# timweiland/DiffEqGMRFs.jl

Hardware: AMD Instinct MI355X
Metric: GMRF posterior solves/sec (mean+samples), 256^2 Darcy (higher is better)
Workload: dtype f64; 1 GPU; darcy256: n=65536, 64 blocks x 1024, nnz=1624084; 256 independent posterior(s) per GPU and step (4 stream(s) x batch 64), each factor + mean + 64 samples; mode=problems, samples_per_problem_per_rank=64, l_blocks_kept=False

## Files before the change

diffeqgmrfs.jl_amd/_cabi.py:

```python
from __future__ import annotations

import ctypes as C
import os
from typing import Optional

_HERE = os.path.dirname(os.path.abspath(__file__))
LIB_PATH = os.environ.get("GMRF_HIP_LIBRARY") or os.path.join(_HERE, "csrc", "libgmrf_hip.so")

GMRF_OK = 0
ERR_NOT_SPD, ERR_BAD_SHAPE, ERR_BAND, ERR_HIP, ERR_NO_FACTOR, ERR_NO_DEVICE, ERR_ALLOC, ERR_RCCL = -1, -2, -3, -4, -5, -6, -7, -8
SOLVE_FULL, SOLVE_FORWARD, SOLVE_BACKWARD = 0, 1, 2
VAR_EXACT, VAR_RBMC, VAR_MC = 0, 1, 2
BLOCK_L, BLOCK_C, BLOCK_LINV = 0, 1, 2
ORDER_REFERENCE, ORDER_TWISTED = 0, 1

EXPORTS = [
    "gmrf_bt_create", "gmrf_bt_destroy", "gmrf_last_error", "gmrf_version",
    "gmrf_bt_factor_csc", "gmrf_bt_factor_blocks", "gmrf_bt_refactor_values",
    "gmrf_bt_solve", "gmrf_bt_sample", "gmrf_bt_posterior", "gmrf_bt_set_factor_rhs", "gmrf_bt_normals", "gmrf_bt_marginal_var",
    "gmrf_bt_var_accumulate", "gmrf_bt_logdet", "gmrf_bt_get_block", "gmrf_bt_factor_buffer",
    "gmrf_bt_adopt_shape", "gmrf_bt_adopt_commit", "gmrf_bt_adopt_layout", "gmrf_bt_get_layout", "gmrf_bt_block_range",
    "gmrf_bt_set_keep_l", "gmrf_bt_storage_bytes", "gmrf_bt_set_storage", "gmrf_bt_factor_begin_csc",
    "gmrf_bt_factor_step_async", "gmrf_bt_factor_end", "gmrf_bt_stats",
    "gmrf_bt_set_profiling", "gmrf_bt_set_eager", "gmrf_bt_synchronize", "gmrf_bt_set_batch", "gmrf_bt_select_problem",
    "gmrf_bt_marginal_var_batch", "gmrf_bt_selinv", "gmrf_bt_trace_inv", "gmrf_bt_set_order", "gmrf_bt_get_order", "gmrf_bt_half_stats", "gmrf_bt_export_size", "gmrf_bt_export_factor", "gmrf_bt_import_factor",
    "gmrf_comm_unique_id", "gmrf_comm_create", "gmrf_comm_destroy", "gmrf_comm_bcast_host", "gmrf_comm_allreduce_sum",
    "gmrf_bt_bcast_blocks_async", "gmrf_bt_allgather_blocks_async", "gmrf_comm_wait", "gmrf_comm_bytes", "gmrf_streams_create", "gmrf_streams_destroy",
    "gmrf_bt_packed_size", "gmrf_bt_pack_blocks_async", "gmrf_bt_unpack_blocks_async",
    "gmrf_csr_create", "gmrf_csr_destroy", "gmrf_spmm", "gmrf_spmm_rows", "gmrf_spmm_async", "gmrf_spmm_rows_async",
    "gmrf_darcy_p1_create", "gmrf_darcy_p2_create", "gmrf_darcy_p1_destroy", "gmrf_darcy_p1_pattern", "gmrf_darcy_p1_assemble",
    "gmrf_burgers_p1_create", "gmrf_burgers_p2_create", "gmrf_burgers_p1_destroy", "gmrf_burgers_p1_pattern", "gmrf_burgers_p1_tangent",
    "gmrf_shallow_water_p1_create", "gmrf_shallow_water_p1_destroy", "gmrf_shallow_water_p1_pattern", "gmrf_shallow_water_p1_qpoints",
    "gmrf_shallow_water_p1_assemble", "gmrf_shallow_water_p1_operators",
    "gmrf_assemble_create", "gmrf_assemble_destroy", "gmrf_assemble_pattern", "gmrf_assemble_precision", "gmrf_assemble_rhs",
    "gmrf_burgers_p1_tangent_batch", "gmrf_assemble_precision_batch", "gmrf_assemble_rhs_batch", "gmrf_assemble_objective_batch",
    "gmrf_gn_create", "gmrf_gn_destroy", "gmrf_gn_run", "gmrf_gn_finalize",
    "gmrf_elliptic_p1_create", "gmrf_elliptic_p1_destroy", "gmrf_elliptic_p1_pattern", "gmrf_elliptic_p1_qpoints",
    "gmrf_elliptic_p1_tangent", "gmrf_elliptic_p1_tangent_batch", "gmrf_elliptic_p1_load", "gmrf_gn_create_elliptic",
    "gmrf_darcy_p1_assemble_batch", "gmrf_dc_create", "gmrf_dc_destroy", "gmrf_dc_run",
    "gmrf_burgers_prior_create", "gmrf_burgers_prior_destroy", "gmrf_burgers_prior_pattern", "gmrf_burgers_prior_values_batch",
    "gmrf_bic_create", "gmrf_bic_destroy", "gmrf_bic_run", "gmrf_field_errors_batch",
    "gmrf_test_gemm", "gmrf_test_gemm_rate", "gmrf_test_gemm_shapes", "gmrf_test_potrf_tile", "gmrf_test_potrf_block", "gmrf_test_tile_timing", "gmrf_test_persist_stamps", "gmrf_test_persist_aborts", "gmrf_test_factor_fwd", "gmrf_test_gn_route", "gmrf_test_dc_route", "gmrf_test_bic_route", "gmrf_test_var_groups", "gmrf_test_persist_budget", "gmrf_test_clock_probe_start", "gmrf_test_clock_probe_finish",
    "gmrf_test_mfma_f64_rate", "gmrf_test_hbm_rate", "gmrf_test_microbench", "gmrf_test_symbolic_csc",
]


class SparseBlock(C.Structure):
    _fields_ = [("nnz", C.c_int64), ("ptr", C.c_void_p), ("idx", C.c_void_p), ("val", C.c_void_p)]


class Stats(C.Structure):
    _fields_ = [
        ("factor_ms", C.c_double), ("solve_ms", C.c_double), ("sample_ms", C.c_double),
        ("factor_flops", C.c_double), ("sweep_bytes", C.c_double), ("sweep_ms", C.c_double),
        ("n", C.c_int64), ("n_blocks", C.c_int64), ("block_size", C.c_int64),
        ("block_size_padded", C.c_int64), ("factor_bytes", C.c_int64),
        ("kernel_ms", C.c_double * 24), ("kernel_work", C.c_double * 24), ("kernel_launches", C.c_int64 * 24),
        ("sweep_bytes_streamed", C.c_double),
        ("persist_route", C.c_int32), ("persist_aborts", C.c_int32), ("persist_cus", C.c_int32), ("persist_refused", C.c_int32),
        ("sweep_persist", C.c_int32), ("sweep_persist_launches", C.c_int32),
    ]


class GmrfError(RuntimeError):
    def __init__(self, status: int, msg: str, info: int = 0):
        super().__init__(f"libgmrf_hip status {status}: {msg}")
        self.status = status
        self.info = info


class NotPositiveDefinite(GmrfError):
    """Julia's PosDefException(info): `.info` is the failing block (1-based)."""


_lib: Optional[C.CDLL] = None


def load() -> C.CDLL:
    global _lib
    if _lib is not None:
        return _lib
    if not os.path.exists(LIB_PATH):
        raise ImportError(
            f"{LIB_PATH} is missing: build it with `python -c 'import __graft_entry__ as g; g.build()'` "
            "or `make -C diffeqgmrfs.jl_amd/csrc` (the HIP library is the only compute path)")
    try:
        import torch
    except Exception:
        pass
    lib = C.CDLL(LIB_PATH)
    vp, i32, i64, u64, dbl = C.c_void_p, C.c_int32, C.c_int64, C.c_uint64, C.c_double
    P = C.POINTER
    sigs = {
        "gmrf_bt_create": [i32, vp, P(vp)],
        "gmrf_bt_destroy": [vp],
        "gmrf_version": [],
        "gmrf_bt_factor_csc": [vp, i64, i64, vp, vp, vp, i32, P(i32)],
        "gmrf_bt_factor_blocks": [vp, i64, i64, vp, vp, i32, i32, P(i32)],
        "gmrf_bt_refactor_values": [vp, vp, P(i32)],
        "gmrf_bt_solve": [vp, vp, vp, i64, i64, i64, i32],
        "gmrf_bt_sample": [vp, u64, i64, i64, vp, vp, vp, i64],
        "gmrf_bt_posterior": [vp, vp, u64, i64, i64, vp, vp, i64],
        "gmrf_bt_set_factor_rhs": [vp, vp],
        "gmrf_bt_normals": [vp, u64, i64, i64, vp, i64],
        "gmrf_bt_marginal_var": [vp, i32, i64, u64, vp, vp],
        "gmrf_bt_var_accumulate": [vp, i32, i64, i64, u64, vp, vp],
        "gmrf_bt_logdet": [vp, P(dbl)],
        "gmrf_bt_get_block": [vp, i32, i64, vp, i64],
        "gmrf_bt_factor_buffer": [vp, i32, P(vp), P(i64)],
        "gmrf_bt_adopt_shape": [vp, i64, i64],
        "gmrf_bt_storage_bytes": [i64, i64, i64, P(i64), P(i64), P(i64)],
        "gmrf_bt_set_storage": [vp, i64, i64, i64, vp, vp, vp],
        "gmrf_bt_adopt_commit": [vp, i32],
        "gmrf_bt_adopt_layout": [vp, i64, i64, vp, i64],
        "gmrf_bt_get_layout": [vp, vp, i64, P(i64)],
        "gmrf_bt_block_range": [vp, i32, i64, i64, P(i64), P(i64), P(i64)],
        "gmrf_bt_set_keep_l": [vp, i32],
        "gmrf_comm_unique_id": [vp],
        "gmrf_comm_create": [i32, i32, i32, vp, P(vp)],
        "gmrf_comm_destroy": [vp],
        "gmrf_comm_bcast_host": [vp, vp, i64, i32],
        "gmrf_comm_allreduce_sum": [vp, vp, vp, i64],
        "gmrf_bt_bcast_blocks_async": [vp, vp, i32, i64, i64, i32],
        "gmrf_bt_allgather_blocks_async": [vp, vp, vp, i64, i64],
        "gmrf_comm_wait": [vp, vp],
        "gmrf_comm_bytes": [vp, i32, P(dbl)],
        "gmrf_bt_packed_size": [vp, i64, i64, P(i64)],
        "gmrf_bt_pack_blocks_async": [vp, i64, i64, vp],
        "gmrf_bt_unpack_blocks_async": [vp, i64, i64, vp],
        "gmrf_streams_create": [i32, i32, vp, vp],
        "gmrf_streams_destroy": [i32, i32, vp],
        "gmrf_bt_factor_begin_csc": [vp, i64, i64, vp, vp, vp, i32],
        "gmrf_bt_factor_step_async": [vp, i64, i64],
        "gmrf_bt_factor_end": [vp, P(i32)],
        "gmrf_bt_stats": [vp, P(Stats)],
        "gmrf_bt_set_order": [vp, i32, i64],
        "gmrf_bt_get_order": [vp, P(i32), P(i64)],
        "gmrf_bt_half_stats": [vp, i32, P(Stats)],
        "gmrf_bt_set_profiling": [vp, i32],
        "gmrf_bt_set_eager": [vp, i32],
        "gmrf_bt_synchronize": [vp],
        "gmrf_bt_set_batch": [vp, i64],
        "gmrf_bt_select_problem": [vp, i64],
        "gmrf_csr_create": [i32, vp, i64, i64, vp, vp, vp, i32, i32, P(vp)],
        "gmrf_bt_marginal_var_batch": [vp, i32, i64, u64, vp, vp, vp],
        "gmrf_bt_selinv": [vp, vp, vp],
        "gmrf_bt_trace_inv": [vp, vp, vp, i64, vp],
        "gmrf_bt_export_size": [vp, P(i64)],
        "gmrf_bt_export_factor": [vp, vp, i64],
        "gmrf_bt_import_factor": [vp, vp, i64],
        "gmrf_csr_destroy": [vp],
        "gmrf_assemble_create": [i32, vp, i64, vp, vp, i64, vp, vp, i32, P(vp)],
        "gmrf_assemble_destroy": [vp],
        "gmrf_assemble_pattern": [vp, P(i64), P(i64), vp, vp, i32],
        "gmrf_assemble_precision": [vp, vp, vp, dbl, vp],
        "gmrf_assemble_rhs": [vp, vp, vp, vp, vp, dbl, vp],
        "gmrf_darcy_p1_create": [i32, vp, i64, i64, P(vp)],
        "gmrf_darcy_p2_create": [i32, vp, i64, i64, P(vp)],
        "gmrf_darcy_p1_destroy": [vp],
        "gmrf_darcy_p1_pattern": [vp, P(i64), vp, vp, i32],
        "gmrf_darcy_p1_assemble": [vp, vp, i64, dbl, vp, vp],
        "gmrf_burgers_p1_create": [i32, vp, i64, i64, dbl, dbl, P(vp)],
        "gmrf_burgers_p2_create": [i32, vp, i64, i64, dbl, dbl, P(vp)],
        "gmrf_burgers_p1_destroy": [vp],
        "gmrf_burgers_p1_pattern": [vp, P(i64), vp, vp, i32],
        "gmrf_burgers_p1_tangent": [vp, vp, vp, vp],
        "gmrf_burgers_p1_tangent_batch": [vp, i64, vp, vp, vp],
        "gmrf_assemble_precision_batch": [vp, i64, vp, i64, vp, dbl, vp],
        "gmrf_assemble_rhs_batch": [vp, i64, vp, vp, vp, vp, dbl, vp],
        "gmrf_assemble_objective_batch": [vp, i64, vp, i64, vp, vp, vp, dbl, vp],
        "gmrf_gn_create": [vp, vp, vp, P(vp)],
        "gmrf_gn_create_elliptic": [vp, vp, vp, P(vp)],
        "gmrf_elliptic_p1_create": [i32, vp, i64, i64, P(vp)],
        "gmrf_elliptic_p1_destroy": [vp],
        "gmrf_elliptic_p1_pattern": [vp, P(i64), vp, vp, i32],
        "gmrf_elliptic_p1_qpoints": [vp, vp],
        "gmrf_elliptic_p1_tangent": [vp, vp, vp, vp],
        "gmrf_elliptic_p1_tangent_batch": [vp, i64, vp, vp, vp],
        "gmrf_elliptic_p1_load": [vp, i64, vp, vp],
        "gmrf_gn_destroy": [vp],
        "gmrf_gn_run": [vp, vp, i64, vp, vp, vp, vp, dbl, dbl, i32, vp, vp, P(i32)],
        "gmrf_gn_finalize": [vp, P(i32)],
        "gmrf_darcy_p1_assemble_batch": [vp, i64, vp, i64, dbl, vp, vp],
        "gmrf_dc_create": [vp, vp, vp, P(vp)],
        "gmrf_dc_destroy": [vp],
        "gmrf_dc_run": [vp, vp, i64, dbl, vp, i64, vp, dbl, i64, u64, i32, i64, u64, vp, vp, vp, vp, P(i32)],
        "gmrf_burgers_prior_create": [i32, vp, i64, i64, dbl, dbl, dbl, P(vp)],
        "gmrf_burgers_prior_destroy": [vp],
        "gmrf_burgers_prior_pattern": [vp, P(i64), vp, vp, i32],
        "gmrf_burgers_prior_values_batch": [vp, i64, vp, vp, vp, vp],
        "gmrf_bic_create": [vp, vp, vp, P(vp)],
        "gmrf_bic_destroy": [vp],
        "gmrf_bic_run": [vp, vp, vp, vp, vp, vp, P(i32)],
        "gmrf_field_errors_batch": [i32, vp, i64, i64, i64, vp, vp, vp],
        "gmrf_shallow_water_p1_create": [i32, vp, i64, i64, P(vp)],
        "gmrf_shallow_water_p1_destroy": [vp],
        "gmrf_shallow_water_p1_pattern": [vp, i32, P(i64), vp, vp, i32],
        "gmrf_shallow_water_p1_qpoints": [vp, vp],
        "gmrf_shallow_water_p1_assemble": [vp, vp, dbl, dbl, dbl, vp, vp, vp, vp],
        "gmrf_shallow_water_p1_operators": [vp, vp, vp, vp, vp, dbl, dbl, dbl, vp, vp, vp, vp],
        "gmrf_spmm": [vp, vp, vp, i64, i64, i64],
        "gmrf_spmm_async": [vp, vp, vp, i64, i64, i64],
        "gmrf_spmm_rows_async": [vp, vp, vp, i64, i64, i64],
        "gmrf_spmm_rows": [vp, vp, vp, i64, i64, i64],
        "gmrf_test_gemm": [i32, i64, i64, i64, i32, i32, i32, i32, dbl, vp, i64, vp, i64, dbl, vp, i64],
        "gmrf_test_gemm_shapes": [vp, P(dbl), i64, P(i64)],
        "gmrf_test_gemm_rate": [i32, i64, i64, i64, i32, i32, i32, i32, i32, i32, P(dbl)],
        "gmrf_test_potrf_tile": [i32, vp, vp, P(i32)],
        "gmrf_test_potrf_block": [i32, i64, vp, vp, P(i32)],
        "gmrf_test_tile_timing": [vp, i32],
        "gmrf_test_persist_stamps": [vp, i32],
        "gmrf_test_persist_aborts": [vp, vp],
        "gmrf_test_factor_fwd": [vp, vp, vp],
        "gmrf_test_gn_route": [vp, P(i32), P(i32)],
        "gmrf_test_dc_route": [vp, vp],
        "gmrf_test_bic_route": [vp, vp],
        "gmrf_test_var_groups": [vp, vp, vp],
        "gmrf_test_persist_budget": [i32, i32, vp, vp],
        "gmrf_test_clock_probe_start": [i32, i32, i32, P(vp)],
        "gmrf_test_clock_probe_finish": [vp, vp, vp],
        "gmrf_test_mfma_f64_rate": [i32, P(dbl)],
        "gmrf_test_hbm_rate": [i32, i64, P(dbl)],
        "gmrf_test_microbench": [i32, vp, i32],
        "gmrf_test_symbolic_csc": [i64, i64, vp, vp, i32, vp],
    }
    for name, args in sigs.items():
        fn = getattr(lib, name)
        fn.argtypes = args
        fn.restype = i32
    lib.gmrf_last_error.argtypes = []
    lib.gmrf_last_error.restype = C.c_char_p
    _lib = lib
    return lib


def check(status: int, info: int = 0):
    if status == GMRF_OK:
        return
    msg = load().gmrf_last_error().decode(errors="replace")
    if status == ERR_NOT_SPD:
        raise NotPositiveDefinite(status, msg, info)
    raise GmrfError(status, msg, info)


def ptr(a) -> C.c_void_p:
    if a is None:
        return C.c_void_p(0)
    if isinstance(a, int):
        return C.c_void_p(a)
    if hasattr(a, "data_ptr"):
        return C.c_void_p(a.data_ptr())
    return C.c_void_p(a.ctypes.data)
```

diffeqgmrfs.jl_amd/csrc/gemm_f64.hpp:

```cpp
#pragma once
#include <hip/hip_runtime.h>
#include <hip/hip_ext.h>
#include <stdint.h>
#include <stdlib.h>
#include <algorithm>
#include <array>
#include <map>
#include <mutex>
#include <vector>

namespace gmrf {

typedef double v4d __attribute__((ext_vector_type(4)));
typedef double v2d __attribute__((ext_vector_type(2)));

enum : int {
    TRI_A_LOWER = 1,
    TRI_A_UPPER = 2,
    TRI_B_LOWER = 4,
    TRI_B_UPPER = 8
};

struct GemmArgs {
    const double* A;
    const double* B;
    double* C;
    int64_t lda, ldb, ldc;
    int64_t strideA, strideB, strideC;
    int64_t pA, pB, pC;
    int nb1;
    int M, N, K;
    int tri;
    int lower_only;
    double alpha, beta;
    const double* D;
    int64_t ldd, pD;
    unsigned long long* stamps;
    const int* kb_m = nullptr;
    const int* kb_n = nullptr;
    const int* ke_n = nullptr;
    const double* tA = nullptr;
    double* tC = nullptr;
    const double* tD = nullptr;
    int64_t ptA = 0, ptC = 0, ptD = 0;
    double tbeta = 0.0;
};

constexpr int GEMM_BM = 64;
constexpr int GEMM_BN = 64;

template <bool ROWS_CONTIG, int BK>
__device__ __forceinline__ void gemm_load_tile(const double* __restrict__ P, int64_t ld, int row0, int k0,
                                               int t, v2d (&rg)[BK / 8]) {
    if (!ROWS_CONTIG) {
        constexpr int TPR = BK / 2, RPP = 256 / TPR;
        const int r = t / TPR, kk = (t % TPR) * 2;
        const double* p = P + (int64_t)(row0 + r) * ld + k0 + kk;
#pragma unroll
        for (int i = 0; i < BK / 8; ++i) rg[i] = *reinterpret_cast<const v2d*>(p + (int64_t)(i * RPP) * ld);
    } else {
        const int kk = t >> 5, r = (t & 31) * 2;
        const double* p = P + (int64_t)(k0 + kk) * ld + row0 + r;
#pragma unroll
        for (int i = 0; i < BK / 8; ++i) rg[i] = *reinterpret_cast<const v2d*>(p + (int64_t)(i * 8) * ld);
    }
}

template <bool ROWS_CONTIG, int BK>
__device__ __forceinline__ void gemm_tile_offsets(int64_t ld, int row0, int t, uint32_t (&off)[BK / 8]) {
    if (!ROWS_CONTIG) {
        constexpr int TPR = BK / 2, RPP = 256 / TPR;
        const int r = t / TPR, kk = (t % TPR) * 2;
#pragma unroll
        for (int i = 0; i < BK / 8; ++i) off[i] = (uint32_t)(((int64_t)(row0 + r + i * RPP) * ld + kk) * 8);
    } else {
        const int kk = t >> 5, r = (t & 31) * 2;
#pragma unroll
        for (int i = 0; i < BK / 8; ++i) off[i] = (uint32_t)(((int64_t)(kk + i * 8) * ld + row0 + r) * 8);
    }
}
template <bool ROWS_CONTIG>
__device__ __forceinline__ const char* gemm_tile_base(const double* P, int64_t ld, int k0) {
    return reinterpret_cast<const char*>(ROWS_CONTIG ? P + (int64_t)k0 * ld : P + k0);
}
template <int BK>
__device__ __forceinline__ void gemm_load_tile_off(const char* base, uint32_t (&off)[BK / 8], v2d (&rg)[BK / 8]) {
#pragma unroll
    for (int i = 0; i < BK / 8; ++i) {
        asm volatile("" : "+v"(off[i]));
        rg[i] = *reinterpret_cast<const v2d*>(base + off[i]);
    }
}

template <int BK>
__device__ __forceinline__ void gemm_store_tile_natural(double* sm, int t, const v2d (&rg)[BK / 8]) {
    const int kk = t >> 5, r = (t & 31) * 2;
#pragma unroll
    for (int i = 0; i < BK / 8; ++i) *reinterpret_cast<v2d*>(sm + (kk + 8 * i) * 64 + r) = rg[i];
}

template <bool ROWS_CONTIG, int BK>
__device__ __forceinline__ void gemm_store_tile(double* sm, int t, const v2d (&rg)[BK / 8]) {
    constexpr int LD = BK + 4;
    if (!ROWS_CONTIG) {
        constexpr int TPR = BK / 2, RPP = 256 / TPR;
        const int r = t / TPR, kk = (t % TPR) * 2;
#pragma unroll
        for (int i = 0; i < BK / 8; ++i) *reinterpret_cast<v2d*>(sm + (r + i * RPP) * LD + kk) = rg[i];
    } else {
        const int kk = t >> 5, r = (t & 31) * 2;
#pragma unroll
        for (int i = 0; i < BK / 8; ++i) {
            sm[r * LD + kk + 8 * i] = rg[i].x;
            sm[(r + 1) * LD + kk + 8 * i] = rg[i].y;
        }
    }
}

template <int BT>
__device__ __forceinline__ void gemm_tile_order(const GemmArgs& g, int& bm, int& bn, int& z) {
    const int nx = g.N / BT, ny = g.M / BT;
    const int tpp = g.lower_only == 1 ? nx * (nx + 1) / 2 : nx * ny;
    const int nz = (int)gridDim.x / tpp;
    const int groups = (nz % 8 == 0) ? 8 : 1;
    const int xg = (int)blockIdx.x % groups, q = (int)blockIdx.x / groups, nzg = nz / groups;
    int zq;
    if (g.lower_only == 1) {
        const int tile = q % tpp;
// ... 594 lines not shown
```

diffeqgmrfs.jl_amd/csrc/gemm_f64_dma.hpp:

```cpp
#pragma once
#include "gemm_f64.hpp"

namespace gmrf {

constexpr int DMA_BK = 16;
constexpr int DMA_ROWS_ASCENDING = 1024;
#ifndef GMRF_DMA_READS_FIRST
#define GMRF_DMA_READS_FIRST 0
#endif

template <int BM, int BN>
constexpr size_t gemm_dma_lds_bytes(int stages) { return (size_t)stages * (BM + BN) * DMA_BK * sizeof(double); }

#define GMRF_LDS_PTR(p) ((__attribute__((address_space(3))) void*)(p))
#define GMRF_GLB_PTR(p) ((const __attribute__((address_space(1))) void*)(p))

template <int BM, int BN>
__device__ __forceinline__ void gemm_dma_tile_order(const GemmArgs& g, int& bm, int& bn, int& z) {
    const int nx = g.N / BN, ny = g.M / BM;
    int tpp;
    if (g.lower_only == 1) {
        if (BM >= BN) tpp = (BM / BN) * ny * (ny + 1) / 2;
        else tpp = 0;
    } else tpp = nx * ny;
    const int nz = (int)gridDim.x / tpp;
    const int groups = (nz % 8 == 0) ? 8 : 1;
    const int xg = (int)blockIdx.x % groups, q = (int)blockIdx.x / groups, nzg = nz / groups;
    int zq;
    if (g.lower_only == 1) {
        constexpr int R = BM / BN > 0 ? BM / BN : 1;
        const int tile = q % tpp;
        zq = q / tpp;
        const int tr = (g.tri & DMA_ROWS_ASCENDING) ? tile : tpp - 1 - tile;
        int b = (int)((sqrtf(8.0f * (float)(tr / R) + 1.0f) - 1.0f) * 0.5f);
        while (R * b * (b + 1) / 2 > tr) --b;
        while (R * (b + 1) * (b + 2) / 2 <= tr) ++b;
        bm = b;
        bn = tr - R * b * (b + 1) / 2;
    } else {
        const bool cls_n = (g.tri & (TRI_B_LOWER | TRI_B_UPPER)) || !(g.tri & (TRI_A_LOWER | TRI_A_UPPER));
        const bool desc = cls_n ? ((g.tri & TRI_B_UPPER) != 0 || (g.ke_n && !g.kb_n)) : (g.tri & TRI_A_LOWER) != 0;
        const int ncls = cls_n ? nx : ny, other = cls_n ? ny : nx;
        int c = q / (other * nzg);
        const int rem = q % (other * nzg);
        const int o = rem % other;
        zq = rem / other;
        if (desc) c = ncls - 1 - c;
        bn = cls_n ? c : o;
        bm = cls_n ? o : c;
    }
    z = xg + groups * zq;
}

template <int BM, int BN, bool B_N, int STAGES, bool A_T = false, bool TAIL = false>
__global__ __launch_bounds__(256, (BM + BN > 128) ? 3 : 4) void gemm_f64_dma(GemmArgs g) {
    constexpr int BK = DMA_BK;
    constexpr int MI = BM / 32, NJ = BN / 32;
    constexpr int NA = BM / 32, NB = BN / 32;
    constexpr int A_ST = BM * BK, B_ST = BN * BK, T_ST = TAIL ? BK : 0, ST = A_ST + B_ST + T_ST;
    static_assert(NJ % 2 == 0 || !B_N, "the [k][n] image pairs neighbouring column tiles");
    static_assert(MI % 2 == 0 || !A_T, "the [k][m] image pairs neighbouring row tiles");
    static_assert(!TAIL || (BM == 64 && BN == 64 && !A_T), "the tail row: 64 x 64 tiles");
    int bm, bn, z;
    gemm_dma_tile_order<BM, BN>(g, bm, bn, z);
    const bool tail = TAIL && (g.lower_only == 1 ? bm == bn : bm == g.M / BM - 1);
    const int m0 = bm * BM, n0 = bn * BN;
    if (g.lower_only == 2 && n0 > m0 + BM - 1) return;
    const int zi = z % g.nb1, zp = z / g.nb1;
    const double* __restrict__ A = g.A + (int64_t)zi * g.strideA + (int64_t)zp * g.pA;
    const double* __restrict__ B = g.B + (int64_t)zi * g.strideB + (int64_t)zp * g.pB;
    double* C = g.C + (int64_t)zi * g.strideC + (int64_t)zp * g.pC;
    const double* Dm = g.D ? g.D + (int64_t)zp * g.pD : C;
    const int64_t ldd = g.D ? g.ldd : g.ldc;

    int kb = 0, ke = g.K;
    if (g.tri & TRI_A_LOWER) ke = min(ke, m0 + BM);
    if (g.tri & TRI_A_UPPER) kb = max(kb, m0);
    if (g.tri & TRI_B_LOWER) kb = max(kb, n0);
    if (g.tri & TRI_B_UPPER) ke = min(ke, n0 + BN);
    if (g.kb_m) kb = max(kb, g.kb_m[bm * (BM / 64)]);
    if (g.kb_n) kb = max(kb, g.kb_n[bn * (BN / 64)]);
    if (g.ke_n) ke = min(ke, g.ke_n[bn * (BN / 64) + BN / 64 - 1]);
    const int nkt = (ke > kb) ? (ke - kb) / BK : 0;

    extern __shared__ __attribute__((aligned(16))) double gsm[];
    const int t = threadIdx.x;
    const int lane = t & 63, w = __builtin_amdgcn_readfirstlane(t >> 6);
    const int wm = (w >> 1) * (BM / 2), wn = (w & 1) * (BN / 2);
    const int li = lane & 15, lq = lane >> 4;
    const bool idle = g.lower_only != 0 && ((n0 + wn) / 64 > (m0 + wm + BM / 2 - 1) / 64);

    uint32_t offa[NA], offb[NB];
#pragma unroll
    for (int i = 0; i < NA; ++i) {
        const int q = w + 4 * i;
        if (A_T) {
            constexpr int LPR = BM / 2;
            const int k = q * (64 / LPR) + lane / LPR, col = (lane % LPR) * 2;
            offa[i] = (uint32_t)(((int64_t)k * g.lda + m0 + col) * 8);
        } else {
            const int row = 8 * q + (lane >> 3), ch = (lane & 7) ^ ((row >> 1) & 7);
            offa[i] = (uint32_t)(((int64_t)(m0 + row) * g.lda + 2 * ch) * 8);
        }
    }
#pragma unroll
    for (int i = 0; i < NB; ++i) {
        const int q = w + 4 * i;
        if (B_N) {
            constexpr int LPR = BN / 2;
            const int k = q * (64 / LPR) + lane / LPR, col = (lane % LPR) * 2;
            offb[i] = (uint32_t)(((int64_t)k * g.ldb + n0 + col) * 8);
        } else {
            const int row = 8 * q + (lane >> 3), ch = (lane & 7) ^ ((row >> 1) & 7);
            offb[i] = (uint32_t)(((int64_t)(n0 + row) * g.ldb + 2 * ch) * 8);
        }
    }
    const double* arow = g.tC ? g.tA + (int64_t)zp * g.ptA : A + (int64_t)g.M * g.lda;
    auto issue = [&](int kt, int stage) {
        const int k0 = kb + kt * BK;
        const char* abase = reinterpret_cast<const char*>(A_T ? A + (int64_t)k0 * g.lda : A + k0);
        const char* bbase = reinterpret_cast<const char*>(B_N ? B + (int64_t)k0 * g.ldb : B + k0);
        double* as = gsm + stage * ST;
        double* bs = as + A_ST;
        if constexpr (TAIL)
            if (tail && w == 0 && lane < 8)
                __builtin_amdgcn_global_load_lds(GMRF_GLB_PTR(arow + k0 + 2 * lane), GMRF_LDS_PTR(bs + B_ST), 16, 0, 0);
#pragma unroll
        for (int i = 0; i < NA; ++i) {
            asm volatile("" : "+v"(offa[i]));
            __builtin_amdgcn_global_load_lds(GMRF_GLB_PTR(abase + offa[i]), GMRF_LDS_PTR(as + (w + 4 * i) * 128), 16, 0, 0);
        }
#pragma unroll
        for (int i = 0; i < NB; ++i) {
            asm volatile("" : "+v"(offb[i]));
            __builtin_amdgcn_global_load_lds(GMRF_GLB_PTR(bbase + offb[i]), GMRF_LDS_PTR(bs + (w + 4 * i) * 128), 16, 0, 0);
        }
    };

    v4d acc[MI][NJ];
#pragma unroll
    for (int i = 0; i < MI; ++i)
#pragma unroll
        for (int j = 0; j < NJ; ++j) acc[i][j] = (v4d){0.0, 0.0, 0.0, 0.0};
    v2d tacc = (v2d){0.0, 0.0};
    const int tkg = w >> 1;

    int fa[MI], fb[NJ];
#pragma unroll
// ... 2 lines not shown
        fa[i] = A_T ? (2 * lq + (i & 1)) * BM + wm + 32 * (i >> 1) + 2 * li : row * 16 + 2 * (lq ^ ((row >> 1) & 3));
    }
    int sa2[MI], sb2[NJ];
#pragma unroll
    for (int i = 0; i < MI; ++i) { const int row = wm + 16 * i + li; sa2[i] = (!A_T && ((row >> 1) & 4)) ? 8 : 0; }
    if (!B_N) {
#pragma unroll
        for (int j = 0; j < NJ; ++j) {
            const int row = wn + 16 * j + li;
            fb[j] = A_ST + row * 16 + 2 * (lq ^ ((row >> 1) & 3));
            sb2[j] = ((row >> 1) & 4) ? 8 : 0;
        }
    } else {
#pragma unroll
        for (int j = 0; j < NJ; ++j) { fb[j] = A_ST + (2 * lq + (j & 1)) * BN + wn + 32 * (j >> 1) + 2 * li; sb2[j] = 0; }
    }

    constexpr int DEPTH = STAGES - 1;
#pragma unroll
    for (int s = 0; s < DEPTH; ++s)
        if (s < nkt) issue(s, s);
    for (int kt = 0; kt < nkt; ++kt) {
        const int ahead = min(DEPTH - 1, nkt - 1 - kt);
        if (ahead <= 0) asm volatile("s_waitcnt vmcnt(0)" ::: "memory");
        else if (ahead == 1) asm volatile("s_waitcnt vmcnt(%0)" ::"n"(NA + NB) : "memory");
        else asm volatile("s_waitcnt vmcnt(%0)" ::"n"(2 * (NA + NB)) : "memory");
        __builtin_amdgcn_s_barrier();
        __builtin_amdgcn_sched_barrier(0);
        if (!GMRF_DMA_READS_FIRST && kt + DEPTH < nkt) issue(kt + DEPTH, (kt + DEPTH) % STAGES);
        if (!idle) {
            const double* sm = gsm + (kt % STAGES) * ST;
            v2d a[BK / 8][MI], b[BK / 8][NJ];
#pragma unroll
            for (int kg = 0; kg < BK / 8; ++kg) {
#pragma unroll
                for (int i = 0; i < MI; ++i) a[kg][i] = *reinterpret_cast<const v2d*>(sm + fa[i] + (A_T ? kg * 8 * BM : ((kg * 8) ^ sa2[i])));
#pragma unroll
                for (int j = 0; j < NJ; ++j)
                    b[kg][j] = *reinterpret_cast<const v2d*>(sm + fb[j] + (B_N ? kg * 8 * BN : ((kg * 8) ^ sb2[j])));
            }
            v2d ta = (v2d){0.0, 0.0};
            if constexpr (TAIL)
                if (tail) ta = *reinterpret_cast<const v2d*>(sm + A_ST + B_ST + tkg * 8 + 2 * lq);
            __builtin_amdgcn_sched_barrier(0);
            if (GMRF_DMA_READS_FIRST && kt + DEPTH < nkt) issue(kt + DEPTH, (kt + DEPTH) % STAGES);
            __builtin_amdgcn_sched_barrier(0);
#pragma unroll
            for (int kg = 0; kg < BK / 8; ++kg)
#pragma unroll
                for (int p = 0; p < 2; ++p)
#pragma unroll
                    for (int i = 0; i < MI; ++i)
#pragma unroll
                        for (int j = 0; j < NJ; ++j) {
                            double av;
                            if (A_T) av = (i & 1) ? a[kg][2 * (i >> 1) + p].y : a[kg][2 * (i >> 1) + p].x;
                            else av = p ? a[kg][i].y : a[kg][i].x;
                            double bv;
                            if (B_N) bv = (j & 1) ? b[kg][2 * (j >> 1) + p].y : b[kg][2 * (j >> 1) + p].x;
                            else bv = p ? b[kg][j].y : b[kg][j].x;
                            acc[i][j] = __builtin_amdgcn_mfma_f64_16x16x4f64(av, bv, acc[i][j], 0, 0, 0);
                        }
            if constexpr (TAIL) {
                if (tail) {
                    const v2d b0 = tkg ? b[1][0] : b[0][0], b1 = tkg ? b[1][1] : b[0][1];
                    if (B_N) {
                        tacc.x = fma(ta.x, b0.x, tacc.x); tacc.x = fma(ta.y, b1.x, tacc.x);
                        tacc.y = fma(ta.x, b0.y, tacc.y); tacc.y = fma(ta.y, b1.y, tacc.y);
                    } else {
                        tacc.x = fma(ta.x, b0.x, tacc.x); tacc.x = fma(ta.y, b0.y, tacc.x);
                        tacc.y = fma(ta.x, b1.x, tacc.y); tacc.y = fma(ta.y, b1.y, tacc.y);
                    }
                }
            }
            __builtin_amdgcn_sched_barrier(0);
        } else if (GMRF_DMA_READS_FIRST && kt + DEPTH < nkt) issue(kt + DEPTH, (kt + DEPTH) % STAGES);
    }
    if (idle) return;

    const double alpha = g.alpha, beta = g.beta;
    auto orow = [&](int i, int r) -> int64_t {
        return A_T ? m0 + wm + 32 * (i >> 1) + 2 * (lq + 4 * r) + (i & 1) : m0 + wm + i * 16 + lq + 4 * r;
    };
    if (B_N) {
        v2d d[MI][4][NJ / 2 > 0 ? NJ / 2 : 1];
        if (beta != 0.0) {
#pragma unroll
            for (int i = 0; i < MI; ++i)
#pragma unroll
                for (int r = 0; r < 4; ++r)
#pragma unroll
                    for (int jp = 0; jp < NJ / 2; ++jp)
                        d[i][r][jp] = *reinterpret_cast<const v2d*>(Dm + orow(i, r) * ldd + n0 + wn + jp * 32 + 2 * li);
        }
#pragma unroll
        for (int i = 0; i < MI; ++i)
#pragma unroll
            for (int r = 0; r < 4; ++r)
#pragma unroll
                for (int jp = 0; jp < NJ / 2; ++jp) {
                    v2d v = (v2d){alpha * acc[i][2 * jp][r], alpha * acc[i][2 * jp + 1][r]};
                    if (beta != 0.0) { v.x += beta * d[i][r][jp].x; v.y += beta * d[i][r][jp].y; }
                    *reinterpret_cast<v2d*>(C + orow(i, r) * g.ldc + n0 + wn + jp * 32 + 2 * li) = v;
                }
    } else {
        double d[MI][4][NJ];
        if (beta != 0.0) {
#pragma unroll
            for (int i = 0; i < MI; ++i)
#pragma unroll
                for (int r = 0; r < 4; ++r)
#pragma unroll
                    for (int j = 0; j < NJ; ++j)
                        d[i][r][j] = Dm[orow(i, r) * ldd + n0 + wn + j * 16 + li];
        }
#pragma unroll
        for (int i = 0; i < MI; ++i)
#pragma unroll
            for (int r = 0; r < 4; ++r)
#pragma unroll
                for (int j = 0; j < NJ; ++j) {
                    double v = alpha * acc[i][j][r];
                    if (beta != 0.0) v += beta * d[i][r][j];
                    C[orow(i, r) * g.ldc + n0 + wn + j * 16 + li] = v;
                }
    }
    if constexpr (TAIL) {
        if (tail) {
            __syncthreads();
            if (B_N) *reinterpret_cast<v2d*>(gsm + (tkg * 4 + lq) * BN + wn + 2 * li) = tacc;
            else { gsm[(tkg * 4 + lq) * BN + wn + li] = tacc.x; gsm[(tkg * 4 + lq) * BN + wn + 16 + li] = tacc.y; }
            __syncthreads();
            if (w == 0) {
                double s = 0.0;
#pragma unroll
                for (int q = 0; q < 8; ++q) s += gsm[q * BN + lane];
                double v = alpha * s;
                if (g.tC) {
                    double* tc = g.tC + (int64_t)zp * g.ptC;
                    const double* td = g.tD ? g.tD + (int64_t)zp * g.ptD : tc;
                    if (g.tbeta != 0.0) v += g.tbeta * td[n0 + lane];
                    tc[n0 + lane] = v;
                } else {
                    if (beta != 0.0) v += beta * Dm[(int64_t)g.M * ldd + n0 + lane];
                    C[(int64_t)g.M * g.ldc + n0 + lane] = v;
                }
            }
        }
    }
}

inline int& gemm_dma_policy() {
    static int v = [] { const char* e = getenv("GMRF_GEMM_DMA"); return e ? atoi(e) : 2; }();
    return v;
}
inline int& gemm_dma_force() {
    static int v = 0;
    return v;
}
inline int gemm_dma_stages() {
    static const int v = [] { const char* e = getenv("GMRF_GEMM_DMA_STAGES"); const int s = e ? atoi(e) : 2; return s == 3 ? 3 : 2; }();
    return v;
}

inline int gemm_dma_shape(bool a_t, const GemmArgs& g, int batch) {
    const int policy = gemm_dma_force() ? 2 : gemm_dma_policy();
    if (policy == 0 || g.stamps || (g.tri & ~15) || g.K % DMA_BK || g.M % 64 || g.N % 64) return 0;
    if ((g.lda & 1) || (g.ldb & 1) || ((uintptr_t)g.A & 15) || ((uintptr_t)g.B & 15) || ((g.strideA | g.strideB | g.pA | g.pB) & 1)) return 0;
    if (((uintptr_t)g.C & 15) || (g.ldc & 1) || ((g.strideC | g.pC) & 1)) return 0;
    if (g.D && (((uintptr_t)g.D & 15) || (g.ldd & 1) || (g.pD & 1))) return 0;
    if ((int64_t)g.M * g.ldc * 8 >= ((int64_t)1 << 32) || (g.D && (int64_t)g.M * g.ldd * 8 >= ((int64_t)1 << 32))) return 0;
    if ((int64_t)(a_t ? g.K : g.M) * g.lda * 8 >= ((int64_t)1 << 32) || (int64_t)std::max(g.N, g.K) * g.ldb * 8 >= ((int64_t)1 << 32)) return 0;
    if (a_t) return 1;
    const int force = gemm_dma_force();
    if (force == 2 && g.M % 128 == 0) return 2;
    if (force == 3 && g.N % 128 == 0 && !g.lower_only) return 3;
    if (force) return 1;
    if (policy == 1) return 1;
    const bool plain = !g.lower_only && !g.tri && !g.kb_m && !g.kb_n && !g.ke_n;
    const int64_t t64 = (int64_t)(g.M / 64) * (g.N / 64) * batch;
    if (policy >= 3 || (plain && t64 >= 2048)) {
        if (g.M % 128 == 0) return 2;
        if (g.N % 128 == 0 && !g.lower_only) return 3;
    }
    return 1;
}
inline bool gemm_uses_dma(bool a_t, const GemmArgs& g, int batch) { return gemm_dma_shape(a_t, g, batch) != 0; }

inline hipError_t gemm_dma_init() {
    hipError_t e = hipSuccess;
#define GMRF_DMA_ATTR(BM, BN, BNAT, ST)                                                                          \
    if (e == hipSuccess)                                                                                          \
        e = hipFuncSetAttribute((const void*)gemm_f64_dma<BM, BN, BNAT, ST>, hipFuncAttributeMaxDynamicSharedMemorySize, \
                                (int)gemm_dma_lds_bytes<BM, BN>(ST) + 64 * 1024);
    GMRF_DMA_ATTR(64, 64, false, 2) GMRF_DMA_ATTR(64, 64, true, 2) GMRF_DMA_ATTR(64, 64, false, 3) GMRF_DMA_ATTR(64, 64, true, 3)
    GMRF_DMA_ATTR(128, 64, false, 2) GMRF_DMA_ATTR(128, 64, true, 2) GMRF_DMA_ATTR(128, 64, false, 3) GMRF_DMA_ATTR(128, 64, true, 3)
    GMRF_DMA_ATTR(64, 128, false, 2) GMRF_DMA_ATTR(64, 128, true, 2) GMRF_DMA_ATTR(64, 128, false, 3) GMRF_DMA_ATTR(64, 128, true, 3)
#undef GMRF_DMA_ATTR
    return e;
}

inline bool gemm_tail_ok(bool a_t, bool b_n, const GemmArgs& g, int batch) {
    if (a_t || gemm_uses_ll(g, batch) || gemm_dma_shape(false, g, batch) != 1) return false;
    if (g.lower_only && g.M != g.N) return false;
    if (g.tC) {
        return g.nb1 == 1 && g.tA && ((uintptr_t)g.tA & 15) == 0 && (g.ptA & 1) == 0;
    }
    if (!b_n || g.lower_only) return false;
    return (int64_t)(g.M + 1) * g.ldc * 8 < ((int64_t)1 << 32) && (!g.D || (int64_t)(g.M + 1) * g.ldd * 8 < ((int64_t)1 << 32));
}
inline bool gemm_try_dma_tail(hipStream_t st, bool a_t, bool b_n, const GemmArgs& g, int batch, hipEvent_t ev_start, hipEvent_t ev_stop,
                              hipError_t* err) {
    if (!gemm_tail_ok(a_t, b_n, g, batch)) return false;
    const bool tri_grid = g.lower_only && g.M == g.N;
    GemmArgs gs = g;
    gs.lower_only = tri_grid ? 1 : 0;
    static const bool asc_off = [] { const char* e = getenv("GMRF_GEMM_G2_ORDER"); return e && atoi(e) == 0; }();
    if (tri_grid && (g.kb_m || g.kb_n) && !asc_off) gs.tri |= DMA_ROWS_ASCENDING;
    const int64_t nx = g.N / 64, ny = g.M / 64;
    const dim3 grid((unsigned)((tri_grid ? ny * (ny + 1) / 2 : nx * ny) * batch)), block(256);
    const size_t lds = (size_t)gemm_dma_stages() * (64 + 64 + DMA_BK) * DMA_BK * sizeof(double);
#define GMRF_DMA_TK(BNAT, ST)                                                                                              \
    do {                                                                                                                   \
        if (ev_start) hipExtLaunchKernelGGL((gemm_f64_dma<64, 64, BNAT, ST, false, true>), grid, block, lds, st, ev_start, ev_stop, 0, gs); \
        else hipLaunchKernelGGL((gemm_f64_dma<64, 64, BNAT, ST, false, true>), grid, block, lds, st, gs);                \
    } while (0)
    if (gemm_dma_stages() == 3) {
        if (b_n) GMRF_DMA_TK(true, 3); else GMRF_DMA_TK(false, 3);
    } else {
        if (b_n) GMRF_DMA_TK(true, 2); else GMRF_DMA_TK(false, 2);
    }
#undef GMRF_DMA_TK
    *err = hipGetLastError();
    return true;
}

inline bool gemm_try_dma(hipStream_t st, bool a_t, bool b_n, const GemmArgs& g, int batch, hipEvent_t ev_start, hipEvent_t ev_stop,
                         hipError_t* err) {
    const int shape = gemm_dma_shape(a_t, g, batch);
    if (shape == 0) return false;
    const bool tri_grid = g.lower_only && g.M == g.N;
    GemmArgs gs = g;
    gs.lower_only = tri_grid ? 1 : (g.lower_only ? 2 : 0);
    static const bool asc_off = [] { const char* e = getenv("GMRF_GEMM_G2_ORDER"); return e && atoi(e) == 0; }();
    if (tri_grid && (g.kb_m || g.kb_n) && !asc_off) gs.tri |= DMA_ROWS_ASCENDING;
    const int stages = gemm_dma_stages();
    const dim3 block(256);
#define GMRF_DMA_GO(BM, BN)                                                                                       \
    do {                                                                                                          \
        const int64_t nx = g.N / BN, ny = g.M / BM;                                                               \
        const int64_t tiles = tri_grid ? (int64_t)(BM / BN > 0 ? BM / BN : 1) * ny * (ny + 1) / 2 : nx * ny;      \
        const dim3 grid((unsigned)(tiles * batch));                                                               \
        static const size_t lds_pad = [] { const char* e = getenv("GMRF_GEMM_DMA_LDS_PAD_KB"); return (size_t)(e ? atoi(e) : 0) * 1024; }();    \
        const size_t lds = gemm_dma_lds_bytes<BM, BN>(stages) + lds_pad;                                          \
        if (a_t && BM == 64 && BN == 64) {                                                                        \
            if (b_n) GMRF_DMA_K((gemm_f64_dma<64, 64, true, 2, true>)); else GMRF_DMA_K((gemm_f64_dma<64, 64, false, 2, true>)); \
        } else if (stages == 3) {                                                                                 \
            if (b_n) GMRF_DMA_K((gemm_f64_dma<BM, BN, true, 3>)); else GMRF_DMA_K((gemm_f64_dma<BM, BN, false, 3>)); \
        } else {                                                                                                  \
            if (b_n) GMRF_DMA_K((gemm_f64_dma<BM, BN, true, 2>)); else GMRF_DMA_K((gemm_f64_dma<BM, BN, false, 2>)); \
        }                                                                                                         \
    } while (0)
#define GMRF_DMA_K(KERNEL)                                                                                        \
    do {                                                                                                          \
        if (ev_start) hipExtLaunchKernelGGL(KERNEL, grid, block, lds, st, ev_start, ev_stop, 0, gs);              \
        else hipLaunchKernelGGL(KERNEL, grid, block, lds, st, gs);                                                \
    } while (0)
    if (shape == 2) GMRF_DMA_GO(128, 64);
    else if (shape == 3) GMRF_DMA_GO(64, 128);
    else GMRF_DMA_GO(64, 64);
#undef GMRF_DMA_K
#undef GMRF_DMA_GO
    *err = hipGetLastError();
    return true;
}

}
```

diffeqgmrfs.jl_amd/csrc/gmrf_hip.hip:

```cpp
#include <hip/hip_runtime.h>
#include <dlfcn.h>
#include <stdint.h>
#include <stdlib.h>
#include <string.h>
#include <time.h>

#include <algorithm>
#include <atomic>
#include <iterator>
#include <cmath>
#include <map>
#include <memory>
#include <chrono>
#include <functional>
#include <initializer_list>
#include <mutex>
#include <string>
#include <type_traits>
#include <vector>

#include "../../include/gmrf_hip.h"
#include "assemble.hpp"
#include "fem_assemble.hpp"
#include "gemm_f64.hpp"
// ... 98 lines not shown
struct GemmShapeStat {
    int64_t key[8];
    double launches = 0, ms = 0, work = 0;
};

struct TwistState;

struct gmrf_handle {
    int device = 0;
    hipStream_t stream = nullptr;
    bool own_stream = false;
    int64_t n = 0, N = 0, bs = 0, bsp = 0, n_pad = 0;
    int64_t B = 1;
    int64_t sel = 0;
    int64_t alloc_B = 0, vals_B = 0;
    int64_t nnz_in = 0, n_entries = 0;
    uint64_t* d_keys = nullptr;
    double* d_vals = nullptr;
    int64_t* d_src = nullptr;
    double* d_nz_stage = nullptr;
    std::vector<int64_t> diag_first, diag_count, low_first, low_count;
    bool analyzed = false;
    int64_t cmin = 0, rmax = 0;
    std::vector<int> kst, mend;
    int* d_kst = nullptr;
    int* d_mend = nullptr;
    int* d_kbx = nullptr;
    int kst_cap = 0;
    double c_streamed = 0.0;
    double g2_tile_k = 0.0;
    bool c_dirty = false;
    int* d_lo_rowptr = nullptr;
    int* d_dg_rowptr = nullptr;
    int* d_bxt_uptr = nullptr; int* d_bxt_ucols = nullptr; uint16_t* d_bxt_lidx = nullptr; int* d_bxt_gtiles = nullptr;
    std::vector<int> bxt_ng;
    int bxt_ecap = 0; int bxt_nrt = 0; bool bxt_plan_ok = false;
    int64_t lo_row_max = 0;
    bool sparse_b = false;
    bool dense_g1 = false;
    double *d_L = nullptr, *d_C = nullptr, *d_Linv = nullptr;
    bool external_storage = false;
    bool keep_l = true;
    bool l_valid = false;
    bool logdet_valid = false;
    std::vector<char> got_block;
    int64_t alloc_rm = 0, alloc_wc = 0;
    bool alloc_keep_l = true;
    double *d_S = nullptr, *d_B = nullptr, *d_T = nullptr, *d_W = nullptr;
    double* d_V = nullptr;
    int64_t v_elems = 0;
    uint64_t layout_gen = 0;
    uint64_t sel_csr = 0, sel_gen = ~0ull;
    int64_t sel_nnz = 0;
    std::vector<int64_t> sel_off, sel_nd;
    int64_t* d_sel_src = nullptr;
    int64_t* d_sel_slot = nullptr;
    int64_t sel_cap = 0;
    double* d_sig = nullptr;
    int64_t sig_elems = 0;
    double* d_dv = nullptr;
    int64_t dv_elems = 0;
    int* d_info = nullptr;
    double* d_logdet = nullptr;
    int64_t alloc_N = 0, alloc_bsp = 0;
    bool factored = false;
    double *d_P = nullptr, *d_Y = nullptr, *d_Tp = nullptr;
    int64_t kp_cap = 0;
    double* d_stage = nullptr;
    int64_t stage_cap = 0;
    DevBuf mean_arena;
    double* d_acc = nullptr;
    int64_t acc_B = 0;
    int32_t var_group = 0, var_groups = 0;
    bool eager = false;
    bool split_step = false;
    bool sweep_no_gemm = false;
    bool no_fused_posterior = false;
    bool tail_probe = false;
    bool tail_refused = false;
    const double* frhs = nullptr;
    const double* fy_for = nullptr;
    bool fwd_run = false;
    bool no_factor_fwd = false;
    double* d_ft = nullptr;
    double* d_fy = nullptr;
    int64_t fy_elems = 0;
    const double* factor_graph_rhs = nullptr;
    unsigned long long* dbg_stamps = nullptr;
    bool fork_graph = false;
    bool no_staircase = false;
    bool doubling_x = false;
    int xsplit = 0;
    int adopt_xsplit = 0;
    bool no_xsplit = false;
    bool no_lookahead = false;
    bool no_persist = false;
    bool persist_gave_up = false;
    bool persist_launched = false;
    int persist_cus = 0;
    int info_checked = 0;
    int factor_graph_route = 0;
    int persist_aborts = 0;
    int cu_count = 0;
    unsigned* d_pflags = nullptr;
    int64_t pflags_words = 0;
    bool no_sweep_persist = false;
    bool no_scatter_fold = false;
    bool sweep_persist_planned = false;
    bool sweep_persist_launched = false;
    unsigned* d_sweep_flags = nullptr;
    double* d_Tsw = nullptr;
    int64_t t_elems = 0;
    unsigned* h_sweep_abort = nullptr;
    int sweep_nw = 0;
    double *d_P2 = nullptr, *d_Y2 = nullptr, *d_T2 = nullptr;
    int64_t p2_elems = 0;
    bool sweep_persist_hold = false;
    bool no_persist_panels = false;
    hipStream_t aux = nullptr;
    bool aux_distinct = false;
    hipStream_t gemm_stream = nullptr;
    bool capturing = false;
    std::vector<hipEvent_t> fork_events;
    size_t fork_next = 0;
    hipGraphExec_t factor_graph = nullptr;
    int64_t factor_graph_i0 = -1, factor_graph_i1 = -1;
    std::map<int64_t, hipGraphExec_t> sweep_graphs;
    int profiling = 0;
    std::vector<EvPair> events;
    std::vector<hipEvent_t> ev_pool;
    std::vector<GemmShapeStat> gemm_shapes;
    gmrf_stats stats;
    hipEvent_t ev0 = nullptr, ev1 = nullptr;
    int order = GMRF_ORDER_REFERENCE;
    int64_t meet_req = -1;
    int32_t eager_bits = 0;
    TwistState* tw = nullptr;
    int64_t tw_blk = -1;
    const double* tw_hj = nullptr;
    double* tw_w = nullptr;
};

struct TwistState {
    gmrf_handle* top = nullptr;
    gmrf_handle* bot = nullptr;
    int64_t m = -1, N = 0, n = 0, bs = 0, bsp = 0, nnz = 0;
    uint64_t* d_mkeys = nullptr;
    int64_t* d_msrc = nullptr;
    double* d_mvals = nullptr;
    int64_t m_count = 0;
    double *d_Bm = nullptr, *d_HJ = nullptr, *d_W = nullptr, *d_Smm = nullptr;
    int64_t dense_bsp = 0;
    double* d_nz = nullptr;
    const double* d_nz_cur = nullptr;
    double* d_z = nullptr;
    double* d_var = nullptr;
    hipEvent_t ev_fork = nullptr, ev_join = nullptr;
};


static bool tw_on(const gmrf_handle* h) { return h && h->tw && h->tw->bot; }
static gmrf_handle* tw_route(gmrf_handle* h) {
    return (h && h->order == GMRF_ORDER_TWISTED && h->tw && h->tw->top && !h->tw->bot && h->factored) ? h->tw->top : h;
}
static gmrf_status tw_refuse(const gmrf_handle* h, const char* what) {
    if (!h || h->order != GMRF_ORDER_TWISTED) return GMRF_OK;
    g_last_error = std::string(what) + ": not supported on a handle in the twisted elimination order (gmrf_bt_set_order)";
    return GMRF_ERR_BAD_SHAPE;
}

static void destroy_graphs(gmrf_handle* h) {
    if (h->factor_graph) { (void)hipGraphExecDestroy(h->factor_graph); h->factor_graph = nullptr; }
    for (auto& kv : h->sweep_graphs) (void)hipGraphExecDestroy(kv.second);
    h->sweep_graphs.clear();
}

static hipEvent_t ev_get(gmrf_handle* h) {
    if (!h->ev_pool.empty()) {
        hipEvent_t e = h->ev_pool.back();
        h->ev_pool.pop_back();
        return e;
    }
    hipEvent_t e;
    (void)hipEventCreate(&e);
    return e;
}

struct ProfScope {
    gmrf_handle* h;
    EvPair p;
    bool on;
    ProfScope(gmrf_handle* hh, int kind, double work) : h(hh), on(hh->profiling > 0) {
        if (on) {
            p.kind = kind; p.work = work;
            p.a = ev_get(h); p.b = ev_get(h);
            (void)hipEventRecord(p.a, h->stream);
        }
    }
    ~ProfScope() {
        if (on) {
            (void)hipEventRecord(p.b, h->stream);
            h->events.push_back(p);
        }
    }
};

static void prof_collect(gmrf_handle* h) {
    for (auto& p : h->events) {
        float ms = 0.f;
        (void)hipEventElapsedTime(&ms, p.a, p.b);
        h->stats.kernel_ms[p.kind] += ms; h->stats.kernel_work[p.kind] += p.work; h->stats.kernel_launches[p.kind]++;
        if (p.shape >= 0) { auto& g = h->gemm_shapes[(size_t)p.shape]; g.launches += 1; g.ms += ms; g.work += p.work; }
        h->ev_pool.push_back(p.a);
        h->ev_pool.push_back(p.b);
    }
    h->events.clear();
}

struct GemmTail {
    const double* A; int64_t pA;
    double* C; int64_t pC;
    const double* D; int64_t pD;
    double beta;
};

static gmrf_status gemm(gmrf_handle* h, bool a_t, bool b_n, int M, int N, int K, int tri, int lower_only,
                        double alpha, const double* A, int64_t lda, const double* B, int64_t ldb,
                        double beta, double* C, int64_t ldc, int64_t pA, int64_t pB, int64_t pC,
                        int batch = 1, int64_t sA = 0, int64_t sB = 0, int64_t sC = 0, const double* D = nullptr,
                        int64_t ldd = 0, int64_t pD = 0, int pclass = 0, double pwork = -1.0,
                        const int* kb_m = nullptr, const int* kb_n = nullptr, const int* ke_n = nullptr, bool tail = false,
                        const GemmTail* gt = nullptr) {
    GemmArgs g;
    if (gt) {
        g.tA = gt->A; g.ptA = gt->pA; g.tC = gt->C; g.ptC = gt->pC; g.tD = gt->D; g.ptD = gt->pD; g.tbeta = gt->beta;
        tail = true;
    }
    g.kb_m = kb_m; g.kb_n = kb_n; g.ke_n = ke_n;
    g.D = D; g.ldd = ldd; g.pD = pD;
    g.A = A; g.B = B; g.C = C;
    g.lda = lda; g.ldb = ldb; g.ldc = ldc;
    g.strideA = sA; g.strideB = sB; g.strideC = sC;
    g.pA = pA; g.pB = pB; g.pC = pC; g.nb1 = batch;
    g.M = M; g.N = N; g.K = K; g.tri = tri; g.lower_only = lower_only;
    g.alpha = alpha; g.beta = beta; g.stamps = nullptr;
    double flops = 2.0 * M * N * (double)K * batch * (double)h->B;
    if (lower_only) flops *= 0.5 * (1.0 + 64.0 / std::max(M, 64));
    if (tri) flops *= 0.5 * (1.0 + 64.0 / std::max(K, 64));
    if (tail) {
        if (!gemm_tail_ok(a_t, b_n, g, batch * (int)h->B)) {
            h->tail_refused = true;
            return h->tail_probe ? GMRF_OK : bad_shape("internal: a product does not qualify for the tail-row GEMM");
        }
        if (h->tail_probe) return GMRF_OK;
        flops *= (M + 1.0) / M;
        if (pwork >= 0.0) pwork *= (M + 1.0) / M;
        pclass = b_n ? 15 : 14;
        hipError_t e = hipSuccess;
        if (h->profiling > 0) {
            EvPair p;
            p.kind = pclass; p.work = pwork >= 0.0 ? pwork : flops;
            p.a = ev_get(h); p.b = ev_get(h);
            const int64_t key[8] = {pclass, M + 1, N, K, tri, lower_only, batch * h->B, (kb_m || kb_n || ke_n) ? 1 : 0};
            for (size_t i = 0; i < h->gemm_shapes.size() && p.shape < 0; ++i)
                if (!memcmp(h->gemm_shapes[i].key, key, sizeof(key))) p.shape = (int)i;
            if (p.shape < 0) {
                GemmShapeStat st; memcpy(st.key, key, sizeof(key));
                h->gemm_shapes.push_back(st); p.shape = (int)h->gemm_shapes.size() - 1;
            }
            (void)gemm_try_dma_tail(h->gemm_stream ? h->gemm_stream : h->stream, a_t, b_n, g, batch * (int)h->B, p.a, p.b, &e);
            HIPCHK(e);
            h->events.push_back(p);
            return GMRF_OK;
        }
        (void)gemm_try_dma_tail(h->gemm_stream ? h->gemm_stream : h->stream, a_t, b_n, g, batch * (int)h->B, nullptr, nullptr, &e);
        HIPCHK(e);
        return GMRF_OK;
    }
    if (gemm_uses_big(a_t, g, batch * (int)h->B)) { pclass = b_n ? 7 : 6; pwork = -1.0; }
    else if (pclass == 0) {
        if (gemm_uses_ll(g, batch * (int)h->B)) pclass = 13;
        else if (gemm_uses_dma(a_t, g, batch * (int)h->B)) pclass = a_t ? 18 : (b_n ? 15 : 14);
        else pclass = a_t ? 12 : (b_n ? 11 : 0);
    }
    if (h->profiling > 0) {
        EvPair p;
        p.kind = pclass; p.work = pwork >= 0.0 ? pwork : flops;
        p.a = ev_get(h); p.b = ev_get(h);
        const int64_t key[8] = {pclass, M, N, K, tri, lower_only, batch * h->B, (kb_m || kb_n || ke_n) ? 1 : 0};
        for (size_t i = 0; i < h->gemm_shapes.size() && p.shape < 0; ++i)
            if (!memcmp(h->gemm_shapes[i].key, key, sizeof(key))) p.shape = (int)i;
        if (p.shape < 0) {
            GemmShapeStat st; memcpy(st.key, key, sizeof(key));
            h->gemm_shapes.push_back(st); p.shape = (int)h->gemm_shapes.size() - 1;
        }
        HIPCHK(launch_gemm(h->gemm_stream ? h->gemm_stream : h->stream, a_t, b_n, g, batch * (int)h->B, p.a, p.b));
        h->events.push_back(p);
        return GMRF_OK;
    }
    HIPCHK(launch_gemm(h->gemm_stream ? h->gemm_stream : h->stream, a_t, b_n, g, batch * (int)h->B));
    return GMRF_OK;
}

static inline int64_t blk_elems(const gmrf_handle* h) { return h->bsp * h->bsp; }
static inline int64_t c_ld(const gmrf_handle* h) { return h->bsp - h->cmin; }
static inline int64_t c_blk(const gmrf_handle* h) { return h->rmax * (h->bsp - h->cmin); }
static inline int64_t stride_pL(const gmrf_handle* h) { return blk_elems(h) * (h->keep_l ? h->N : 1); }
static inline int64_t stride_pX(const gmrf_handle* h) { return blk_elems(h) * h->N; }
static inline int64_t stride_pC(const gmrf_handle* h) { return c_blk(h) * std::max<int64_t>(h->N - 1, 1); }
static inline double* l_block(const gmrf_handle* h, int64_t i) { return h->d_L + (h->keep_l ? i * blk_elems(h) : 0); }

static gmrf_status set_layout(gmrf_handle* h, int64_t cmin, int64_t rmax, const std::vector<int64_t>& kst_abs) {
    const int64_t bsp = h->bsp;
    if (cmin < 0 || cmin >= bsp || cmin % 64 || rmax <= 0 || rmax > bsp || rmax % 64) return bad_shape("bad coupling-block layout");
    const int nrt = (int)(rmax / 64), nct = (int)((bsp - cmin) / 64), ntile = (int)(bsp / 64);
    if ((int)kst_abs.size() != nrt) return bad_shape("bad coupling-block layout (row tiles)");
    (void)hipStreamSynchronize(h->stream);
    destroy_graphs(h);
    h->cmin = cmin; h->rmax = rmax;
    h->layout_gen++;
    h->kst.assign((size_t)ntile, 0);
    int64_t run = bsp - 64;
    for (int t = nrt - 1; t >= 0; --t) {
        int64_t v = std::min(std::max(kst_abs[t], cmin), bsp - 64);
        run = std::min(run, (v / 64) * 64);
        h->kst[t] = (int)(run - cmin);
    }
    if (nrt > 0) h->kst[0] = 0;
    for (int t = nrt; t < ntile; ++t) h->kst[t] = (int)(bsp - cmin);
    h->mend.assign((size_t)ntile, (int)rmax);
    for (int u = 0; u < nct; ++u) {
        int m = 0;
        for (int t = 0; t < nrt; ++t) if (h->kst[t] <= 64 * u) m = 64 * (t + 1);
        h->mend[u] = m;
    }
    h->c_streamed = 0.0; h->g2_tile_k = 0.0;
    for (int t = 0; t < nrt; ++t) {
        h->c_streamed += 64.0 * (double)(bsp - cmin - h->kst[t]);
        h->g2_tile_k += (double)(t + 1) * (double)(bsp - cmin - h->kst[t]);
    }
    if (!h->d_kst || !h->d_mend || h->kst_cap < ntile) {
        free_dev(h->d_kst); free_dev(h->d_mend); free_dev(h->d_kbx); h->d_kst = h->d_mend = h->d_kbx = nullptr; h->kst_cap = 0;
        HIPCHK(hipMalloc(&h->d_kst, sizeof(int) * ntile));
        HIPCHK(hipMalloc(&h->d_mend, sizeof(int) * ntile));
        HIPCHK(hipMalloc(&h->d_kbx, sizeof(int) * ntile));
        h->kst_cap = ntile;
    }
    {
        std::vector<int> kbx((size_t)ntile);
        for (int u = 0; u < ntile; ++u) kbx[(size_t)u] = (int)std::max<int64_t>(0, 64 * (int64_t)u - cmin);
        HIPCHK(hipMemcpyAsync(h->d_kbx, kbx.data(), sizeof(int) * ntile, hipMemcpyHostToDevice, h->stream));
        HIPCHK(hipStreamSynchronize(h->stream));
    }
    HIPCHK(hipMemcpyAsync(h->d_kst, h->kst.data(), sizeof(int) * ntile, hipMemcpyHostToDevice, h->stream));
    HIPCHK(hipMemcpyAsync(h->d_mend, h->mend.data(), sizeof(int) * ntile, hipMemcpyHostToDevice, h->stream));
    HIPCHK(hipStreamSynchronize(h->stream));
    h->c_dirty = true;
    return GMRF_OK;
}

static gmrf_status set_layout_dense(gmrf_handle* h) {
    return set_layout(h, 0, h->bsp, std::vector<int64_t>((size_t)(h->bsp / 64), 0));
}

static gmrf_status alloc_work(gmrf_handle* h);
static gmrf_status alloc_factor(gmrf_handle* h) {
    if (h->alloc_N == h->N && h->alloc_bsp == h->bsp && h->alloc_B == h->B && h->alloc_rm == h->rmax &&
        h->alloc_wc == c_ld(h) && h->alloc_keep_l == h->keep_l && h->d_Linv)
        return GMRF_OK;
    destroy_graphs(h);
    h->logdet_valid = false;
    if (h->external_storage) {
        if (h->alloc_N != h->N || h->alloc_bsp != h->bsp || h->alloc_B != h->B || h->alloc_keep_l != h->keep_l) {
            g_last_error = "external factor storage does not match the shape / batch";
            return GMRF_ERR_BAD_SHAPE;
        }
        h->alloc_rm = h->rmax; h->alloc_wc = c_ld(h);
        h->l_valid = false;
        return GMRF_OK;
    }
    free_dev(h->d_L); free_dev(h->d_C); free_dev(h->d_Linv);
    free_dev(h->d_S); free_dev(h->d_B); free_dev(h->d_T); free_dev(h->d_W);
    free_dev(h->d_logdet);
// ... 513 lines not shown
    return GMRF_OK;
}

static gmrf_status potrf_block(gmrf_handle* h, double* S, double* L, double* X, double* T, int blk_id, double* fy = nullptr) {
    const int bsp = (int)h->bsp;
    const int64_t ld = bsp;
    const int nt = bsp / 64;
    const int route = potrf_route(h);
    const bool fused = route == ROUTE_FUSED;
    if (h->xsplit > 0 && route != ROUTE_PANELS256) return bad_shape("internal: split inverse planned off the 256-column panel route");
    static const int pw_env = [] { const char* e = getenv("GMRF_PANEL_TILES"); return e ? atoi(e) : 4; }();
    const int pw = (!fused && nt >= 8) ? ((pw_env == 2 || pw_env == 8) ? pw_env : 4) : nt;
    const bool fused_in_panel = route == ROUTE_BIG_ONE;
    const bool overlap = h->capturing && h->fork_graph && nt >= 8;
    if (overlap && !h->aux) HIPCHK(hipStreamCreateWithFlags(&h->aux, hipStreamNonBlocking));
    hipEvent_t ev_fork = nullptr, ev_join = nullptr;
    if (overlap) { GCHK(fork_event(h, &ev_fork)); GCHK(fork_event(h, &ev_join)); }
    if (fused && !h->no_lookahead && !h->doubling_x && !overlap && nt >= 2 && persist_fits(h, nt, 0, nt, 1)) {
        const double t3 = 64.0 * 64.0 * 64.0;
        double fl = t3 / 3.0 * nt;
        for (int j = 0; j + 1 < nt; ++j) {
            const int m = nt - j - 1;
            fl += (double)m * t3 + 2.0 * t3 * (m * (m + 1) / 2) + 2.0 * t3 * (0.5 * (double)(j + 1) * (j + 2) + 0.625 * (j + 1));
        }
        return launch_persist(h, S, L, X, nt, 0, nt, 1, blk_id, fl);
    }
    if (fused && !h->no_lookahead && !h->doubling_x && !overlap && nt >= 2) {
        StepArgs sa;
        sa.S = S; sa.L = L; sa.X = X; sa.ld = ld; sa.nt = nt; sa.cend = nt;
        sa.info = h->d_info; sa.blk = blk_id; sa.dbg = nullptr;
        sa.pS = (int64_t)bsp * bsp; sa.pL = stride_pL(h); sa.pX = stride_pX(h); sa.blk_per_problem = (int)h->N;
        const double t3 = 64.0 * 64.0 * 64.0;
        {
            sa.j = 0; sa.lookahead = 0; sa.xrow = -1;
            ProfScope ps(h, 1, t3 / 3.0);
            hipLaunchKernelGGL(potrf_step<false>, dim3(1, 1), dim3(256), POTRF_TILE_LDS, h->stream, sa);
        }
        for (int j = 0; j + 1 < nt; ++j) {
            const int m = nt - j - 1, ntile_wg = m * (m + 1) / 2;
            sa.j = j; sa.lookahead = 1;
            sa.xrow = (j >= 1) ? j : -1; sa.xrow_first = ntile_wg;
            const int nx_wg = (j >= 1) ? 4 * j : 0;
            const double f_x = (j >= 1) ? 2.0 * t3 * (0.5 * (double)j * (j + 1) + 0.625 * j) : 0.0;
            ProfScope ps(h, 1, t3 / 3.0 + (double)m * t3 + 2.0 * t3 * ntile_wg + f_x);
            hipLaunchKernelGGL(potrf_step<false>, dim3(ntile_wg + nx_wg, 1), dim3(256), POTRF_STEP_LDS, h->stream, sa);
        }
        {
            sa.j = nt - 1; sa.lookahead = 0; sa.xrow = nt - 1; sa.xrow_first = 0;
            ProfScope ps(h, 1, 2.0 * t3 * (0.5 * (double)(nt - 1) * nt + 0.625 * (nt - 1)));
            hipLaunchKernelGGL(potrf_step<false>, dim3(4 * (nt - 1), 1), dim3(256), 64 * 18 * sizeof(double), h->stream, sa);
        }
        HIPCHK(hipGetLastError());
        return GMRF_OK;
    }
    if (fy && (route != ROUTE_PANELS256 || overlap)) return bad_shape("internal: forward solve planned off the 256-column panel route");
    if (route == ROUTE_PANELS256 && !overlap) {
        StepArgs sa;
        sa.S = S; sa.L = L; sa.X = X; sa.ld = ld; sa.nt = nt; sa.cend = nt;
        sa.info = h->d_info; sa.blk = blk_id; sa.dbg = nullptr;
        sa.pS = (int64_t)bsp * bsp; sa.pL = stride_pL(h); sa.pX = stride_pX(h); sa.blk_per_problem = (int)h->N;
        const int64_t pW = (int64_t)bsp * bsp;
        const double t3 = 64.0 * 64.0 * 64.0, nb = (double)h->B;
        auto diag128 = [&](int j) -> gmrf_status {
            sa.j = j;
            ProfScope ps(h, 16, (2.0 * t3 / 3.0 + 4.0 * 2.0 * t3 * 0.625) * nb);
            static const size_t lds_pad = [] { const char* e = getenv("GMRF_DIAG128_LDS_PAD_KB"); return (size_t)(e ? atoi(e) : 0) * 1024; }();
            static const bool fat = [] { const char* e = getenv("GMRF_DIAG128_FAT"); return e && atoi(e) != 0; }();
            if (fat) hipLaunchKernelGGL(potrf_diag128, dim3(1, (unsigned)h->B), dim3(256), POTRF_DIAG128_LDS + lds_pad, h->stream, sa);
            else hipLaunchKernelGGL(potrf_diag128_slim, dim3(1, (unsigned)h->B), dim3(256), POTRF_DIAG128_SLIM_LDS + lds_pad, h->stream, sa);
            HIPCHK(hipGetLastError());
            return GMRF_OK;
        };
        static const bool no_small = [] { const char* e = getenv("GMRF_PERSIST_PANELS"); return e && atoi(e) == 0; }();
        const bool persist_panels = !no_small && !h->no_persist_panels && persist_fits(h, 4, 0, 4, 2);
        for (int j = 0; j < nt; j += 4) {
            const int64_t oa = (int64_t)j * 64, ob = oa + 128, oc = oa + 256;
            if (persist_panels) {
                const double fl = (4.0 * t3 / 3.0 + 2.0 * t3 * (6.0 * 0.625 + 10.0 + 10.0 + 6.0 * 0.625)) * nb;
                GCHK(launch_persist(h, S + oa * ld + oa, L + oa * ld + oa, X + oa * ld + oa, 4, 0, 4, 2, blk_id, fl));
            } else {
                GCHK(diag128(j));
                GCHK(gemm(h, false, false, 128, 128, 128, TRI_B_UPPER, 0, 1.0, S + ob * ld + oa, ld, X + oa * ld + oa, ld, 0.0, L + ob * ld + oa, ld,
                          sa.pS, sa.pX, sa.pL, 1, 0, 0, 0, nullptr, 0, 0, 0, 2.0 * t3 * 3.0 * 2.0 * nb));
                GCHK(gemm(h, false, false, 128, 128, 128, 0, 1, -1.0, L + ob * ld + oa, ld, L + ob * ld + oa, ld, 1.0, S + ob * ld + ob, ld,
                          sa.pL, sa.pL, sa.pS, 1, 0, 0, 0, nullptr, 0, 0, 0, 2.0 * t3 * 2.0 * 3.0 * nb));
                GCHK(diag128(j + 2));
                GCHK(gemm(h, false, true, 128, 128, 128, TRI_B_LOWER, 0, 1.0, L + ob * ld + oa, ld, X + oa * ld + oa, ld, 0.0, T + ob * ld + oa, ld,
                          sa.pL, sa.pX, pW));
                GCHK(gemm(h, false, true, 128, 128, 128, TRI_A_LOWER, 0, -1.0, X + ob * ld + ob, ld, T + ob * ld + oa, ld, 0.0, X + ob * ld + oa, ld,
                          sa.pX, pW, sa.pX));
            }
            const int m3 = nt - j - 4;
            const int64_t pT = bsp, pY = h->n_pad;
            if (m3 <= 0) {
                if (fy) {
                    SweepArgs sw;
                    sw.Mat = X + oa * ld + oa; sw.ld = ld; sw.Xin = h->d_ft + oa; sw.ldx = pT; sw.Bin = nullptr; sw.ldb = 0;
                    sw.Out = fy + oa; sw.ldo = pY; sw.rows = 256; sw.kdim = 256; sw.sub = 0;
                    sw.pMat = sa.pX; sw.pXin = pT; sw.pBin = 0; sw.pOut = pY;
                    ProfScope ps(h, 3, 4.0 * 256.0 * 257.0 * nb);
                    HIPCHK(launch_sweep(h->stream, false, true, 1, sw, (int)h->B));
                }
                continue;
            }
            const GemmTail tp{h->d_ft + oa, pT, fy + oa, pY, nullptr, 0, 0.0};
            const GemmTail tu{fy + oa, pY, h->d_ft + oc, pT, nullptr, 0, 1.0};
            const bool in_slot = (j == 0 && h->xsplit == 256 && !h->keep_l);
            double* Lb = in_slot ? X + oc * ld + oa : L + oc * ld + oa;
            const int64_t pLb = in_slot ? sa.pX : sa.pL;
            GCHK(gemm(h, false, false, 64 * m3, 256, 256, TRI_B_UPPER, 0, 1.0, S + oc * ld + oa, ld, X + oa * ld + oa, ld, 0.0, Lb, ld,
                      sa.pS, sa.pX, pLb, 1, 0, 0, 0, nullptr, 0, 0, 0, 2.0 * t3 * 10.0 * m3 * nb, nullptr, nullptr, nullptr, false,
                      fy ? &tp : nullptr));
            GCHK(gemm(h, false, false, m3 * 64, m3 * 64, 256, 0, 1, -1.0, Lb, ld, Lb, ld, 1.0, S + oc * ld + oc, ld, pLb, pLb, sa.pS,
                      1, 0, 0, 0, nullptr, 0, 0, 0, 2.0 * t3 * 4.0 * (m3 * (m3 + 1) / 2) * nb, nullptr, nullptr, nullptr, false,
                      fy ? &tu : nullptr));
        }
        const int p = h->xsplit;
        GCHK(doubling_levels(h, L, X, T, 256, bsp / 2, -1, p));
        if (p > 0 && !(p == 256 && !h->keep_l)) {
            hipLaunchKernelGGL(copy_rect, dim3((unsigned)((bsp - p) / 4), (unsigned)h->B), dim3(256), 0, h->stream,
                               L + (int64_t)p * ld, ld, sa.pL, X + (int64_t)p * ld, ld, sa.pX, bsp - p, p);
            HIPCHK(hipGetLastError());
        }
        return GMRF_OK;
    }
    if (h->xsplit > 0) return bad_shape("internal: split inverse planned off the 256-column panel route");
    for (int j = 0; j < nt; ++j) {
        StepArgs sa;
        sa.S = S; sa.L = L; sa.X = X; sa.ld = ld; sa.j = j; sa.nt = nt;
        sa.info = h->d_info; sa.blk = blk_id; sa.dbg = h->dbg_stamps;
        sa.pS = (int64_t)bsp * bsp; sa.pL = stride_pL(h); sa.pX = stride_pX(h); sa.blk_per_problem = (int)h->N;
        const int m = nt - j - 1;
        const int cend = std::min(nt, (j / pw + 1) * pw);
        sa.cend = cend;
        int utiles = 0;
        for (int c = j + 1; c < cend; ++c) utiles += nt - c;
        const double rem = 64.0 * m, nb = (double)h->B;
        const double f_tile = 64.0 * 64.0 * 64.0 / 3.0 * nb, f_panel = rem * 64.0 * 64.0 * nb;
        const double f_upd = 2.0 * 64.0 * 64.0 * 64.0 * utiles * nb;
        if (fused_in_panel && !h->no_lookahead && !overlap && j % pw == 0 && cend - j >= 2 && persist_fits(h, nt, j, cend, 0)) {
            const int npc = cend - j;
            double fl = 64.0 * 64.0 * 64.0 / 3.0 * npc;
            for (int jj = j; jj + 1 < cend; ++jj) {
                int ut = 0;
                for (int c = jj + 1; c < cend; ++c) ut += nt - c;
                fl += 64.0 * (nt - jj - 1) * 64.0 * 64.0 + 2.0 * 64.0 * 64.0 * 64.0 * ut;
            }
            fl += 64.0 * (nt - cend) * 64.0 * 64.0;
            GCHK(launch_persist(h, S, L, X, nt, j, cend, 0, blk_id, fl));
            j = cend - 1;
            sa.j = j;
        } else if (fused || m == 0) {
            const bool xrows = fused && !h->doubling_x && !overlap && j >= 2;
            const int ntile_wg = 1 + m * (m + 1) / 2;
            sa.xrow = xrows ? j - 1 : -1; sa.xrow_first = ntile_wg;
            const int nx_wg = xrows ? 4 * (j - 1) : 0;
            const double f_x = xrows ? 2.0 * 64.0 * 64.0 * 64.0 * (0.5 * (double)(j - 1) * j + 0.625 * (j - 1)) : 0.0;
            ProfScope ps(h, 1, f_tile + f_panel + f_upd + f_x);
            hipLaunchKernelGGL(potrf_step<false>, dim3(ntile_wg + nx_wg, (unsigned)h->B), dim3(256),
                               m == 0 ? POTRF_TILE_LDS : POTRF_STEP_LDS, h->stream, sa);
            sa.xrow = -1;
        } else if (fused_in_panel && utiles > 0) {
            ProfScope ps(h, 1, f_tile + f_panel + f_upd);
            hipLaunchKernelGGL(potrf_step<false>, dim3(1 + utiles, 1), dim3(256), POTRF_STEP_LDS, h->stream, sa);
        } else {
            {
                ProfScope ps(h, 1, f_tile);
                hipLaunchKernelGGL(potrf_step<false>, dim3(1, (unsigned)h->B), dim3(256), POTRF_TILE_LDS, h->stream, sa);
            }
            {
                ProfScope ps(h, 8, f_panel);
// ... 412 lines not shown
        *h->h_sweep_abort = 0u;
    }
    const int64_t need = (int64_t)kp * h->n_pad;
    if (!h->d_Tsw || h->t_elems < need) {
        HIPCHK(hipStreamSynchronize(h->stream));
        free_dev(h->d_Tsw); h->d_Tsw = nullptr; h->t_elems = 0;
        destroy_graphs(h);
        HIPCHK(hipMalloc(&h->d_Tsw, sizeof(double) * (size_t)need));
        h->t_elems = need;
    }
    return GMRF_OK;
}

static gmrf_status launch_sweep_persist(gmrf_handle* h, bool backward, int kp, double* Pin, double* Yout, hipStream_t st_over = nullptr,
                                        double* T_over = nullptr) {
    const int nw = h->sweep_nw;
    const int64_t elems = (int64_t)kp * h->n_pad;
    hipStream_t st = st_over ? st_over : h->stream;
    double* Tp = T_over ? T_over : h->d_Tsw;
    if (!h->d_sweep_flags || !h->h_sweep_abort || nw <= 0 || !Tp || (!T_over && h->t_elems < elems))
        return bad_shape("internal: words / panel of the persistent sweeps not allocated");
    if (elems % 2 != 0) return bad_shape("internal: the persistent sweeps' panels need an even element count (sweep_fill_sentinel)");
    SweepPersistArgs a;
    a.C = h->d_C; a.Linv = h->d_Linv; a.Pin = Pin; a.T = Tp; a.Yout = Yout;
    a.N = (int)h->N; a.bsp = (int)h->bsp; a.cm = (int)h->cmin; a.rm = (int)h->rmax; a.kp = kp; a.backward = backward ? 1 : 0; a.nw = nw;
    a.npad = h->n_pad; a.ldc = c_ld(h); a.cstride = c_blk(h); a.bstride = (int64_t)h->bsp * h->bsp;
    a.kst = h->d_kst; a.mend = h->d_mend;
    a.abort_w = h->d_sweep_flags;
    void* dev_abort = nullptr;
    HIPCHK(hipHostGetDevicePointer(&dev_abort, h->h_sweep_abort, 0));
    a.host_abort = reinterpret_cast<unsigned*>(dev_abort);
    static const int limit_ms = [] {
        const char* e = getenv("GMRF_SWEEP_SPIN_MS");
        if (!e) e = getenv("GMRF_PERSIST_SPIN_MS");
        return e ? atoi(e) : -1;
    }();
    a.spin_limit = (unsigned)(limit_ms >= 0 ? limit_ms : 2000) * 100000u;
    static const int dbg = [] { const char* e = getenv("GMRF_SWEEP_DBG"); return e ? atoi(e) : 0; }();
    a.dbg = dbg;
    static const int pause_env = [] { const char* e = getenv("GMRF_SWEEP_PAUSE"); return e ? atoi(e) : -1; }();
    a.pause = (kp == 1) ? 8 : (pause_env >= 0 ? pause_env : 64);
    const double N = (double)h->N, bsp = (double)h->bsp;
    const double work = (kp == 1) ? 8.0 * ((N - 1) * h->c_streamed + N * 0.5 * bsp * (bsp + 1))
                                  : kp * (2.0 * (N - 1) * h->c_streamed + N * bsp * (bsp + 1));
    {
        ProfScope ps(h, 5, 16.0 * (double)elems);
        hipLaunchKernelGGL(sweep_fill_sentinel, dim3((unsigned)((elems / 2 + 255) / 256)), dim3(256), 0, st, Tp, Yout, elems);
        HIPCHK(hipGetLastError());
    }
    ProfScope ps(h, kp == 1 ? 19 : 20, work);
    if (kp == 1) hipLaunchKernelGGL(sweep_persist<true>, dim3((unsigned)nw), dim3(256), 0, st, a);
    else hipLaunchKernelGGL(sweep_persist<false>, dim3((unsigned)nw), dim3(256), 0, st, a);
    HIPCHK(hipGetLastError());
    return GMRF_OK;
}

static gmrf_status sweep_persist_check(gmrf_handle* h, bool* repeat) {
    *repeat = false;
    if (!h->sweep_persist_launched) return GMRF_OK;
    h->sweep_persist_launched = false;
    if (!h->h_sweep_abort || *reinterpret_cast<volatile unsigned*>(h->h_sweep_abort) == 0u) return GMRF_OK;
    *h->h_sweep_abort = 0u;
    persist_give_up(h);
    HIPCHK(hipMemsetAsync(h->d_sweep_flags, 0, sizeof(unsigned) * 16, h->stream));
    h->stats.sweep_persist = 0;
    *repeat = true;
    return GMRF_OK;
}

struct SweepIo { const void* in; int64_t in_bytes; const void* out; int64_t out_bytes; };

static gmrf_status sweep_guarded(gmrf_handle* h, std::initializer_list<SweepIo> io, const std::function<gmrf_status()>& body,
                                 const std::function<gmrf_status()>& restore = nullptr) {
    h->stats.sweep_persist = 0;
    h->sweep_persist_hold = std::any_of(io.begin(), io.end(), [](const SweepIo& r) { return ranges_overlap(r.in, r.in_bytes, r.out, r.out_bytes); });
    GCHK(body());
    bool repeat = false;
    GCHK(sweep_persist_check(h, &repeat));
    if (!repeat) return GMRF_OK;
    if (restore) GCHK(restore());
    return body();
}

static gmrf_status sweep_launches(gmrf_handle* h, bool backward, int kp, double* Pin, double* Yout, bool tail = false) {
    if (!tail && sweep_persist_ok(h, kp)) return launch_sweep_persist(h, backward, kp, Pin, Yout);
    const int bsp = (int)h->bsp;
    const int64_t ld = bsp, bstride = (int64_t)bsp * bsp, npad = h->n_pad;
    const int64_t N = h->N;
    SweepArgs s;
    s.ld = ld;
    const int nprob = (int)h->B;
    s.narrow = (nprob < 8 && bsp >= 512 && bsp <= SWEEP_PERSIST_XMAX) ? 1 : 0;
    const int64_t pPanel = (int64_t)(kp + (tail ? 1 : 0)) * npad;
    const int64_t pX = stride_pX(h), pCm = stride_pC(h);
    const int64_t ldc = c_ld(h), cstride = c_blk(h);
    const int cm = (int)h->cmin, rm = (int)h->rmax, wc = bsp - cm;
    const int pclass = (kp == 1) ? 3 : 2;
    const double blk_work_c = ((kp == 1) ? 8.0 * h->c_streamed : 2.0 * h->c_streamed * kp) * nprob;
    const double blk_work_t = ((kp == 1) ? 4.0 * bsp * (double)(bsp + 1) : 1.0 * bsp * (double)(bsp + 1) * kp) * nprob;
    const bool via_gemm = (kp % 64 == 0) && !h->sweep_no_gemm && (int64_t)nprob * (bsp / 64) * (kp / 64) >= 128;
    if (tail && (!via_gemm || !backward)) return bad_shape("internal: the tail row needs the backward sweep on the GEMM");
    for (int64_t step = 0; step < N; ++step) {
        const int64_t i = backward ? (N - 1 - step) : step;
        double* rhs = Pin + i * bsp;
        if (step > 0) {
            const int64_t ci = backward ? i : (i - 1);
            const int64_t prev = backward ? (i + 1) : (i - 1);
            const double* Cs = h->d_C + ci * cstride;
            const double* xin = Yout + prev * bsp + (backward ? 0 : cm);
            double* out = rhs + (backward ? cm : 0);
            const int rows = backward ? wc : rm, kdim = backward ? rm : wc;
            if (via_gemm) {
                GCHK(gemm(h, false, backward, kp, rows, kdim, 0, 0, -1.0, xin, npad, Cs, ldc, 1.0, out, npad, pPanel, pCm,
                          pPanel, 1, 0, 0, 0, nullptr, 0, 0, 0, 2.0 * h->c_streamed * kp * nprob,
                          nullptr, backward ? nullptr : h->d_kst, backward ? h->d_mend : nullptr, tail));
            } else {
                s.Mat = Cs; s.ld = ldc; s.Xin = xin; s.ldx = npad; s.Bin = out; s.ldb = npad; s.Out = out; s.ldo = npad;
                s.rows = rows; s.kdim = kdim; s.sub = 1;
                s.pMat = pCm; s.pXin = pPanel; s.pBin = pPanel; s.pOut = pPanel;
                s.kst = h->d_kst; s.mend = h->d_mend;
                ProfScope ps(h, pclass, blk_work_c);
                HIPCHK(launch_sweep(h->stream, backward, false, kp, s, nprob));
            }
        }
        const double* X = h->d_Linv + i * bstride;
        double* yout = Yout + i * bsp;
        if (h->xsplit > 0) {
            const int p = h->xsplit, q = bsp - p;
            const double* Xbb = X + (int64_t)p * ld + p;
            const double* Lba = X + (int64_t)p * ld;
            for (int part = 0; part < 3; ++part) {
                const int which = backward ? 2 - part : part;
                if (via_gemm) {
                    constexpr int64_t z0 = 0;
                    if (which == 0)
                        GCHK(gemm(h, false, backward, kp, p, p, backward ? TRI_B_LOWER : TRI_B_UPPER, 0, 1.0, rhs, npad, X, ld, 0.0, yout, npad,
                                  pPanel, pX, pPanel, 1, z0, z0, z0, nullptr, z0, z0, 0, -1.0, nullptr, nullptr, nullptr, tail));
                    else if (which == 2)
                        GCHK(gemm(h, false, backward, kp, q, q, backward ? TRI_B_LOWER : TRI_B_UPPER, 0, 1.0, rhs + p, npad, Xbb, ld, 0.0,
                                  yout + p, npad, pPanel, pX, pPanel, 1, z0, z0, z0, nullptr, z0, z0, 0, -1.0, nullptr, nullptr, nullptr, tail));
                    else if (!backward)
                        GCHK(gemm(h, false, false, kp, q, p, 0, 0, -1.0, yout, npad, Lba, ld, 1.0, rhs + p, npad, pPanel, pX, pPanel));
                    else
                        GCHK(gemm(h, false, true, kp, p, q, 0, 0, -1.0, yout + p, npad, Lba, ld, 1.0, rhs, npad, pPanel, pX, pPanel,
                                  1, z0, z0, z0, nullptr, z0, z0, 0, -1.0, nullptr, nullptr, nullptr, tail));
                } else {
                    s.ld = ld; s.ldx = npad; s.ldo = npad; s.pMat = pX; s.pXin = pPanel; s.pOut = pPanel; s.kst = nullptr; s.mend = nullptr;
                    if (which == 0) { s.Mat = X; s.Xin = rhs; s.Bin = nullptr; s.ldb = 0; s.Out = yout; s.rows = p; s.kdim = p; s.sub = 0; s.pBin = 0; }
                    else if (which == 2) { s.Mat = Xbb; s.Xin = rhs + p; s.Bin = nullptr; s.ldb = 0; s.Out = yout + p; s.rows = q; s.kdim = q; s.sub = 0; s.pBin = 0; }
                    else if (!backward) { s.Mat = Lba; s.Xin = yout; s.Bin = rhs + p; s.ldb = npad; s.Out = rhs + p; s.rows = q; s.kdim = p; s.sub = 1; s.pBin = pPanel; }
                    else { s.Mat = Lba; s.Xin = yout + p; s.Bin = rhs; s.ldb = npad; s.Out = rhs; s.rows = p; s.kdim = q; s.sub = 1; s.pBin = pPanel; }
                    const double frac = which == 0 ? (double)p * (p + 1) : (which == 2 ? (double)q * (q + 1) : 2.0 * p * q);
                    ProfScope ps(h, pclass, blk_work_t * frac / ((double)bsp * (bsp + 1)));
                    HIPCHK(launch_sweep(h->stream, backward, which != 1, kp, s, nprob));
                }
            }
        } else if (via_gemm) {
            GCHK(gemm(h, false, backward, kp, bsp, bsp, backward ? TRI_B_LOWER : TRI_B_UPPER, 0, 1.0, rhs, npad, X, ld, 0.0,
                      yout, npad, pPanel, pX, pPanel, 1, 0, 0, 0, nullptr, 0, 0, 0, -1.0, nullptr, nullptr, nullptr, tail));
        } else {
            s.Mat = X; s.ld = ld; s.Xin = rhs; s.ldx = npad; s.Bin = nullptr; s.ldb = 0; s.Out = yout; s.ldo = npad;
            s.rows = bsp; s.kdim = bsp; s.sub = 0;
            s.pMat = pX; s.pXin = pPanel; s.pBin = 0; s.pOut = pPanel;
            s.kst = nullptr; s.mend = nullptr;
            ProfScope ps(h, pclass, blk_work_t);
            HIPCHK(launch_sweep(h->stream, backward, true, kp, s, nprob));
        }
    }
    return GMRF_OK;
}

constexpr int SWEEP_BACKWARD_YP = 3, SWEEP_BACKWARD_TAIL = 4;
static gmrf_status run_sweeps(gmrf_handle* h, int mode, int kp) {
    auto body = [&]() -> gmrf_status {
        if (mode == GMRF_SOLVE_FORWARD) return sweep_launches(h, false, kp, h->d_P, h->d_Y);
        if (mode == SWEEP_BACKWARD_TAIL) return sweep_launches(h, true, kp, h->d_P, h->d_Y, true);
        if (mode == SWEEP_BACKWARD_YP) return sweep_launches(h, true, kp, h->d_Y, h->d_P);
        if (mode == GMRF_SOLVE_BACKWARD) return sweep_launches(h, true, kp, h->d_P, h->d_Y);
        GCHK(sweep_launches(h, false, kp, h->d_P, h->d_Y));
        return sweep_launches(h, true, kp, h->d_Y, h->d_P);
    };
    const bool persistent = mode != SWEEP_BACKWARD_TAIL && sweep_persist_ok(h, kp);
    if (persistent) {
        GCHK(sweep_persist_prepare(h, kp));
        h->sweep_persist_launched = true;
        h->stats.sweep_persist = 1;
        h->stats.sweep_persist_launches += (mode == GMRF_SOLVE_FULL) ? 2 : 1;
    }
    if (h->eager || h->profiling) return body();
    const int64_t key = ((int64_t)h->xsplit << 32) | ((int64_t)mode * 4096 + kp) |
                        (persistent ? ((int64_t)1 << 60) : 0);
    auto it = h->sweep_graphs.find(key);
    if (it == h->sweep_graphs.end()) {
        std::lock_guard<std::mutex> capture_lock(g_capture_mu);
        hipGraph_t graph = nullptr;
        hipGraphExec_t exec = nullptr;
        HIPCHK(hipStreamBeginCapture(h->stream, hipStreamCaptureModeThreadLocal));
        gmrf_status s = body();
        hipError_t e = hipStreamEndCapture(h->stream, &graph);
        if (s != GMRF_OK) { if (graph) (void)hipGraphDestroy(graph); return s; }
        HIPCHK(e);
        HIPCHK(hipGraphInstantiate(&exec, graph, nullptr, nullptr, 0));
        (void)hipGraphDestroy(graph);
        it = h->sweep_graphs.emplace(key, exec).first;
    }
    HIPCHK(hipGraphLaunch(it->second, h->stream));
    return GMRF_OK;
}

static int pad_k(int64_t k) { return k == 1 ? 1 : (int)((k + 15) / 16 * 16); }

static gmrf_status launch_pack(gmrf_handle* h, const double* d_src, int64_t ld, int k, int kp) {
    const int64_t total = (int64_t)kp * h->n_pad;
    hipLaunchKernelGGL(pack_panel, dim3((unsigned)((total + 255) / 256), (unsigned)h->B), dim3(256), 0, h->stream, d_src, ld,
                       h->d_P, h->n_pad, (int)h->bs, (int)h->bsp, (int)h->N, k, kp);
    HIPCHK(hipGetLastError());
    return GMRF_OK;
}

static gmrf_status launch_unpack(gmrf_handle* h, const double* panel, double* d_dst, int64_t ld, int k,
                                 const double* d_mean) {
    const int64_t total = h->n * (int64_t)k;
    hipLaunchKernelGGL(unpack_panel, dim3((unsigned)((total + 255) / 256), (unsigned)h->B), dim3(256), 0, h->stream, panel,
                       h->n_pad, d_dst, ld, (int)h->bs, (int)h->bsp, h->n, k, pad_k(k), d_mean);
    HIPCHK(hipGetLastError());
    return GMRF_OK;
}

static gmrf_status cols_in(gmrf_handle* h, const double* src, int64_t ld, bool src_dev, int k, const double** d_src, int64_t* d_ld) {
    *d_src = src; *d_ld = ld;
    if (src_dev) return GMRF_OK;
    GCHK(ensure_stage(h, (int64_t)k * h->n * h->B));
    HIPCHK(hipMemcpy2DAsync(h->d_stage, h->n * sizeof(double), src, ld * sizeof(double),
                            h->n * sizeof(double), k * h->B, hipMemcpyHostToDevice, h->stream));
    *d_src = h->d_stage; *d_ld = h->n;
    return GMRF_OK;
}

static gmrf_status cols_out(gmrf_handle* h, const double* panel, int k, const double* d_mean, double* dst, int64_t ld, bool dst_dev) {
    if (dst_dev) return launch_unpack(h, panel, dst, ld, k, d_mean);
    GCHK(ensure_stage(h, (int64_t)k * h->n * h->B));
    GCHK(launch_unpack(h, panel, h->d_stage, h->n, k, d_mean));
    HIPCHK(hipMemcpy2DAsync(dst, ld * sizeof(double), h->d_stage, h->n * sizeof(double),
                            h->n * sizeof(double), k * h->B, hipMemcpyDeviceToHost, h->stream));
    return GMRF_OK;
}

constexpr int64_t KP_CHUNK = 128;

static void tw_free(gmrf_handle* h);
static gmrf_status tw_analyze(gmrf_handle* h, int64_t n, int64_t N, const int64_t* colptr, const int64_t* rowval, int32_t base);
static gmrf_status tw_numeric(gmrf_handle* h, const double* nzval, int32_t* info);
static gmrf_status tw_solve(gmrf_handle* h, const double* b, double* y, int64_t k, int64_t ldb, int64_t ldy, int mode);
static gmrf_status tw_sample(gmrf_handle* h, uint64_t seed, int64_t first_id, int64_t k, const double* mean, const double* z,
                             double* out, int64_t ld);
static gmrf_status tw_logdet(gmrf_handle* h, double* out);
static gmrf_status tw_get_block(gmrf_handle* h, int32_t kind, int64_t i, double* out, int64_t ld);
static gmrf_status tw_var_exact(gmrf_handle* h, double* d_out);
static gmrf_status tw_var_accumulate_dev(gmrf_handle* h, int method, int64_t first_id, int64_t k, uint64_t seed, const gmrf_csr* Q,
                                         double* d_acc);

extern "C" {

int32_t gmrf_version(void) { return 100; }
const char* gmrf_last_error(void) { return g_last_error.c_str(); }

gmrf_status gmrf_bt_create(int32_t device, void* stream, gmrf_handle** out) {
    if (!out) return bad_shape("null out pointer");
    int count = 0;
    if (hipGetDeviceCount(&count) != hipSuccess || count <= 0 || device < 0 || device >= count) {
        (void)hipGetLastError();
        g_last_error = "no HIP device visible (libgmrf_hip needs an MI355X / gfx950 GPU)";
        return GMRF_ERR_NO_DEVICE;
    }
    HIPCHK(hipSetDevice(device));
    gmrf_handle* h = new gmrf_handle();
    memset(&h->stats, 0, sizeof(h->stats));
    h->device = device;
    if (stream) { h->stream = (hipStream_t)stream; h->own_stream = false; }
    else { HIPCHK(hipStreamCreateWithFlags(&h->stream, hipStreamNonBlocking)); h->own_stream = true; }
    HIPCHK(hipMalloc(&h->d_info, 4 * sizeof(int)));
    HIPCHK(hipMemsetAsync(h->d_info, 0, 4 * sizeof(int), h->stream));
    HIPCHK(hipStreamSynchronize(h->stream));
    HIPCHK(hipEventCreate(&h->ev0));
    HIPCHK(hipEventCreate(&h->ev1));
    HIPCHK(hipFuncSetAttribute((const void*)potrf_step<false>, hipFuncAttributeMaxDynamicSharedMemorySize, (int)POTRF_STEP_LDS));
    HIPCHK(hipFuncSetAttribute((const void*)potrf_diag128, hipFuncAttributeMaxDynamicSharedMemorySize, 160 * 1024));
    HIPCHK(hipFuncSetAttribute((const void*)potrf_persist<false>, hipFuncAttributeMaxDynamicSharedMemorySize, (int)POTRF_PERSIST_LDS));
    HIPCHK(hipDeviceGetAttribute(&h->cu_count, hipDeviceAttributeMultiprocessorCount, device));
    { const char* e = getenv("GMRF_PERSIST"); if (e && atoi(e) == 0) h->no_persist = true; }
    { const char* e = getenv("GMRF_SWEEP_PERSIST"); if (e && atoi(e) == 0) h->no_sweep_persist = true; }
    HIPCHK(hipFuncSetAttribute((const void*)potrf_diag128_slim, hipFuncAttributeMaxDynamicSharedMemorySize, 160 * 1024));
    HIPCHK(gemm_init());
    HIPCHK(gemm_dma_init());
    *out = h;
    return GMRF_OK;
}

gmrf_status gmrf_bt_destroy(gmrf_handle* h) {
    if (!h) return GMRF_OK;
    (void)hipSetDevice(h->device);
    tw_free(h);
    (void)hipStreamSynchronize(h->stream);
    persist_release(h);
    destroy_graphs(h);
    free_dev(h->d_keys); free_dev(h->d_vals); free_dev(h->d_src); free_dev(h->d_nz_stage);
    free_dev(h->d_lo_rowptr); free_dev(h->d_dg_rowptr); free_dev(h->d_kst); free_dev(h->d_mend);
    free_dev(h->d_bxt_uptr); free_dev(h->d_bxt_ucols); free_dev(h->d_bxt_lidx); free_dev(h->d_bxt_gtiles);
    if (!h->external_storage) { free_dev(h->d_L); free_dev(h->d_C); free_dev(h->d_Linv); }
    else if (!h->keep_l) free_dev(h->d_L);
    free_dev(h->d_S); free_dev(h->d_B); free_dev(h->d_T); free_dev(h->d_W);
    free_dev(h->d_sweep_flags); free_dev(h->d_Tsw); free_dev(h->d_P2); free_dev(h->d_Y2); free_dev(h->d_T2);
    if (h->h_sweep_abort) { (void)hipHostFree(h->h_sweep_abort); h->h_sweep_abort = nullptr; }
    free_dev(h->d_info); free_dev(h->d_logdet); free_dev(h->d_pflags); free_dev(h->d_kbx); free_dev(h->d_V);
    free_dev(h->d_P); free_dev(h->d_Y); free_dev(h->d_Tp);
    free_dev(h->d_stage); h->mean_arena.release(); free_dev(h->d_acc);
    free_dev(h->d_ft); free_dev(h->d_fy);
    free_dev(h->d_sel_src); free_dev(h->d_sel_slot); free_dev(h->d_sig); free_dev(h->d_dv);
    for (auto e : h->ev_pool) (void)hipEventDestroy(e);
    if (h->ev0) (void)hipEventDestroy(h->ev0);
    if (h->ev1) (void)hipEventDestroy(h->ev1);
    for (auto e : h->fork_events) (void)hipEventDestroy(e);
    if (h->aux) (void)hipStreamDestroy(h->aux);
    if (h->own_stream) (void)hipStreamDestroy(h->stream);
    delete h;
    return GMRF_OK;
}

gmrf_status gmrf_bt_set_batch(gmrf_handle* h, int64_t batch) {
    if (!h || batch < 1 || batch > 4096) return bad_shape("batch must be in [1, 4096]");
    if (batch != 1) GCHK(tw_refuse(h, "gmrf_bt_set_batch (batch > 1)"));
    if (batch != h->B) {
        HIPCHK(hipSetDevice(h->device));
        HIPCHK(hipStreamSynchronize(h->stream));
        destroy_graphs(h);
        h->B = batch;
        h->sel = 0;
        h->factored = false;
        release_shape_buffers(h);
        if (h->n > 0) (void)set_shape(h, h->n, h->N);
    }
    return GMRF_OK;
}

gmrf_status gmrf_bt_select_problem(gmrf_handle* h, int64_t p) {
    if (!h || p < 0 || p >= h->B) return bad_shape("problem index out of range");
    h->sel = p;
    return GMRF_OK;
}

gmrf_status gmrf_bt_set_profiling(gmrf_handle* h, int32_t level) {
    if (!h) return bad_shape("null handle");
    h->profiling = level;
    if (h->tw)
        for (gmrf_handle* s : {h->tw->top, h->tw->bot}) if (s) GCHK(gmrf_bt_set_profiling(s, level));
    if (level > 0 && h->events.empty()) h->gemm_shapes.clear();
    for (int i = 0; i < GMRF_KERNEL_CLASSES; ++i) { h->stats.kernel_ms[i] = h->stats.kernel_work[i] = 0; h->stats.kernel_launches[i] = 0; }
    return GMRF_OK;
}

gmrf_status gmrf_bt_set_eager(gmrf_handle* h, int32_t eager) {
    if (!h) return bad_shape("null handle");
    if (((eager & 2) != 0) != h->split_step) { destroy_graphs(h); h->split_step = (eager & 2) != 0; }
    if (((eager & 4) != 0) != h->sweep_no_gemm) { destroy_graphs(h); h->sweep_no_gemm = (eager & 4) != 0; }
    if (((eager & 8) != 0) != h->dense_g1) { destroy_graphs(h); h->dense_g1 = (eager & 8) != 0; }
    if (((eager & 16) != 0) != h->fork_graph) { destroy_graphs(h); h->fork_graph = (eager & 16) != 0; }
    h->no_staircase = (eager & 32) != 0;
    if (((eager & 128) != 0) != h->doubling_x) { destroy_graphs(h); h->doubling_x = (eager & 128) != 0; }
    if (((eager & 256) != 0) != h->no_lookahead) { destroy_graphs(h); h->no_lookahead = (eager & 256) != 0; }
    if (((eager & 4096) != 0) != h->no_xsplit) { destroy_graphs(h); h->no_xsplit = (eager & 4096) != 0; }
    if (((eager & 8192) != 0) != h->no_persist) { destroy_graphs(h); h->no_persist = (eager & 8192) != 0; }
    if (((eager & 32768) != 0) != h->no_persist_panels) { destroy_graphs(h); h->no_persist_panels = (eager & 32768) != 0; }
    if (((eager & 65536) != 0) != h->no_sweep_persist) { destroy_graphs(h); h->no_sweep_persist = (eager & 65536) != 0; }
    if (((eager & 131072) != 0) != h->no_scatter_fold) { destroy_graphs(h); h->no_scatter_fold = (eager & 131072) != 0; }
    h->no_fused_posterior = (eager & 262144) != 0;
    h->no_factor_fwd = (eager & 524288) != 0;
    if (eager != h->eager_bits) h->fy_for = nullptr;
    h->eager = (eager & 1) != 0;
    h->eager_bits = eager;
    if (h->tw)
        for (gmrf_handle* s : {h->tw->top, h->tw->bot})
            if (s) {
                GCHK(gmrf_bt_set_eager(s, eager));
                if (h->tw->bot) s->no_sweep_persist = true;
            }
    return GMRF_OK;
}

gmrf_status gmrf_bt_synchronize(gmrf_handle* h) {
    if (!h) return bad_shape("null handle");
    HIPCHK(hipStreamSynchronize(h->stream));
    if (tw_on(h)) HIPCHK(hipStreamSynchronize(h->tw->bot->stream));
    return GMRF_OK;
}

gmrf_status gmrf_bt_stats(gmrf_handle* h, gmrf_stats* out) {
    if (!h || !out) return bad_shape("null pointer");
    if (tw_on(h)) {
        const gmrf_stats &a = h->tw->top->stats, &b = h->tw->bot->stats;
        *out = h->stats;
        out->persist_route = a.persist_route;
        out->persist_aborts = a.persist_aborts + b.persist_aborts;
        out->persist_cus = a.persist_cus + b.persist_cus;
        out->persist_refused = a.persist_refused | b.persist_refused;
        out->factor_bytes = a.factor_bytes + b.factor_bytes;
        return GMRF_OK;
    }
    h = tw_route(h);
    *out = h->stats;
    return GMRF_OK;
}

gmrf_status gmrf_bt_factor_csc(gmrf_handle* h, int64_t n, int64_t n_blocks, const int64_t* colptr,
                               const int64_t* rowval, const double* nzval, int32_t index_base,
                               int32_t* info) {
    if (!h) return bad_shape("null handle");
    HIPCHK(hipSetDevice(h->device));
    if (info) *info = 0;
    if (h->order == GMRF_ORDER_TWISTED) {
        GCHK(tw_analyze(h, n, n_blocks, colptr, rowval, index_base));
        return tw_numeric(h, nzval, info);
    }
    GCHK(analyze_csc(h, n, n_blocks, colptr, rowval, index_base));
    return numeric_factor(h, nzval, info);
}

gmrf_status gmrf_bt_factor_begin_csc(gmrf_handle* h, int64_t n, int64_t n_blocks, const int64_t* colptr,
                                     const int64_t* rowval, const double* nzval, int32_t index_base) {
    GCHK(tw_refuse(h, "gmrf_bt_factor_begin_csc"));
    if (!h) return bad_shape("null handle");
    HIPCHK(hipSetDevice(h->device));
    if (colptr) GCHK(analyze_csc(h, n, n_blocks, colptr, rowval, index_base));
    if (!h->analyzed) { g_last_error = "no sparsity pattern analysed"; return GMRF_ERR_NO_FACTOR; }
    GCHK(alloc_factor(h));
    if (h->c_dirty) {
        HIPCHK(hipMemsetAsync(h->d_C, 0, sizeof(double) * stride_pC(h) * h->B, h->stream));
        h->c_dirty = false;
    }
    persist_plan(h);
    GCHK(load_values(h, nzval));
    HIPCHK(hipMemsetAsync(h->d_info, 0, 4 * sizeof(int), h->stream));
    h->info_checked = 0; h->persist_launched = false; h->stats.persist_route = 0;
    h->factored = false; h->fy_for = nullptr;
    return GMRF_OK;
}

gmrf_status gmrf_bt_factor_step_async(gmrf_handle* h, int64_t i0, int64_t i1) {
    GCHK(tw_refuse(h, "gmrf_bt_factor_step_async"));
    if (!h) return bad_shape("null handle");
    if (i0 < 0 || i1 > h->N || i0 > i1) return bad_shape("bad block range");
    HIPCHK(hipSetDevice(h->device));
    GCHK(factor_blocks_range(h, i0, i1));
    if (h->persist_launched) GCHK(persist_check_range(h, i0, i1, nullptr));
    return GMRF_OK;
}

gmrf_status gmrf_bt_factor_end(gmrf_handle* h, int32_t* info) {
    GCHK(tw_refuse(h, "gmrf_bt_factor_end"));
    if (!h) return bad_shape("null handle");
// ... 706 lines not shown
        HIPCHK(hipStreamSynchronize(h->stream));
        return GMRF_OK;
    }));
    float ms = 0.f;
    (void)hipEventElapsedTime(&ms, h->ev0, h->ev1);
    h->stats.sample_ms = ms;
    if (h->profiling) prof_collect(h);
    return GMRF_OK;
}

static gmrf_status ensure_aux(gmrf_handle* h) {
    if (h->aux_distinct) return GMRF_OK;
    HIPCHK(hipStreamSynchronize(h->stream));
    if (h->aux) { (void)hipStreamSynchronize(h->aux); (void)hipStreamDestroy(h->aux); h->aux = nullptr; }
    const unsigned long long ticks = 100000ull;
    double one = 1e30;
    for (int r = 0; r < 2; ++r) one = std::min(one, spin_pair_ms(h->stream, nullptr, ticks));
    std::vector<hipStream_t> cand;
    for (int c = 0; c < 12 && !h->aux; ++c) {
        hipStream_t st = nullptr;
        HIPCHK(hipStreamCreateWithFlags(&st, hipStreamNonBlocking));
        hipLaunchKernelGGL(gmrf_spin_kernel, dim3(1), dim3(64), 0, st, 1ull);
        (void)hipStreamSynchronize(st);
        const double t = std::min(spin_pair_ms(h->stream, st, ticks), spin_pair_ms(h->stream, st, ticks));
        if (t < 1.5 * one) h->aux = st; else cand.push_back(st);
    }
    if (!h->aux && !cand.empty()) { h->aux = cand.back(); cand.pop_back(); }
    for (hipStream_t st : cand) (void)hipStreamDestroy(st);
    if (!h->aux) return bad_shape("internal: no second stream");
    h->aux_distinct = true;
    return GMRF_OK;
}

static gmrf_status posterior_beside(gmrf_handle* h, const double* b, uint64_t seed, int64_t first_id, int64_t k, double* mean,
                                    double* samples, int64_t ld) {
    const int kp = pad_k(k);
    GCHK(ensure_panels(h, 1));
    GCHK(sweep_persist_prepare(h, 1));
    const int64_t elems = (int64_t)kp * h->n_pad;
    if (!h->d_P2 || h->p2_elems < elems) {
        HIPCHK(hipStreamSynchronize(h->stream));
        free_dev(h->d_P2); free_dev(h->d_Y2); free_dev(h->d_T2);
        h->d_P2 = h->d_Y2 = h->d_T2 = nullptr; h->p2_elems = 0;
        HIPCHK(hipMalloc(&h->d_P2, sizeof(double) * (size_t)elems));
        HIPCHK(hipMalloc(&h->d_Y2, sizeof(double) * (size_t)elems));
        HIPCHK(hipMalloc(&h->d_T2, sizeof(double) * (size_t)elems));
        h->p2_elems = elems;
    }
    GCHK(ensure_aux(h));
    h->fork_next = 0;
    hipEvent_t ev_fork = nullptr, ev_join = nullptr;
    GCHK(fork_event(h, &ev_fork)); GCHK(fork_event(h, &ev_join));
    h->sweep_persist_launched = true;
    h->stats.sweep_persist = 1;
    h->stats.sweep_persist_launches += 3;
    HIPCHK(hipEventRecord(h->ev0, h->stream));
    HIPCHK(hipEventRecord(ev_fork, h->stream));
    HIPCHK(hipStreamWaitEvent(h->aux, ev_fork, 0));
    {
        const int64_t total = (int64_t)kp * h->n_pad;
        hipLaunchKernelGGL(fill_normals_panel, dim3((unsigned)((total + 255) / 256), 1), dim3(256), 0, h->aux, h->d_P2, h->n_pad,
                           (int)h->bs, (int)h->bsp, (int)k, kp, seed, first_id, k, nullptr, (int64_t)0);
        HIPCHK(hipGetLastError());
        GCHK(launch_sweep_persist(h, true, kp, h->d_P2, h->d_Y2, h->aux, h->d_T2));
        HIPCHK(hipEventRecord(ev_join, h->aux));
    }
    GCHK(launch_pack(h, b, h->n, 1, 1));
    GCHK(launch_sweep_persist(h, false, 1, h->d_P, h->d_Y));
    GCHK(launch_sweep_persist(h, true, 1, h->d_Y, h->d_P));
    GCHK(launch_unpack(h, h->d_P, mean, h->n, 1, nullptr));
    HIPCHK(hipStreamWaitEvent(h->stream, ev_join, 0));
    GCHK(launch_unpack(h, h->d_Y2, samples, ld, (int)k, mean));
    HIPCHK(hipEventRecord(h->ev1, h->stream));
    HIPCHK(hipStreamSynchronize(h->stream));
    return GMRF_OK;
}

static bool posterior_fused_ok(gmrf_handle* h, int64_t k, bool dev_all) {
    if (tw_on(h) || h->B <= 1 || !dev_all || h->no_fused_posterior || h->sweep_no_gemm || k <= 0 || k > KP_CHUNK) return false;
    const int kp = pad_k(k);
    if (kp % 64 != 0 || (int64_t)h->B * (h->bsp / 64) * (kp / 64) < 128) return false;
    if ((int64_t)(kp + 1) * h->n_pad * 8 >= ((int64_t)1 << 32)) return false;
    if (ensure_panels(h, kp + 1) != GMRF_OK) return false;
    h->tail_probe = true; h->tail_refused = false;
    const gmrf_status st = sweep_launches(h, true, kp, h->d_P, h->d_Y, true);
    h->tail_probe = false;
    return st == GMRF_OK && !h->tail_refused;
}

static gmrf_status posterior_fused(gmrf_handle* h, const double* b, uint64_t seed, int64_t first_id, int64_t k, double* mean,
                                   double* samples, int64_t ld) {
    const int kp = pad_k(k);
    GCHK(ensure_panels(h, kp + 1));
    HIPCHK(hipEventRecord(h->ev0, h->stream));
    const bool have_y = h->fy_for && b == h->fy_for;
    if (!have_y) {
        GCHK(launch_pack(h, b, h->n, 1, 1));
        GCHK(run_sweeps(h, GMRF_SOLVE_FORWARD, 1));
    }
    {
        const int64_t total = (int64_t)(kp + 1) * h->n_pad;
        hipLaunchKernelGGL(fill_normals_panel, dim3((unsigned)((total + 255) / 256), (unsigned)h->B), dim3(256), 0,
                           h->stream, h->d_P, h->n_pad, (int)h->bs, (int)h->bsp, (int)k, kp, seed, first_id, k,
                           have_y ? h->d_fy : h->d_Y, h->n_pad);
        HIPCHK(hipGetLastError());
    }
    GCHK(run_sweeps(h, SWEEP_BACKWARD_TAIL, kp));
    {
        const int64_t total = h->n * (k + 1);
        hipLaunchKernelGGL(unpack_panel_mean, dim3((unsigned)((total + 255) / 256), (unsigned)h->B), dim3(256), 0, h->stream, h->d_Y,
                           h->n_pad, samples, ld, mean, (int)h->bs, (int)h->bsp, h->n, (int)k, kp);
        HIPCHK(hipGetLastError());
    }
    HIPCHK(hipEventRecord(h->ev1, h->stream));
    HIPCHK(hipStreamSynchronize(h->stream));
    if (h->profiling) prof_collect(h);
    return GMRF_OK;
}

gmrf_status gmrf_bt_posterior(gmrf_handle* h, const double* b, uint64_t seed, int64_t first_id, int64_t k, double* mean,
                              double* samples, int64_t ld) {
    h = tw_route(h);
    if (!h || !b || !mean || !samples) return bad_shape("null pointer");
    if (!h->factored) { g_last_error = "posterior before factor"; return GMRF_ERR_NO_FACTOR; }
    if (k <= 0 || ld < h->n) return bad_shape("bad k / ld");
    HIPCHK(hipSetDevice(h->device));
    const bool dev_all = is_device_ptr(b) && is_device_ptr(mean) && is_device_ptr(samples);
    const int64_t vec_bytes = h->n * h->B * (int64_t)sizeof(double), smp_bytes = cols_bytes(h->n, k * h->B, ld);
    bool beside = false, fused = false;
    GCHK(sweep_guarded(h, {{b, vec_bytes, mean, vec_bytes}, {b, vec_bytes, samples, smp_bytes}, {mean, vec_bytes, samples, smp_bytes}},
                       [&]() -> gmrf_status {
        beside = !tw_on(h) && h->B == 1 && k <= KP_CHUNK && k >= 2 && dev_all && !h->profiling && sweep_persist_ok(h, 1) &&
                 sweep_persist_ok(h, pad_k(k));
        if (beside) return posterior_beside(h, b, seed, first_id, k, mean, samples, ld);
        fused = !h->sweep_persist_hold && posterior_fused_ok(h, k, dev_all);
        return fused ? posterior_fused(h, b, seed, first_id, k, mean, samples, ld) : GMRF_OK;
    }, [&]() -> gmrf_status {
        if (h->aux) HIPCHK(hipStreamSynchronize(h->aux));
        return GMRF_OK;
    }));
    if (!beside && !fused) {
        GCHK(gmrf_bt_solve(h, b, mean, 1, h->n, h->n, GMRF_SOLVE_FULL));
        return gmrf_bt_sample(h, seed, first_id, k, mean, nullptr, samples, ld);
    }
    float ms = 0.f;
    (void)hipEventElapsedTime(&ms, h->ev0, h->ev1);
    h->stats.solve_ms = ms;
    h->stats.sample_ms = 0.0;
    return GMRF_OK;
}

gmrf_status gmrf_bt_set_factor_rhs(gmrf_handle* h, const double* b) {
    if (!h) return bad_shape("null handle");
    if (b && !is_device_ptr(b)) return bad_shape("the factor's right-hand side must be device memory");
    h->frhs = b;
    h->fy_for = nullptr;
    return GMRF_OK;
}

gmrf_status gmrf_bt_normals(gmrf_handle* h, uint64_t seed, int64_t first_id, int64_t k, double* z, int64_t ld) {
    if (!h || !z) return bad_shape("null pointer");
    if (h->n <= 0) return bad_shape("no shape set");
    if (k <= 0 || ld < h->n) return bad_shape("bad k / ld");
    if (h->B > 1 && k > KP_CHUNK) return bad_shape("with a batch of problems k is limited to 128 per call");
    HIPCHK(hipSetDevice(h->device));
    const bool z_dev = is_device_ptr(z);
    for (int64_t c0 = 0; c0 < k; c0 += KP_CHUNK) {
        const int kc = (int)std::min<int64_t>(KP_CHUNK, k - c0);
        const int kp = pad_k(kc);
        GCHK(ensure_panels(h, kp));
        const int64_t total = (int64_t)kp * h->n_pad;
        hipLaunchKernelGGL(fill_normals_panel, dim3((unsigned)((total + 255) / 256), (unsigned)h->B), dim3(256), 0,
                           h->stream, h->d_P, h->n_pad, (int)h->bs, (int)h->bsp, kc, kp, seed, first_id + c0, k, nullptr, (int64_t)0);
        HIPCHK(hipGetLastError());
        GCHK(cols_out(h, h->d_P, kc, nullptr, z + c0 * ld, ld, z_dev));
        HIPCHK(hipStreamSynchronize(h->stream));
    }
    return GMRF_OK;
}

gmrf_status gmrf_bt_logdet(gmrf_handle* h, double* out) {
    h = tw_route(h);
    if (!h || !out) return bad_shape("null pointer");
    if (!h->factored) { g_last_error = "logdet before factor"; return GMRF_ERR_NO_FACTOR; }
    HIPCHK(hipSetDevice(h->device));
    if (tw_on(h)) return tw_logdet(h, out);
    if (h->keep_l && h->l_valid) {
        hipLaunchKernelGGL(logdet_blocks, dim3((unsigned)h->N, 1), dim3(256), 0, h->stream,
                           h->d_L + h->sel * stride_pL(h), blk_elems(h), h->bsp, (int)h->bs, h->d_logdet + h->sel * h->N,
                           (int64_t)0, (int64_t)0);
        HIPCHK(hipGetLastError());
    } else if (!h->logdet_valid) {
        g_last_error = "neither the L blocks nor the log-determinant parts of this factor are resident (adopted as raw buffers without L)";
        return GMRF_ERR_NO_FACTOR;
    }
    std::vector<double> part((size_t)h->N);
// ... 2711 lines not shown
    tw_free(h);
    tw_drop_own_factor(h);
    h->order = order;
    h->meet_req = meet;
    return GMRF_OK;
}

gmrf_status gmrf_bt_get_order(gmrf_handle* h, int32_t* order, int64_t* meet) {
    if (!h || !order || !meet) return bad_shape("null pointer");
    *order = h->order;
    if (h->order == GMRF_ORDER_TWISTED) *meet = (h->tw && h->tw->m >= 0) ? h->tw->m : h->meet_req;
    else *meet = h->N > 0 ? h->N - 1 : -1;
    return GMRF_OK;
}

gmrf_status gmrf_bt_half_stats(gmrf_handle* h, int32_t half, gmrf_stats* out) {
    if (!h || !out) return bad_shape("null pointer");
    if (h->order != GMRF_ORDER_TWISTED || !h->tw || !h->tw->top) return bad_shape("gmrf_bt_half_stats: not a factored twisted handle");
    if (half != 0 && half != 1) return bad_shape("half must be 0 (top) or 1 (bottom)");
    if (half == 1 && !h->tw->bot) { memset(out, 0, sizeof(*out)); return GMRF_OK; }
    *out = (half == 0 ? h->tw->top : h->tw->bot)->stats;
    return GMRF_OK;
}

gmrf_status gmrf_test_gemm(int32_t device, int64_t M, int64_t N, int64_t K, int32_t transA, int32_t transB,
                           int32_t tri_flags, int32_t lower_only, double alpha, const double* A, int64_t lda,
                           const double* B, int64_t ldb, double beta, double* C, int64_t ldc) {
    if (M % 64 || N % 64 || K % 16 || (lda & 1) || (ldb & 1)) return bad_shape("gemm test sizes");
    const bool tail = (tri_flags & 65536) != 0;
    if (tail && (transA || transB)) return bad_shape("gemm test: the tail row needs A [m][k] and B [k][n]");
    HIPCHK(hipSetDevice(device));
    const int64_t a_rows = transA ? K : M + (tail ? 1 : 0), b_rows = transB ? N : K, c_rows = M + (tail ? 1 : 0);
    double *dA, *dB, *dC;
    HIPCHK(hipMalloc(&dA, sizeof(double) * a_rows * lda));
    HIPCHK(hipMalloc(&dB, sizeof(double) * b_rows * ldb));
    HIPCHK(hipMalloc(&dC, sizeof(double) * c_rows * ldc));
    HIPCHK(hipMemcpy(dA, A, sizeof(double) * a_rows * lda, hipMemcpyHostToDevice));
    HIPCHK(hipMemcpy(dB, B, sizeof(double) * b_rows * ldb, hipMemcpyHostToDevice));
    HIPCHK(hipMemcpy(dC, C, sizeof(double) * c_rows * ldc, hipMemcpyHostToDevice));
    GemmArgs g;
    g.A = dA; g.B = dB; g.C = dC; g.lda = lda; g.ldb = ldb; g.ldc = ldc;
    g.strideA = g.strideB = g.strideC = 0;
    g.pA = g.pB = g.pC = 0; g.nb1 = 1;
    g.D = nullptr; g.ldd = 0; g.pD = 0;
    const bool force_big = (tri_flags & 2048) != 0, use_ll = (tri_flags & 4096) != 0;
    const int dma_shape = (tri_flags & 8192) ? 1 : ((tri_flags & 16384) ? 2 : ((tri_flags & 32768) ? 3 : 0));
    g.M = (int)M; g.N = (int)N; g.K = (int)K; g.tri = tri_flags & ~(2048 | 4096 | 8192 | 16384 | 32768 | 65536); g.lower_only = lower_only;
    g.alpha = alpha; g.beta = beta;
    unsigned long long* dst = nullptr;
    HIPCHK(hipMalloc(&dst, 16));
    HIPCHK(hipMemset(dst, 0, 16));
    g.stamps = (force_big || use_ll || dma_shape || tail) ? nullptr : dst;
    HIPCHK(gemm_init());
    HIPCHK(gemm_dma_init());
    if (tail) {
        const int saved_dma = gemm_dma_policy(), saved_ll = gemm_ll_policy();
        gemm_dma_policy() = 1; gemm_ll_policy() = 2;
        hipError_t le = hipSuccess;
        const bool ok = gemm_try_dma_tail(nullptr, false, true, g, 1, nullptr, nullptr, &le);
        gemm_dma_policy() = saved_dma; gemm_ll_policy() = saved_ll;
        if (!ok) { hipFree(dst); hipFree(dA); hipFree(dB); hipFree(dC); return bad_shape("gemm test: not a tail-row product"); }
        HIPCHK(le);
        HIPCHK(hipDeviceSynchronize());
        HIPCHK(hipMemcpy(C, dC, sizeof(double) * c_rows * ldc, hipMemcpyDeviceToHost));
        hipFree(dst); hipFree(dA); hipFree(dB); hipFree(dC);
        return GMRF_OK;
    }
    const int saved = gemm_big_policy(), saved_ll = gemm_ll_policy(), saved_dma = gemm_dma_policy(), saved_force = gemm_dma_force();
    gemm_big_policy() = force_big ? 1 : 2;
    gemm_ll_policy() = use_ll ? 0 : 2;
    gemm_dma_policy() = dma_shape ? 2 : 0;
    gemm_dma_force() = dma_shape;
    hipError_t le = launch_gemm(nullptr, transA != 0, transB == 0, g, 1);
    gemm_big_policy() = saved; gemm_ll_policy() = saved_ll; gemm_dma_policy() = saved_dma; gemm_dma_force() = saved_force;
    HIPCHK(le);
    HIPCHK(hipDeviceSynchronize());
    HIPCHK(hipMemcpy(C, dC, sizeof(double) * M * ldc, hipMemcpyDeviceToHost));
    HIPCHK(hipMemcpy(g_tile_stamps, dst, 16, hipMemcpyDeviceToHost));
    hipFree(dst);
    hipFree(dA); hipFree(dB); hipFree(dC);
    return GMRF_OK;
}

gmrf_status gmrf_test_gemm_shapes(gmrf_handle* h, double* rows, int64_t cap_rows, int64_t* n_rows) {
    if (!h || !n_rows) return bad_shape("null argument");
    HIPCHK(hipStreamSynchronize(h->stream));
    prof_collect(h);
    *n_rows = (int64_t)h->gemm_shapes.size();
    for (int64_t i = 0; rows && i < std::min<int64_t>(cap_rows, *n_rows); ++i) {
        const auto& g = h->gemm_shapes[(size_t)i];
        for (int c = 0; c < 8; ++c) rows[i * 11 + c] = (double)g.key[c];
        rows[i * 11 + 8] = g.launches; rows[i * 11 + 9] = g.ms; rows[i * 11 + 10] = g.work;
    }
    return GMRF_OK;
}

struct ClockProbe { int device; hipStream_t st; unsigned long long* d; int n; };
gmrf_status gmrf_test_clock_probe_start(int32_t device, int32_t n, int32_t sleeps, void** probe) {
    if (!probe || n < 2 || n > 100000 || sleeps < 1 || sleeps > 64) return bad_shape("clock probe: 2 <= n <= 100000, 1 <= sleeps <= 64");
    HIPCHK(hipSetDevice(device));
    ClockProbe* p = new ClockProbe{device, nullptr, nullptr, n};
    auto drop = [&](hipError_t e) {
        if (p->d) (void)hipFree(p->d);
        if (p->st) (void)hipStreamDestroy(p->st);
        delete p;
        g_last_error = std::string("clock probe: ") + hipGetErrorString(e);
        return GMRF_ERR_HIP;
    };
    hipError_t e = hipStreamCreateWithFlags(&p->st, hipStreamNonBlocking);
    if (e == hipSuccess) e = hipMalloc(&p->d, sizeof(unsigned long long) * 2 * 8 * (size_t)n);
    if (e == hipSuccess) e = hipMemsetAsync(p->d, 0, sizeof(unsigned long long) * 2 * 8 * (size_t)n, p->st);
    if (e != hipSuccess) return drop(e);
    hipLaunchKernelGGL(clock_probe_kernel, dim3(8), dim3(64), 0, p->st, p->d, n, sleeps);
    if ((e = hipGetLastError()) != hipSuccess) return drop(e);
    *probe = p;
    return GMRF_OK;
}
gmrf_status gmrf_test_clock_probe_finish(void* probe, double* ghz, double* t_ms) {
    ClockProbe* p = static_cast<ClockProbe*>(probe);
    if (!p || !ghz) return bad_shape("null pointer");
    std::vector<unsigned long long> h((size_t)2 * 8 * p->n);
    hipError_t e = hipSetDevice(p->device);
    if (e == hipSuccess) e = hipStreamSynchronize(p->st);
    if (e == hipSuccess) e = hipMemcpy(h.data(), p->d, h.size() * sizeof(unsigned long long), hipMemcpyDeviceToHost);
    if (e != hipSuccess) {
        (void)hipFree(p->d); (void)hipStreamDestroy(p->st);
        delete p;
        g_last_error = std::string("clock probe: ") + hipGetErrorString(e);
        return GMRF_ERR_HIP;
    }
    for (int i = 0; i + 1 < p->n; ++i) {
        double v[8];
        for (int b = 0; b < 8; ++b) {
            const unsigned long long* a = &h[((size_t)b * p->n + i) * 2];
            const double dc = (double)(a[2] - a[0]), dr = (double)(a[3] - a[1]);
            v[b] = dr > 0 ? dc / dr * 0.1 : 0.0;
        }
        std::sort(v, v + 8);
        ghz[i] = 0.5 * (v[3] + v[4]);
        if (t_ms) t_ms[i] = (double)(h[(size_t)i * 2 + 1] - h[1]) * 1e-5;
    }
    (void)hipFree(p->d); (void)hipStreamDestroy(p->st);
    delete p;
    return GMRF_OK;
}

gmrf_status gmrf_test_gemm_rate(int32_t device, int64_t M, int64_t N, int64_t K, int32_t transB, int32_t tri_flags,
                                int32_t lower_only, int32_t batch, int32_t big, int32_t reps, double* ms_per_launch) {
    if (M % 64 || N % 64 || K % 16 || batch < 1 || reps < 1) return bad_shape("gemm rate sizes");
    HIPCHK(hipSetDevice(device));
    const int64_t ld = std::max(std::max(M, N), K);
    const int64_t pm = ld * ld;
    double *dA, *dB, *dC;
    HIPCHK(hipMalloc(&dA, sizeof(double) * pm * batch));
    HIPCHK(hipMalloc(&dB, sizeof(double) * pm * batch));
    HIPCHK(hipMalloc(&dC, sizeof(double) * pm * batch));
    const int64_t tot = pm * batch;
    hipLaunchKernelGGL(fill_normals_panel, dim3((unsigned)((tot + 255) / 256)), dim3(256), 0, nullptr, dA, tot, 1 << 30,
                       1 << 30, 1, 1, 1ull, 0, 0, nullptr, (int64_t)0);
    hipLaunchKernelGGL(fill_normals_panel, dim3((unsigned)((tot + 255) / 256)), dim3(256), 0, nullptr, dB, tot, 1 << 30,
                       1 << 30, 1, 1, 2ull, 0, 0, nullptr, (int64_t)0);
    HIPCHK(hipMemset(dC, 0, sizeof(double) * pm * batch));
    GemmArgs g;
    g.A = dA; g.B = dB; g.C = dC; g.lda = g.ldb = g.ldc = ld;
    g.strideA = g.strideB = g.strideC = 0;
    g.pA = g.pB = g.pC = pm; g.nb1 = 1;
// ... 306 lines not shown
```

diffeqgmrfs.jl_amd/csrc/misc_kernels.hpp:

```cpp
#pragma once
#include <hip/hip_runtime.h>
#include <stdint.h>

namespace gmrf {

__global__ void scatter_block(const uint64_t* __restrict__ keys, const double* __restrict__ vals,
                              int64_t first, int64_t count, double* __restrict__ dst, int64_t ld,
                              int64_t pvals, int64_t pdst, int add) {
    const int64_t i = (int64_t)blockIdx.x * blockDim.x + threadIdx.x;
    if (i >= count) return;
    const uint64_t key = keys[first + i];
    const int64_t r = (int64_t)(key >> 32), c = (int64_t)(key & 0xffffffffu);
    double* d = dst + (int64_t)blockIdx.y * pdst + r * ld + c;
    const double v = vals[(int64_t)blockIdx.y * pvals + first + i];
    *d = add ? *d + v : v;
}

__global__ void zero_rows(double* __restrict__ dst, int64_t count, int64_t pdst) {
    const int64_t i = ((int64_t)blockIdx.x * blockDim.x + threadIdx.x) * 2;
    if (i < count) *reinterpret_cast<v2d*>(dst + (int64_t)blockIdx.y * pdst + i) = (v2d){0.0, 0.0};
}

__global__ void pad_identity(double* __restrict__ dst, int64_t ld, int bs, int bsp, int64_t pdst) {
    const int i = bs + blockIdx.x * blockDim.x + threadIdx.x;
// ... 22 lines not shown
constexpr double PACK_TAG_MAGIC = 1196249670.0;
__global__ void pack_tag_write(double* __restrict__ buf, int64_t pbuf, double xsplit) {
    double* q = buf + (int64_t)threadIdx.x * pbuf;
    q[0] = xsplit; q[1] = PACK_TAG_MAGIC;
}
__global__ void pack_tag_read(const double* __restrict__ buf, int64_t pbuf, int nprob, int* __restrict__ seen) {
    int code = *seen;
    for (int p = 0; p < nprob; ++p) {
        const double* q = buf + (int64_t)p * pbuf;
        const double v = q[0];
        const int c = (q[1] == PACK_TAG_MAGIC && v >= 0.0 && v < 1.0e6 && v == (double)(int)v) ? (int)v + 1 : -1;
        code = (code == 0 || code == c) ? c : -1;
    }
    *seen = code;
}

__global__ void factor_rhs_block(const double* __restrict__ b, int64_t n, int bs, int bsp, int64_t blk, double* __restrict__ t) {
    const int r = blockIdx.x * blockDim.x + threadIdx.x;
    if (r >= bsp) return;
    const int64_t p = blockIdx.y;
    t[p * bsp + r] = (r < bs) ? b[p * n + blk * bs + r] : 0.0;
}

__global__ void pack_panel(const double* __restrict__ src, int64_t ld, double* __restrict__ P,
                           int64_t n_pad, int bs, int bsp, int nblk, int k, int kp) {
    const int64_t idx = (int64_t)blockIdx.x * blockDim.x + threadIdx.x;
    const int64_t total = (int64_t)kp * n_pad;
    if (idx >= total) return;
    const int64_t r = idx / n_pad, j = idx % n_pad;
    const int64_t blk = j / bsp, off = j % bsp;
    double v = 0.0;
    if (r < k && off < bs) v = src[((int64_t)blockIdx.y * k + r) * ld + blk * bs + off];
    P[(int64_t)blockIdx.y * total + idx] = v;
}

__global__ void unpack_panel(const double* __restrict__ P, int64_t n_pad, double* __restrict__ dst,
                             int64_t ld, int bs, int bsp, int64_t n, int k, int kp,
                             const double* __restrict__ mean) {
    const int64_t idx = (int64_t)blockIdx.x * blockDim.x + threadIdx.x;
    if (idx >= n * (int64_t)k) return;
    const int64_t r = idx / n, j = idx % n;
    const int64_t blk = j / bs, off = j % bs;
    double v = P[(int64_t)blockIdx.y * kp * n_pad + r * n_pad + blk * bsp + off];
    if (mean) v += mean[(int64_t)blockIdx.y * n + j];
    dst[((int64_t)blockIdx.y * k + r) * ld + j] = v;
}

__device__ __host__ inline void philox4x32_10(uint32_t c[4], uint32_t k0, uint32_t k1) {
    for (int i = 0; i < 10; ++i) {
        const uint64_t p0 = (uint64_t)0xD2511F53u * c[0];
        const uint64_t p1 = (uint64_t)0xCD9E8D57u * c[2];
        const uint32_t n0 = (uint32_t)(p1 >> 32) ^ c[1] ^ k0;
        const uint32_t n1 = (uint32_t)p1;
        const uint32_t n2 = (uint32_t)(p0 >> 32) ^ c[3] ^ k1;
        const uint32_t n3 = (uint32_t)p0;
        c[0] = n0; c[1] = n1; c[2] = n2; c[3] = n3;
        k0 += 0x9E3779B9u; k1 += 0xBB67AE85u;
    }
}

__device__ __host__ inline double philox_normal(uint64_t seed, uint64_t dof, uint64_t sample) {
    uint32_t c[4] = {(uint32_t)dof, (uint32_t)(dof >> 32), (uint32_t)sample, (uint32_t)(sample >> 32)};
    philox4x32_10(c, (uint32_t)seed, (uint32_t)(seed >> 32));
    const uint64_t a = ((uint64_t)c[1] << 32) | c[0];
    const uint64_t b = ((uint64_t)c[3] << 32) | c[2];
    const double u1 = ((double)(a >> 11) + 0.5) * (1.0 / 9007199254740992.0);
    const double u2 = ((double)(b >> 11) + 0.5) * (1.0 / 9007199254740992.0);
    return sqrt(-2.0 * log(u1)) * cos(6.283185307179586476925 * u2);
}

__global__ void fill_normals_panel(double* __restrict__ P, int64_t n_pad, int bs, int bsp,
                                   int k, int kp, uint64_t seed, int64_t first_id, int64_t id_stride,
                                   const double* __restrict__ yrow, int64_t ystride) {
    const int64_t idx = (int64_t)blockIdx.x * blockDim.x + threadIdx.x;
    const int rows = kp + (yrow ? 1 : 0);
    if (idx >= (int64_t)rows * n_pad) return;
    const int64_t r = idx / n_pad, j = idx % n_pad;
    const int64_t blk = j / bsp, off = j % bsp;
    double v = 0.0;
    if (r == kp) v = yrow[(int64_t)blockIdx.y * ystride + j];
    else if (r < k && off < bs)
        v = philox_normal(seed, (uint64_t)(blk * bs + off), (uint64_t)(first_id + (int64_t)blockIdx.y * id_stride + r));
    P[(int64_t)blockIdx.y * rows * n_pad + idx] = v;
}

__global__ void unpack_panel_mean(const double* __restrict__ P, int64_t n_pad, double* __restrict__ dst, int64_t ld,
                                  double* __restrict__ mean_out, int bs, int bsp, int64_t n, int k, int kp) {
    const int64_t idx = (int64_t)blockIdx.x * blockDim.x + threadIdx.x;
    if (idx >= n * (int64_t)(k + 1)) return;
    const int64_t r = idx / n, j = idx % n;
    const int64_t blk = j / bs, off = j % bs;
    const double* Pp = P + (int64_t)blockIdx.y * (kp + 1) * n_pad + blk * bsp + off;
    const double mu = Pp[(int64_t)kp * n_pad];
    if (r == k) mean_out[(int64_t)blockIdx.y * n + j] = mu;
    else dst[((int64_t)blockIdx.y * k + r) * ld + j] = Pp[r * n_pad] + mu;
}

struct BxtArgs {
    const int* rowptr;
    const uint64_t* keys;
    const double* vals;
    int64_t n_entries;
    const double* X;
    double* C;
    int64_t ld, ldc, pX, pC;
    const int* kst;
    int cm, rm, bsp;
    int cw;
};

template <int KM>
__global__ __launch_bounds__(256) void spmm_bxt(BxtArgs a) {
    const int ncc = (a.bsp - a.cm) / a.cw, nrc = (a.rm + 255) / 256;
    const int nprob = (int)gridDim.x / (ncc * nrc);
    int cc, rc, prob;
    {
        const int groups = (nprob % 8 == 0) ? 8 : 1;
        const int xg = (int)blockIdx.x % groups, q = (int)blockIdx.x / groups;
        rc = q % nrc;
        cc = (q / nrc) % ncc;
        prob = xg + groups * (q / (nrc * ncc));
    }
    const int r = rc * 256 + (int)threadIdx.x;
    const int c0 = a.cm + cc * a.cw;
    const double* __restrict__ X = a.X + (int64_t)prob * a.pX;
    double* __restrict__ C = a.C + (int64_t)prob * a.pC;
    const double* __restrict__ vals = a.vals + (int64_t)prob * a.n_entries;
    int k0 = 0, len = 0;
    if (r < a.rm) { k0 = a.rowptr[r]; len = a.rowptr[r + 1] - k0; }
    int jt[KM];
    double vt[KM];
#pragma unroll
    for (int t = 0; t < KM; ++t) {
        const bool ok = t < len;
        jt[t] = ok ? (int)(a.keys[k0 + t] & 0xffffffffu) : 0;
        vt[t] = ok ? vals[k0 + t] : 0.0;
    }
    int lm = len;
#pragma unroll
    for (int off = 32; off > 0; off >>= 1) lm = max(lm, __shfl_xor(lm, off));
    lm = __builtin_amdgcn_readfirstlane(lm);
    __shared__ double ls[256 * 17];
    const int tid = (int)threadIdx.x;
    const int wr = tid >> 4, wc = tid & 15;
    const int rbase = rc * 256;
    const int cfirst = a.cm + (a.kst ? a.kst[rbase >> 6] : 0);
    for (int c = c0; c < c0 + a.cw; c += 16) {
        if (c + 16 <= cfirst) continue;
        const double* xr = X + (int64_t)c * a.ld;
        double acc[16];
#pragma unroll
        for (int u = 0; u < 16; ++u) acc[u] = 0.0;
#pragma unroll
        for (int t = 0; t < KM; ++t)
            if (t < lm) {
#pragma unroll
                for (int u = 0; u < 16; ++u) acc[u] = fma(vt[t], xr[(int64_t)u * a.ld + jt[t]], acc[u]);
            }
#pragma unroll
        for (int u = 0; u < 16; ++u) ls[tid * 17 + u] = acc[u];
        __syncthreads();
#pragma unroll 4
        for (int p = 0; p < 16; ++p) {
            const int rr = p * 16 + wr;
            if (rbase + rr < a.rm) C[(int64_t)(rbase + rr) * a.ldc + (c - a.cm) + wc] = ls[rr * 17 + wc];
        }
        __syncthreads();
    }
}

struct BxtTileArgs {
    const int* rowptr;
    const uint16_t* lidx;
    const double* vals;
    int64_t n_entries;
    const int* gtiles;
    int ng;
    const int* uptr;
// ... 929 lines not shown
```

include/gmrf_hip.h:

```cpp
#ifndef GMRF_HIP_H
#define GMRF_HIP_H

#include <stdint.h>

#ifdef __cplusplus
extern "C" {
#endif

typedef int32_t gmrf_status;

enum {
    GMRF_OK = 0,
    GMRF_ERR_NOT_SPD = -1,
    GMRF_ERR_BAD_SHAPE = -2,
    GMRF_ERR_BAND = -3,
    GMRF_ERR_HIP = -4,
    GMRF_ERR_NO_FACTOR = -5,
    GMRF_ERR_NO_DEVICE = -6,
    GMRF_ERR_ALLOC = -7,
    GMRF_ERR_RCCL = -8
};

enum { GMRF_SOLVE_FULL = 0, GMRF_SOLVE_FORWARD = 1, GMRF_SOLVE_BACKWARD = 2 };
enum { GMRF_VAR_EXACT = 0, GMRF_VAR_RBMC = 1, GMRF_VAR_MC = 2 };
// ... 177 lines not shown
                                   double* vals_out, double* f_out);

typedef struct gmrf_burgers_p1 gmrf_burgers_p1;
gmrf_status gmrf_burgers_p1_create(int32_t device, void* stream, int64_t ns, int64_t nt, double dt, double nu,
                                   gmrf_burgers_p1** out);
gmrf_status gmrf_burgers_p2_create(int32_t device, void* stream, int64_t ns, int64_t nt, double dt, double nu,
                                   gmrf_burgers_p1** out);
gmrf_status gmrf_burgers_p1_destroy(gmrf_burgers_p1* b);
gmrf_status gmrf_burgers_p1_pattern(const gmrf_burgers_p1* b, int64_t* nnz_out, int64_t* rowptr, int64_t* colidx,
                                    int32_t index_base);
gmrf_status gmrf_burgers_p1_tangent(gmrf_burgers_p1* b, const double* w, double* vals_out, double* f_out);

typedef struct gmrf_burgers_prior gmrf_burgers_prior;
gmrf_status gmrf_burgers_prior_create(int32_t device, void* stream, int64_t ns, int64_t nt, double dt, double nu, double ic_noise,
                                      gmrf_burgers_prior** out);
gmrf_status gmrf_burgers_prior_destroy(gmrf_burgers_prior* p);
gmrf_status gmrf_burgers_prior_pattern(const gmrf_burgers_prior* p, int64_t* nnz_out, int64_t* colptr, int64_t* rowval,
                                       int32_t index_base);
gmrf_status gmrf_burgers_prior_values_batch(gmrf_burgers_prior* p, int64_t batch, const double* ic, double* bulk_out,
                                            double* q_values_out, double* qx_out);

gmrf_status gmrf_burgers_p1_tangent_batch(gmrf_burgers_p1* b, int64_t batch, const double* w, double* vals_out, double* f_out);
gmrf_status gmrf_assemble_precision_batch(gmrf_assembler* as, int64_t batch, const double* q_nzval, int64_t q_stride,
                                          const double* j_vals, double noise, double* out_nzval);
gmrf_status gmrf_assemble_rhs_batch(gmrf_assembler* as, int64_t batch, const double* base, const double* j_vals,
                                    const double* x, const double* obs_diff, double noise, double* out);
gmrf_status gmrf_assemble_objective_batch(gmrf_assembler* as, int64_t batch, const double* q_nzval, int64_t q_stride,
                                          const double* x_prior, const double* x, const double* obs_diff, double noise,
                                          double* obj_out);
typedef struct gmrf_gn gmrf_gn;
gmrf_status gmrf_gn_create(gmrf_handle* h, gmrf_assembler* as, gmrf_burgers_p1* b, gmrf_gn** out);
gmrf_status gmrf_gn_destroy(gmrf_gn* g);
gmrf_status gmrf_gn_run(gmrf_gn* g, const double* q_nzval, int64_t q_stride, const double* qx_prior, const double* x_prior,
                        double* x, const double* y, double noise, double rtol, int32_t max_steps, int32_t* steps_out,
                        double* obj_hist_out, int32_t* info);
gmrf_status gmrf_gn_finalize(gmrf_gn* g, int32_t* info);

typedef struct gmrf_bic gmrf_bic;
gmrf_status gmrf_bic_create(gmrf_handle* h, gmrf_assembler* as, gmrf_burgers_prior* prior, gmrf_bic** out);
gmrf_status gmrf_bic_destroy(gmrf_bic* g);
gmrf_status gmrf_bic_run(gmrf_bic* g, const double* ic, double* x_ic_out, double* q_values_out, double* qx_out, double* bulk_out,
                         int32_t* info);

gmrf_status gmrf_field_errors_batch(int32_t device, void* stream, int64_t batch, int64_t n, int64_t first, const double* pred,
                                    const double* soln, double* out);

typedef struct gmrf_elliptic_p1 gmrf_elliptic_p1;
gmrf_status gmrf_elliptic_p1_create(int32_t device, void* stream, int64_t nx, int64_t ny, gmrf_elliptic_p1** out);
gmrf_status gmrf_elliptic_p1_destroy(gmrf_elliptic_p1* e);
gmrf_status gmrf_elliptic_p1_pattern(const gmrf_elliptic_p1* e, int64_t* nnz_out, int64_t* rowptr, int64_t* colidx,
                                     int32_t index_base);
gmrf_status gmrf_elliptic_p1_qpoints(const gmrf_elliptic_p1* e, double* xy);
gmrf_status gmrf_elliptic_p1_tangent(gmrf_elliptic_p1* e, const double* w, double* vals_out, double* f_out);
gmrf_status gmrf_elliptic_p1_tangent_batch(gmrf_elliptic_p1* e, int64_t batch, const double* w, double* vals_out, double* f_out);
gmrf_status gmrf_elliptic_p1_load(gmrf_elliptic_p1* e, int64_t batch, const double* src_q, double* b_out);
gmrf_status gmrf_gn_create_elliptic(gmrf_handle* h, gmrf_assembler* as, gmrf_elliptic_p1* e, gmrf_gn** out);

gmrf_status gmrf_darcy_p1_assemble_batch(gmrf_darcy_p1* d, int64_t batch, const double* coeff_tables, int64_t ng, double beta,
                                         double* vals_out, double* f_out);
typedef struct gmrf_dc gmrf_dc;
gmrf_status gmrf_dc_create(gmrf_handle* h, gmrf_assembler* as, gmrf_darcy_p1* d, gmrf_dc** out);
gmrf_status gmrf_dc_destroy(gmrf_dc* g);
gmrf_status gmrf_dc_run(gmrf_dc* g, const double* coeff_tables, int64_t ng, double beta, const double* q_nzval, int64_t q_stride,
                        const double* q_mu, double q_eps, int64_t k_samples, uint64_t sample_seed, int32_t var_method, int64_t k_var,
                        uint64_t var_seed, double* mean_out, double* samples_out, double* std_out, double* std_norm_out,
                        int32_t* info);

typedef struct gmrf_swe_p1 gmrf_swe_p1;
gmrf_status gmrf_shallow_water_p1_create(int32_t device, void* stream, int64_t nx, int64_t ny, gmrf_swe_p1** out);
gmrf_status gmrf_shallow_water_p1_destroy(gmrf_swe_p1* w);
gmrf_status gmrf_shallow_water_p1_pattern(const gmrf_swe_p1* w, int32_t which, int64_t* nnz_out, int64_t* rowptr, int64_t* colidx,
                                          int32_t index_base);
gmrf_status gmrf_shallow_water_p1_qpoints(const gmrf_swe_p1* w, double* xy);
gmrf_status gmrf_shallow_water_p1_assemble(gmrf_swe_p1* w, const double* H_q, double k, double f, double g, const uint8_t* prescribed,
                                           double* K_vals, double* M_lumped, double* S_vals);
gmrf_status gmrf_shallow_water_p1_operators(gmrf_swe_p1* w, const double* K_vals, const double* M_lumped, const double* S_vals,
                                            const uint8_t* prescribed, double kappa_matern, double tau, double dt, double* G_vals,
                                            double* J_vals, double* M_tilde, double* beta);

gmrf_status gmrf_test_gemm(int32_t device, int64_t M, int64_t N, int64_t K, int32_t transA,
                           int32_t transB, int32_t tri_flags, int32_t lower_only,
                           double alpha, const double* A, int64_t lda, const double* B,
                           int64_t ldb, double beta, double* C, int64_t ldc);
gmrf_status gmrf_test_gemm_rate(int32_t device, int64_t M, int64_t N, int64_t K, int32_t transB,
                                int32_t tri_flags, int32_t lower_only, int32_t batch,
                                int32_t big, int32_t reps, double* ms_per_launch);
gmrf_status gmrf_test_gemm_shapes(gmrf_handle* h, double* rows, int64_t cap_rows, int64_t* n_rows);
gmrf_status gmrf_test_potrf_tile(int32_t device, double* tile64 ,
                                 double* inv64, int32_t* info);
gmrf_status gmrf_test_tile_timing(double* out, int32_t n);
gmrf_status gmrf_test_potrf_block(int32_t device, int64_t bs, double* S ,
                                  double* Linv, int32_t* info);
gmrf_status gmrf_test_persist_stamps(double* out, int32_t n);
gmrf_status gmrf_test_persist_aborts(gmrf_handle* h, int32_t* n);
gmrf_status gmrf_test_factor_fwd(gmrf_handle* h, int32_t* state, double* y_out);
gmrf_status gmrf_test_gn_route(gmrf_gn* g, int32_t* iterations, int32_t* fwd_iterations);
gmrf_status gmrf_test_dc_route(gmrf_dc* g, int32_t* fwd_in_factor);
gmrf_status gmrf_test_bic_route(gmrf_bic* g, int32_t* fwd_in_factor);
gmrf_status gmrf_test_var_groups(gmrf_handle* h, int32_t* group_size, int32_t* groups);
gmrf_status gmrf_test_persist_budget(int32_t cus, int32_t n, const int32_t* demands, int32_t* granted);
gmrf_status gmrf_test_mfma_f64_rate(int32_t device, double* tflops);
gmrf_status gmrf_test_clock_probe_start(int32_t device, int32_t n, int32_t sleeps, void** probe);
gmrf_status gmrf_test_clock_probe_finish(void* probe, double* ghz, double* t_ms);
gmrf_status gmrf_test_hbm_rate(int32_t device, int64_t bytes, double* gbps);
gmrf_status gmrf_test_microbench(int32_t device, double* out, int32_t n);
gmrf_status gmrf_test_symbolic_csc(int64_t n, int64_t n_blocks, const int64_t* colptr, const int64_t* rowval,
                                   int32_t index_base, int64_t* out8);

#ifdef __cplusplus
}
#endif
#endif
```

Before: 53260 solves/s.

## Fuse sample+mean unpack into tail GEMM epilogue and add grouped two-GEMM launch

The backward tail-row GEMM now writes the final samples (panel value plus mean) and the mean straight to the user output buffers from its epilogue. This removes the separate unpack_panel_mean kernel and its extra read and write of the panel. A grouped kernel that runs two independent 64x64 LDS-DMA GEMMs in one launch is also added, switchable through an eager bit, to cut launch count. The cost is extra epilogue stores and LDS syncs in every tile of the direct-output GEMM, plus a small pointer-setup kernel before each sweep.

```diff
diff --git a/diffeqgmrfs.jl_amd/_cabi.py b/diffeqgmrfs.jl_amd/_cabi.py
--- a/diffeqgmrfs.jl_amd/_cabi.py
+++ b/diffeqgmrfs.jl_amd/_cabi.py
@@ -40,7 +40,7 @@
     "gmrf_darcy_p1_assemble_batch", "gmrf_dc_create", "gmrf_dc_destroy", "gmrf_dc_run",
     "gmrf_burgers_prior_create", "gmrf_burgers_prior_destroy", "gmrf_burgers_prior_pattern", "gmrf_burgers_prior_values_batch",
     "gmrf_bic_create", "gmrf_bic_destroy", "gmrf_bic_run", "gmrf_field_errors_batch",
-    "gmrf_test_gemm", "gmrf_test_gemm_rate", "gmrf_test_gemm_shapes", "gmrf_test_potrf_tile", "gmrf_test_potrf_block", "gmrf_test_tile_timing", "gmrf_test_persist_stamps", "gmrf_test_persist_aborts", "gmrf_test_factor_fwd", "gmrf_test_gn_route", "gmrf_test_dc_route", "gmrf_test_bic_route", "gmrf_test_var_groups", "gmrf_test_persist_budget", "gmrf_test_clock_probe_start", "gmrf_test_clock_probe_finish",
+    "gmrf_test_gemm", "gmrf_test_gemm_pair", "gmrf_test_gemm_rate", "gmrf_test_gemm_shapes", "gmrf_test_potrf_tile", "gmrf_test_potrf_block", "gmrf_test_tile_timing", "gmrf_test_persist_stamps", "gmrf_test_persist_aborts", "gmrf_test_factor_fwd", "gmrf_test_gn_route", "gmrf_test_dc_route", "gmrf_test_bic_route", "gmrf_test_var_groups", "gmrf_test_persist_budget", "gmrf_test_clock_probe_start", "gmrf_test_clock_probe_finish",
     "gmrf_test_mfma_f64_rate", "gmrf_test_hbm_rate", "gmrf_test_microbench", "gmrf_test_symbolic_csc",
 ]
 
@@ -205,6 +205,7 @@
         "gmrf_spmm_rows": [vp, vp, vp, i64, i64, i64],
         "gmrf_test_gemm": [i32, i64, i64, i64, i32, i32, i32, i32, dbl, vp, i64, vp, i64, dbl, vp, i64],
         "gmrf_test_gemm_shapes": [vp, P(dbl), i64, P(i64)],
+        "gmrf_test_gemm_pair": [i32, i32, i32, vp, vp, vp, vp, vp, vp, vp, vp],
         "gmrf_test_gemm_rate": [i32, i64, i64, i64, i32, i32, i32, i32, i32, i32, P(dbl)],
         "gmrf_test_potrf_tile": [i32, vp, vp, P(i32)],
         "gmrf_test_potrf_block": [i32, i64, vp, vp, P(i32)],
diff --git a/diffeqgmrfs.jl_amd/csrc/gemm_f64.hpp b/diffeqgmrfs.jl_amd/csrc/gemm_f64.hpp
--- a/diffeqgmrfs.jl_amd/csrc/gemm_f64.hpp
+++ b/diffeqgmrfs.jl_amd/csrc/gemm_f64.hpp
@@ -19,6 +19,12 @@
     TRI_A_UPPER = 2,
     TRI_B_LOWER = 4,
     TRI_B_UPPER = 8
+};
+
+struct GemmDirectOut {
+    double* samples;
+    double* mean;
+    int64_t ld, k;
 };
 
 struct GemmArgs {
@@ -44,6 +50,9 @@
     const double* tD = nullptr;
     int64_t ptA = 0, ptC = 0, ptD = 0;
     double tbeta = 0.0;
+    const GemmDirectOut* dout = nullptr;
+    int64_t o_j0 = 0, o_n = 0;
+    int o_cols = 0;
 };
 
 constexpr int GEMM_BM = 64;
diff --git a/diffeqgmrfs.jl_amd/csrc/gemm_f64_dma.hpp b/diffeqgmrfs.jl_amd/csrc/gemm_f64_dma.hpp
--- a/diffeqgmrfs.jl_amd/csrc/gemm_f64_dma.hpp
+++ b/diffeqgmrfs.jl_amd/csrc/gemm_f64_dma.hpp
@@ -16,16 +16,16 @@
 #define GMRF_GLB_PTR(p) ((const __attribute__((address_space(1))) void*)(p))
 
 template <int BM, int BN>
-__device__ __forceinline__ void gemm_dma_tile_order(const GemmArgs& g, int& bm, int& bn, int& z) {
+__device__ __forceinline__ void gemm_dma_tile_order(const GemmArgs& g, int bid, int gdim, int& bm, int& bn, int& z) {
     const int nx = g.N / BN, ny = g.M / BM;
     int tpp;
     if (g.lower_only == 1) {
         if (BM >= BN) tpp = (BM / BN) * ny * (ny + 1) / 2;
         else tpp = 0;
     } else tpp = nx * ny;
-    const int nz = (int)gridDim.x / tpp;
+    const int nz = gdim / tpp;
     const int groups = (nz % 8 == 0) ? 8 : 1;
-    const int xg = (int)blockIdx.x % groups, q = (int)blockIdx.x / groups, nzg = nz / groups;
+    const int xg = bid % groups, q = bid / groups, nzg = nz / groups;
     int zq;
     if (g.lower_only == 1) {
         constexpr int R = BM / BN > 0 ? BM / BN : 1;
@@ -52,8 +52,8 @@
     z = xg + groups * zq;
 }
 
-template <int BM, int BN, bool B_N, int STAGES, bool A_T = false, bool TAIL = false>
-__global__ __launch_bounds__(256, (BM + BN > 128) ? 3 : 4) void gemm_f64_dma(GemmArgs g) {
+template <int BM, int BN, bool B_N, int STAGES, bool A_T, bool TAIL, bool DOUT>
+__device__ __forceinline__ void gemm_dma_body(const GemmArgs& g, const int bid, const int gdim) {
     constexpr int BK = DMA_BK;
     constexpr int MI = BM / 32, NJ = BN / 32;
     constexpr int NA = BM / 32, NB = BN / 32;
@@ -61,9 +61,11 @@
     static_assert(NJ % 2 == 0 || !B_N, "the [k][n] image pairs neighbouring column tiles");
     static_assert(MI % 2 == 0 || !A_T, "the [k][m] image pairs neighbouring row tiles");
     static_assert(!TAIL || (BM == 64 && BN == 64 && !A_T), "the tail row: 64 x 64 tiles");
+    static_assert(!DOUT || (TAIL && B_N), "direct output: the tail-row product on B [k][n]");
     int bm, bn, z;
-    gemm_dma_tile_order<BM, BN>(g, bm, bn, z);
-    const bool tail = TAIL && (g.lower_only == 1 ? bm == bn : bm == g.M / BM - 1);
+    gemm_dma_tile_order<BM, BN>(g, bid, gdim, bm, bn, z);
+    const bool tail_owner = TAIL && (g.lower_only == 1 ? bm == bn : bm == g.M / BM - 1);
+    const bool tail = DOUT || tail_owner;
     const int m0 = bm * BM, n0 = bn * BN;
     if (g.lower_only == 2 && n0 > m0 + BM - 1) return;
     const int zi = z % g.nb1, zp = z / g.nb1;
@@ -232,6 +234,33 @@
     auto orow = [&](int i, int r) -> int64_t {
         return A_T ? m0 + wm + 32 * (i >> 1) + 2 * (lq + 4 * r) + (i & 1) : m0 + wm + i * 16 + lq + 4 * r;
     };
+    v2d mu[NJ / 2 > 0 ? NJ / 2 : 1];
+    double* o_s = nullptr;
+    int64_t o_ld = 0;
+    int o_k = 0;
+    if constexpr (DOUT) {
+        const GemmDirectOut o = *g.dout;
+        o_ld = o.ld; o_k = (int)o.k;
+        o_s = o.samples + (int64_t)zp * o.k * o.ld + g.o_j0;
+        __syncthreads();
+        *reinterpret_cast<v2d*>(gsm + (tkg * 4 + lq) * BN + wn + 2 * li) = tacc;
+        __syncthreads();
+        if (w == 0) {
+            double s = 0.0;
+#pragma unroll
+            for (int q = 0; q < 8; ++q) s += gsm[q * BN + lane];
+            double v = alpha * s;
+            if (beta != 0.0) v += beta * Dm[(int64_t)g.M * ldd + n0 + lane];
+            if (tail_owner) {
+                C[(int64_t)g.M * g.ldc + n0 + lane] = v;
+                if (n0 + lane < g.o_cols) o.mean[(int64_t)zp * g.o_n + g.o_j0 + n0 + lane] = v;
+            }
+            gsm[8 * BN + lane] = v;
+        }
+        __syncthreads();
+#pragma unroll
+        for (int jp = 0; jp < NJ / 2; ++jp) mu[jp] = *reinterpret_cast<const v2d*>(gsm + 8 * BN + wn + jp * 32 + 2 * li);
+    }
     if (B_N) {
         v2d d[MI][4][NJ / 2 > 0 ? NJ / 2 : 1];
         if (beta != 0.0) {
@@ -252,6 +281,14 @@
                     v2d v = (v2d){alpha * acc[i][2 * jp][r], alpha * acc[i][2 * jp + 1][r]};
                     if (beta != 0.0) { v.x += beta * d[i][r][jp].x; v.y += beta * d[i][r][jp].y; }
                     *reinterpret_cast<v2d*>(C + orow(i, r) * g.ldc + n0 + wn + jp * 32 + 2 * li) = v;
+                    if constexpr (DOUT) {
+                        const int c = n0 + wn + jp * 32 + 2 * li;
+                        if (orow(i, r) < o_k) {
+                            double* sp = o_s + orow(i, r) * o_ld + c;
+                            if (c < g.o_cols) sp[0] = __dadd_rn(v.x, mu[jp].x);
+                            if (c + 1 < g.o_cols) sp[1] = __dadd_rn(v.y, mu[jp].y);
+                        }
+                    }
                 }
     } else {
         double d[MI][4][NJ];
@@ -275,7 +312,7 @@
                     C[orow(i, r) * g.ldc + n0 + wn + j * 16 + li] = v;
                 }
     }
-    if constexpr (TAIL) {
+    if constexpr (TAIL && !DOUT) {
         if (tail) {
             __syncthreads();
             if (B_N) *reinterpret_cast<v2d*>(gsm + (tkg * 4 + lq) * BN + wn + 2 * li) = tacc;
@@ -298,6 +335,24 @@
             }
         }
     }
+}
+
+__global__ void set_direct_out(GemmDirectOut* o, double* samples, double* mean, int64_t ld, int64_t k) {
+    o->samples = samples; o->mean = mean; o->ld = ld; o->k = k;
+}
+
+template <int BM, int BN, bool B_N, int STAGES, bool A_T = false, bool TAIL = false, bool DOUT = false>
+__global__ __launch_bounds__(256, (BM + BN > 128) ? 3 : 4) void gemm_f64_dma(GemmArgs g) {
+    gemm_dma_body<BM, BN, B_N, STAGES, A_T, TAIL, DOUT>(g, (int)blockIdx.x, (int)gridDim.x);
+}
+
+template <int STAGES>
+__global__ __launch_bounds__(256, 4) void gemm_f64_dma_grouped(GemmArgs g0, GemmArgs g1, int wg0, int wg1, int b_n) {
+    const bool second = (int)blockIdx.x >= wg0;
+    const GemmArgs g = second ? g1 : g0;
+    const int bid = second ? (int)blockIdx.x - wg0 : (int)blockIdx.x, gdim = second ? wg1 : wg0;
+    if ((b_n >> (second ? 1 : 0)) & 1) gemm_dma_body<64, 64, true, STAGES, false, false, false>(g, bid, gdim);
+    else gemm_dma_body<64, 64, false, STAGES, false, false, false>(g, bid, gdim);
 }
 
 inline int& gemm_dma_policy() {
@@ -353,10 +408,13 @@
 inline bool gemm_tail_ok(bool a_t, bool b_n, const GemmArgs& g, int batch) {
     if (a_t || gemm_uses_ll(g, batch) || gemm_dma_shape(false, g, batch) != 1) return false;
     if (g.lower_only && g.M != g.N) return false;
+    if (g.tC && g.dout) return false;
     if (g.tC) {
         return g.nb1 == 1 && g.tA && ((uintptr_t)g.tA & 15) == 0 && (g.ptA & 1) == 0;
     }
     if (!b_n || g.lower_only) return false;
+    if (g.dout && g.nb1 != 1) return false;
+    if (g.dout && (g.beta != 0.0 || g.kb_m || g.kb_n || g.ke_n)) return false;
     return (int64_t)(g.M + 1) * g.ldc * 8 < ((int64_t)1 << 32) && (!g.D || (int64_t)(g.M + 1) * g.ldd * 8 < ((int64_t)1 << 32));
 }
 inline bool gemm_try_dma_tail(hipStream_t st, bool a_t, bool b_n, const GemmArgs& g, int batch, hipEvent_t ev_start, hipEvent_t ev_stop,
@@ -375,11 +433,19 @@
         if (ev_start) hipExtLaunchKernelGGL((gemm_f64_dma<64, 64, BNAT, ST, false, true>), grid, block, lds, st, ev_start, ev_stop, 0, gs); \
         else hipLaunchKernelGGL((gemm_f64_dma<64, 64, BNAT, ST, false, true>), grid, block, lds, st, gs);                \
     } while (0)
-    if (gemm_dma_stages() == 3) {
+#define GMRF_DMA_TKO(ST)                                                                                                   \
+    do {                                                                                                                   \
+        if (ev_start) hipExtLaunchKernelGGL((gemm_f64_dma<64, 64, true, ST, false, true, true>), grid, block, lds, st, ev_start, ev_stop, 0, gs); \
+        else hipLaunchKernelGGL((gemm_f64_dma<64, 64, true, ST, false, true, true>), grid, block, lds, st, gs);          \
+    } while (0)
+    if (g.dout) {
+        if (gemm_dma_stages() == 3) GMRF_DMA_TKO(3); else GMRF_DMA_TKO(2);
+    } else if (gemm_dma_stages() == 3) {
         if (b_n) GMRF_DMA_TK(true, 3); else GMRF_DMA_TK(false, 3);
     } else {
         if (b_n) GMRF_DMA_TK(true, 2); else GMRF_DMA_TK(false, 2);
     }
+#undef GMRF_DMA_TKO
 #undef GMRF_DMA_TK
     *err = hipGetLastError();
     return true;
@@ -425,4 +491,40 @@
     return true;
 }
 
-}
+inline bool gemm_grouped_ok(const GemmArgs& g0, const GemmArgs& g1, int batch) {
+    if (gemm_dma_policy() == 0 || g0.tC || g1.tC || g0.dout || g1.dout) return false;
+    if (g0.lower_only && g0.M != g0.N) return false;
+    if (g1.lower_only && g1.M != g1.N) return false;
+    return gemm_dma_shape(false, g0, batch) != 0 && gemm_dma_shape(false, g1, batch) != 0;
+}
+inline int64_t gemm_dma_grid64(const GemmArgs& g, int batch) {
+    const int64_t nx = g.N / 64, ny = g.M / 64;
+    return ((g.lower_only && g.M == g.N) ? ny * (ny + 1) / 2 : nx * ny) * batch;
+}
+inline bool gemm_try_dma_grouped(hipStream_t st, bool b_n0, const GemmArgs& g0, bool b_n1, const GemmArgs& g1, int batch,
+                                 hipEvent_t ev_start, hipEvent_t ev_stop, hipError_t* err) {
+    if (!gemm_grouped_ok(g0, g1, batch)) return false;
+    static const bool asc_off = [] { const char* e = getenv("GMRF_GEMM_G2_ORDER"); return e && atoi(e) == 0; }();
+    GemmArgs gs[2] = {g0, g1};
+    for (GemmArgs& g : gs) {
+        const bool tri_grid = g.lower_only && g.M == g.N;
+        g.lower_only = tri_grid ? 1 : 0;
+        if (tri_grid && (g.kb_m || g.kb_n) && !asc_off) g.tri |= DMA_ROWS_ASCENDING;
+    }
+    const int wg0 = (int)gemm_dma_grid64(g0, batch), wg1 = (int)gemm_dma_grid64(g1, batch);
+    const int bn = (b_n0 ? 1 : 0) | (b_n1 ? 2 : 0);
+    const dim3 grid((unsigned)(wg0 + wg1)), block(256);
+    const int stages = gemm_dma_stages();
+    const size_t lds = gemm_dma_lds_bytes<64, 64>(stages);
+#define GMRF_DMA_GK(ST)                                                                                                   \
+    do {                                                                                                                  \
+        if (ev_start) hipExtLaunchKernelGGL((gemm_f64_dma_grouped<ST>), grid, block, lds, st, ev_start, ev_stop, 0, gs[0], gs[1], wg0, wg1, bn); \
+        else hipLaunchKernelGGL((gemm_f64_dma_grouped<ST>), grid, block, lds, st, gs[0], gs[1], wg0, wg1, bn);           \
+    } while (0)
+    if (stages == 3) GMRF_DMA_GK(3); else GMRF_DMA_GK(2);
+#undef GMRF_DMA_GK
+    *err = hipGetLastError();
+    return true;
+}
+
+}
diff --git a/diffeqgmrfs.jl_amd/csrc/gmrf_hip.hip b/diffeqgmrfs.jl_amd/csrc/gmrf_hip.hip
--- a/diffeqgmrfs.jl_amd/csrc/gmrf_hip.hip
+++ b/diffeqgmrfs.jl_amd/csrc/gmrf_hip.hip
@@ -204,6 +204,8 @@
     const double* fy_for = nullptr;
     bool fwd_run = false;
     bool no_factor_fwd = false;
+    bool no_grouped_gemm = false;
+    GemmDirectOut* d_dout = nullptr;
     double* d_ft = nullptr;
     double* d_fy = nullptr;
     int64_t fy_elems = 0;
@@ -344,7 +346,24 @@
     double* C; int64_t pC;
     const double* D; int64_t pD;
     double beta;
+    const GemmDirectOut* out = nullptr;
+    int64_t j0 = 0;
+    int cols = 0;
 };
+
+static inline double gemm_flops(int M, int N, int K, int tri, int lower_only, double nprob) {
+    double flops = 2.0 * M * N * (double)K * nprob;
+    if (lower_only) flops *= 0.5 * (1.0 + 64.0 / std::max(M, 64));
+    if (tri) flops *= 0.5 * (1.0 + 64.0 / std::max(K, 64));
+    return flops;
+}
+static int gemm_shape_row(gmrf_handle* h, const int64_t (&key)[8]) {
+    for (size_t i = 0; i < h->gemm_shapes.size(); ++i)
+        if (!memcmp(h->gemm_shapes[i].key, key, sizeof(key))) return (int)i;
+    GemmShapeStat st; memcpy(st.key, key, sizeof(key));
+    h->gemm_shapes.push_back(st);
+    return (int)h->gemm_shapes.size() - 1;
+}
 
 static gmrf_status gemm(gmrf_handle* h, bool a_t, bool b_n, int M, int N, int K, int tri, int lower_only,
                         double alpha, const double* A, int64_t lda, const double* B, int64_t ldb,
@@ -355,7 +374,8 @@
                         const GemmTail* gt = nullptr) {
     GemmArgs g;
     if (gt) {
-        g.tA = gt->A; g.ptA = gt->pA; g.tC = gt->C; g.ptC = gt->pC; g.tD = gt->D; g.ptD = gt->pD; g.tbeta = gt->beta;
+        if (gt->C) { g.tA = gt->A; g.ptA = gt->pA; g.tC = gt->C; g.ptC = gt->pC; g.tD = gt->D; g.ptD = gt->pD; g.tbeta = gt->beta; }
+        g.dout = gt->out; g.o_j0 = gt->j0; g.o_cols = gt->cols; g.o_n = h->n;
         tail = true;
     }
     g.kb_m = kb_m; g.kb_n = kb_n; g.ke_n = ke_n;
@@ -366,9 +386,7 @@
     g.pA = pA; g.pB = pB; g.pC = pC; g.nb1 = batch;
     g.M = M; g.N = N; g.K = K; g.tri = tri; g.lower_only = lower_only;
     g.alpha = alpha; g.beta = beta; g.stamps = nullptr;
-    double flops = 2.0 * M * N * (double)K * batch * (double)h->B;
-    if (lower_only) flops *= 0.5 * (1.0 + 64.0 / std::max(M, 64));
-    if (tri) flops *= 0.5 * (1.0 + 64.0 / std::max(K, 64));
+    double flops = gemm_flops(M, N, K, tri, lower_only, batch * (double)h->B);
     if (tail) {
         if (!gemm_tail_ok(a_t, b_n, g, batch * (int)h->B)) {
             h->tail_refused = true;
@@ -384,12 +402,7 @@
             p.kind = pclass; p.work = pwork >= 0.0 ? pwork : flops;
             p.a = ev_get(h); p.b = ev_get(h);
             const int64_t key[8] = {pclass, M + 1, N, K, tri, lower_only, batch * h->B, (kb_m || kb_n || ke_n) ? 1 : 0};
-            for (size_t i = 0; i < h->gemm_shapes.size() && p.shape < 0; ++i)
-                if (!memcmp(h->gemm_shapes[i].key, key, sizeof(key))) p.shape = (int)i;
-            if (p.shape < 0) {
-                GemmShapeStat st; memcpy(st.key, key, sizeof(key));
-                h->gemm_shapes.push_back(st); p.shape = (int)h->gemm_shapes.size() - 1;
-            }
+            p.shape = gemm_shape_row(h, key);
             (void)gemm_try_dma_tail(h->gemm_stream ? h->gemm_stream : h->stream, a_t, b_n, g, batch * (int)h->B, p.a, p.b, &e);
             HIPCHK(e);
             h->events.push_back(p);
@@ -410,17 +423,57 @@
         p.kind = pclass; p.work = pwork >= 0.0 ? pwork : flops;
         p.a = ev_get(h); p.b = ev_get(h);
         const int64_t key[8] = {pclass, M, N, K, tri, lower_only, batch * h->B, (kb_m || kb_n || ke_n) ? 1 : 0};
-        for (size_t i = 0; i < h->gemm_shapes.size() && p.shape < 0; ++i)
-            if (!memcmp(h->gemm_shapes[i].key, key, sizeof(key))) p.shape = (int)i;
-        if (p.shape < 0) {
-            GemmShapeStat st; memcpy(st.key, key, sizeof(key));
-            h->gemm_shapes.push_back(st); p.shape = (int)h->gemm_shapes.size() - 1;
-        }
+        p.shape = gemm_shape_row(h, key);
         HIPCHK(launch_gemm(h->gemm_stream ? h->gemm_stream : h->stream, a_t, b_n, g, batch * (int)h->B, p.a, p.b));
         h->events.push_back(p);
         return GMRF_OK;
     }
     HIPCHK(launch_gemm(h->gemm_stream ? h->gemm_stream : h->stream, a_t, b_n, g, batch * (int)h->B));
+    return GMRF_OK;
+}
+
+struct GemmOne {
+    bool b_n; int M, N, K, tri, lower_only;
+    double alpha; const double* A; int64_t lda; const double* B; int64_t ldb; double beta; double* C; int64_t ldc;
+    int64_t pA, pB, pC;
+    double pwork;
+};
+static gmrf_status gemm_one(gmrf_handle* h, const GemmOne& q) {
+    return gemm(h, false, q.b_n, q.M, q.N, q.K, q.tri, q.lower_only, q.alpha, q.A, q.lda, q.B, q.ldb, q.beta, q.C, q.ldc, q.pA, q.pB, q.pC,
+                1, 0, 0, 0, nullptr, 0, 0, 0, q.pwork);
+}
+static gmrf_status gemm_pair(gmrf_handle* h, const GemmOne& q0, const GemmOne& q1) {
+    GemmArgs g[2];
+    const GemmOne* q[2] = {&q0, &q1};
+    double work[2];
+    for (int i = 0; i < 2; ++i) {
+        GemmArgs& a = g[i];
+        a.A = q[i]->A; a.B = q[i]->B; a.C = q[i]->C; a.lda = q[i]->lda; a.ldb = q[i]->ldb; a.ldc = q[i]->ldc;
+        a.strideA = a.strideB = a.strideC = 0;
+        a.pA = q[i]->pA; a.pB = q[i]->pB; a.pC = q[i]->pC; a.nb1 = 1;
+        a.M = q[i]->M; a.N = q[i]->N; a.K = q[i]->K; a.tri = q[i]->tri; a.lower_only = q[i]->lower_only;
+        a.alpha = q[i]->alpha; a.beta = q[i]->beta; a.D = nullptr; a.ldd = 0; a.pD = 0; a.stamps = nullptr;
+        work[i] = q[i]->pwork >= 0.0 ? q[i]->pwork : gemm_flops(a.M, a.N, a.K, a.tri, a.lower_only, (double)h->B);
+    }
+    if (h->no_grouped_gemm || !gemm_grouped_ok(g[0], g[1], (int)h->B)) {
+        GCHK(gemm_one(h, q0));
+        return gemm_one(h, q1);
+    }
+    hipStream_t st = h->gemm_stream ? h->gemm_stream : h->stream;
+    hipError_t e = hipSuccess;
+    if (h->profiling > 0) {
+        EvPair p;
+        p.kind = 14; p.work = work[0] + work[1];
+        p.a = ev_get(h); p.b = ev_get(h);
+        const int64_t key[8] = {14, q0.M + q1.M, q0.N, q0.K, q0.tri | (q1.tri << 8), q0.lower_only | (q1.lower_only << 8), h->B, 0};
+        p.shape = gemm_shape_row(h, key);
+        (void)gemm_try_dma_grouped(st, q0.b_n, g[0], q1.b_n, g[1], (int)h->B, p.a, p.b, &e);
+        HIPCHK(e);
+        h->events.push_back(p);
+        return GMRF_OK;
+    }
+    (void)gemm_try_dma_grouped(st, q0.b_n, g[0], q1.b_n, g[1], (int)h->B, nullptr, nullptr, &e);
+    HIPCHK(e);
     return GMRF_OK;
 }
 
@@ -1100,11 +1153,12 @@
                 GCHK(diag128(j));
                 GCHK(gemm(h, false, false, 128, 128, 128, TRI_B_UPPER, 0, 1.0, S + ob * ld + oa, ld, X + oa * ld + oa, ld, 0.0, L + ob * ld + oa, ld,
                           sa.pS, sa.pX, sa.pL, 1, 0, 0, 0, nullptr, 0, 0, 0, 2.0 * t3 * 3.0 * 2.0 * nb));
-                GCHK(gemm(h, false, false, 128, 128, 128, 0, 1, -1.0, L + ob * ld + oa, ld, L + ob * ld + oa, ld, 1.0, S + ob * ld + ob, ld,
-                          sa.pL, sa.pL, sa.pS, 1, 0, 0, 0, nullptr, 0, 0, 0, 2.0 * t3 * 2.0 * 3.0 * nb));
+                GCHK(gemm_pair(h,
+                               GemmOne{false, 128, 128, 128, 0, 1, -1.0, L + ob * ld + oa, ld, L + ob * ld + oa, ld, 1.0, S + ob * ld + ob, ld,
+                                       sa.pL, sa.pL, sa.pS, 2.0 * t3 * 2.0 * 3.0 * nb},
+                               GemmOne{true, 128, 128, 128, TRI_B_LOWER, 0, 1.0, L + ob * ld + oa, ld, X + oa * ld + oa, ld, 0.0, T + ob * ld + oa, ld,
+                                       sa.pL, sa.pX, pW, -1.0}));
                 GCHK(diag128(j + 2));
-                GCHK(gemm(h, false, true, 128, 128, 128, TRI_B_LOWER, 0, 1.0, L + ob * ld + oa, ld, X + oa * ld + oa, ld, 0.0, T + ob * ld + oa, ld,
-                          sa.pL, sa.pX, pW));
                 GCHK(gemm(h, false, true, 128, 128, 128, TRI_A_LOWER, 0, -1.0, X + ob * ld + ob, ld, T + ob * ld + oa, ld, 0.0, X + ob * ld + oa, ld,
                           sa.pX, pW, sa.pX));
             }
@@ -1683,7 +1737,8 @@
     return body();
 }
 
-static gmrf_status sweep_launches(gmrf_handle* h, bool backward, int kp, double* Pin, double* Yout, bool tail = false) {
+static gmrf_status sweep_launches(gmrf_handle* h, bool backward, int kp, double* Pin, double* Yout, bool tail = false,
+                                  const GemmDirectOut* dout = nullptr) {
     if (!tail && sweep_persist_ok(h, kp)) return launch_sweep_persist(h, backward, kp, Pin, Yout);
     const int bsp = (int)h->bsp;
     const int64_t ld = bsp, bstride = (int64_t)bsp * bsp, npad = h->n_pad;
@@ -1701,6 +1756,7 @@
     const double blk_work_t = ((kp == 1) ? 4.0 * bsp * (double)(bsp + 1) : 1.0 * bsp * (double)(bsp + 1) * kp) * nprob;
     const bool via_gemm = (kp % 64 == 0) && !h->sweep_no_gemm && (int64_t)nprob * (bsp / 64) * (kp / 64) >= 128;
     if (tail && (!via_gemm || !backward)) return bad_shape("internal: the tail row needs the backward sweep on the GEMM");
+    if (dout && !tail) return bad_shape("internal: direct output needs the tail-row sweep");
     for (int64_t step = 0; step < N; ++step) {
         const int64_t i = backward ? (N - 1 - step) : step;
         double* rhs = Pin + i * bsp;
@@ -1726,6 +1782,7 @@
         }
         const double* X = h->d_Linv + i * bstride;
         double* yout = Yout + i * bsp;
+        auto direct = [&](int first) { return GemmTail{nullptr, 0, nullptr, 0, nullptr, 0, 0.0, dout, i * h->bs + first, (int)h->bs - first}; };
         if (h->xsplit > 0) {
             const int p = h->xsplit, q = bsp - p;
             const double* Xbb = X + (int64_t)p * ld + p;
@@ -1734,12 +1791,15 @@
                 const int which = backward ? 2 - part : part;
                 if (via_gemm) {
                     constexpr int64_t z0 = 0;
+                    const GemmTail da = direct(0), db = direct(p);
                     if (which == 0)
                         GCHK(gemm(h, false, backward, kp, p, p, backward ? TRI_B_LOWER : TRI_B_UPPER, 0, 1.0, rhs, npad, X, ld, 0.0, yout, npad,
-                                  pPanel, pX, pPanel, 1, z0, z0, z0, nullptr, z0, z0, 0, -1.0, nullptr, nullptr, nullptr, tail));
+                                  pPanel, pX, pPanel, 1, z0, z0, z0, nullptr, z0, z0, 0, -1.0, nullptr, nullptr, nullptr, tail,
+                                  dout ? &da : nullptr));
                     else if (which == 2)
                         GCHK(gemm(h, false, backward, kp, q, q, backward ? TRI_B_LOWER : TRI_B_UPPER, 0, 1.0, rhs + p, npad, Xbb, ld, 0.0,
-                                  yout + p, npad, pPanel, pX, pPanel, 1, z0, z0, z0, nullptr, z0, z0, 0, -1.0, nullptr, nullptr, nullptr, tail));
+                                  yout + p, npad, pPanel, pX, pPanel, 1, z0, z0, z0, nullptr, z0, z0, 0, -1.0, nullptr, nullptr, nullptr, tail,
+                                  dout ? &db : nullptr));
                     else if (!backward)
                         GCHK(gemm(h, false, false, kp, q, p, 0, 0, -1.0, yout, npad, Lba, ld, 1.0, rhs + p, npad, pPanel, pX, pPanel));
                     else
@@ -1757,8 +1817,9 @@
                 }
             }
         } else if (via_gemm) {
+            const GemmTail da = direct(0);
             GCHK(gemm(h, false, backward, kp, bsp, bsp, backward ? TRI_B_LOWER : TRI_B_UPPER, 0, 1.0, rhs, npad, X, ld, 0.0,
-                      yout, npad, pPanel, pX, pPanel, 1, 0, 0, 0, nullptr, 0, 0, 0, -1.0, nullptr, nullptr, nullptr, tail));
+                      yout, npad, pPanel, pX, pPanel, 1, 0, 0, 0, nullptr, 0, 0, 0, -1.0, nullptr, nullptr, nullptr, tail, dout ? &da : nullptr));
         } else {
             s.Mat = X; s.ld = ld; s.Xin = rhs; s.ldx = npad; s.Bin = nullptr; s.ldb = 0; s.Out = yout; s.ldo = npad;
             s.rows = bsp; s.kdim = bsp; s.sub = 0;
@@ -1775,7 +1836,7 @@
 static gmrf_status run_sweeps(gmrf_handle* h, int mode, int kp) {
     auto body = [&]() -> gmrf_status {
         if (mode == GMRF_SOLVE_FORWARD) return sweep_launches(h, false, kp, h->d_P, h->d_Y);
-        if (mode == SWEEP_BACKWARD_TAIL) return sweep_launches(h, true, kp, h->d_P, h->d_Y, true);
+        if (mode == SWEEP_BACKWARD_TAIL) return sweep_launches(h, true, kp, h->d_P, h->d_Y, true, h->d_dout);
         if (mode == SWEEP_BACKWARD_YP) return sweep_launches(h, true, kp, h->d_Y, h->d_P);
         if (mode == GMRF_SOLVE_BACKWARD) return sweep_launches(h, true, kp, h->d_P, h->d_Y);
         GCHK(sweep_launches(h, false, kp, h->d_P, h->d_Y));
@@ -1913,7 +1974,7 @@
     free_dev(h->d_S); free_dev(h->d_B); free_dev(h->d_T); free_dev(h->d_W);
     free_dev(h->d_sweep_flags); free_dev(h->d_Tsw); free_dev(h->d_P2); free_dev(h->d_Y2); free_dev(h->d_T2);
     if (h->h_sweep_abort) { (void)hipHostFree(h->h_sweep_abort); h->h_sweep_abort = nullptr; }
-    free_dev(h->d_info); free_dev(h->d_logdet); free_dev(h->d_pflags); free_dev(h->d_kbx); free_dev(h->d_V);
+    free_dev(h->d_dout); free_dev(h->d_info); free_dev(h->d_logdet); free_dev(h->d_pflags); free_dev(h->d_kbx); free_dev(h->d_V);
     free_dev(h->d_P); free_dev(h->d_Y); free_dev(h->d_Tp);
     free_dev(h->d_stage); h->mean_arena.release(); free_dev(h->d_acc);
     free_dev(h->d_ft); free_dev(h->d_fy);
@@ -1976,6 +2037,7 @@
     if (((eager & 131072) != 0) != h->no_scatter_fold) { destroy_graphs(h); h->no_scatter_fold = (eager & 131072) != 0; }
     h->no_fused_posterior = (eager & 262144) != 0;
     h->no_factor_fwd = (eager & 524288) != 0;
+    if (((eager & 1048576) != 0) != h->no_grouped_gemm) { destroy_graphs(h); h->no_grouped_gemm = (eager & 1048576) != 0; }
     if (eager != h->eager_bits) h->fy_for = nullptr;
     h->eager = (eager & 1) != 0;
     h->eager_bits = eager;
@@ -2848,8 +2910,9 @@
     if (kp % 64 != 0 || (int64_t)h->B * (h->bsp / 64) * (kp / 64) < 128) return false;
     if ((int64_t)(kp + 1) * h->n_pad * 8 >= ((int64_t)1 << 32)) return false;
     if (ensure_panels(h, kp + 1) != GMRF_OK) return false;
+    if (!h->d_dout && hipMalloc(&h->d_dout, sizeof(GemmDirectOut)) != hipSuccess) { (void)hipGetLastError(); return false; }
     h->tail_probe = true; h->tail_refused = false;
-    const gmrf_status st = sweep_launches(h, true, kp, h->d_P, h->d_Y, true);
+    const gmrf_status st = sweep_launches(h, true, kp, h->d_P, h->d_Y, true, h->d_dout);
     h->tail_probe = false;
     return st == GMRF_OK && !h->tail_refused;
 }
@@ -2871,13 +2934,9 @@
                            have_y ? h->d_fy : h->d_Y, h->n_pad);
         HIPCHK(hipGetLastError());
     }
+    hipLaunchKernelGGL(set_direct_out, dim3(1), dim3(1), 0, h->stream, h->d_dout, samples, mean, ld, k);
+    HIPCHK(hipGetLastError());
     GCHK(run_sweeps(h, SWEEP_BACKWARD_TAIL, kp));
-    {
-        const int64_t total = h->n * (k + 1);
-        hipLaunchKernelGGL(unpack_panel_mean, dim3((unsigned)((total + 255) / 256), (unsigned)h->B), dim3(256), 0, h->stream, h->d_Y,
-                           h->n_pad, samples, ld, mean, (int)h->bs, (int)h->bsp, h->n, (int)k, kp);
-        HIPCHK(hipGetLastError());
-    }
     HIPCHK(hipEventRecord(h->ev1, h->stream));
     HIPCHK(hipStreamSynchronize(h->stream));
     if (h->profiling) prof_collect(h);
@@ -5755,6 +5814,56 @@
     return GMRF_OK;
 }
 
+gmrf_status gmrf_test_gemm_pair(int32_t device, int32_t batch, int32_t grouped, const int64_t* desc, const double* ab,
+                                const double* A0, const double* B0, double* C0, const double* A1, const double* B1, double* C1) {
+    if (!desc || !ab || !A0 || !B0 || !C0 || !A1 || !B1 || !C1 || batch < 1) return bad_shape("gemm pair test: null pointer / batch");
+    HIPCHK(hipSetDevice(device));
+    HIPCHK(gemm_init());
+    HIPCHK(gemm_dma_init());
+    const double* hA[2] = {A0, A1};
+    const double* hB[2] = {B0, B1};
+    double* hC[2] = {C0, C1};
+    double *dA[2] = {nullptr, nullptr}, *dB[2] = {nullptr, nullptr}, *dC[2] = {nullptr, nullptr};
+    GemmArgs g[2];
+    bool b_n[2];
+    auto drop = [&]() { for (int i = 0; i < 2; ++i) { free_dev(dA[i]); free_dev(dB[i]); free_dev(dC[i]); } };
+    for (int i = 0; i < 2; ++i) {
+        const int64_t M = desc[6 * i], N = desc[6 * i + 1], K = desc[6 * i + 2];
+        b_n[i] = desc[6 * i + 3] != 0;
+        if (M <= 0 || N <= 0 || K <= 0 || M % 64 || N % 64 || K % 16) { drop(); return bad_shape("gemm pair test sizes"); }
+        const size_t na = sizeof(double) * M * K * batch, nb = sizeof(double) * K * N * batch, nc = sizeof(double) * M * N * batch;
+        hipError_t e = hipMalloc(&dA[i], na);
+        if (e == hipSuccess) e = hipMalloc(&dB[i], nb);
+        if (e == hipSuccess) e = hipMalloc(&dC[i], nc);
+        if (e == hipSuccess) e = hipMemcpy(dA[i], hA[i], na, hipMemcpyHostToDevice);
+        if (e == hipSuccess) e = hipMemcpy(dB[i], hB[i], nb, hipMemcpyHostToDevice);
+        if (e == hipSuccess) e = hipMemcpy(dC[i], hC[i], nc, hipMemcpyHostToDevice);
+        if (e != hipSuccess) { drop(); HIPCHK(e); }
+        GemmArgs& a = g[i];
+        a.A = dA[i]; a.B = dB[i]; a.C = dC[i]; a.lda = K; a.ldb = b_n[i] ? N : K; a.ldc = N;
+        a.strideA = a.strideB = a.strideC = 0;
+        a.pA = M * K; a.pB = K * N; a.pC = M * N; a.nb1 = 1;
+        a.M = (int)M; a.N = (int)N; a.K = (int)K; a.tri = (int)desc[6 * i + 4]; a.lower_only = (int)desc[6 * i + 5];
+        a.alpha = ab[2 * i]; a.beta = ab[2 * i + 1]; a.D = nullptr; a.ldd = 0; a.pD = 0; a.stamps = nullptr;
+    }
+    const int saved = gemm_big_policy(), saved_ll = gemm_ll_policy(), saved_dma = gemm_dma_policy(), saved_force = gemm_dma_force();
+    gemm_big_policy() = 2; gemm_ll_policy() = 2; gemm_dma_policy() = 2; gemm_dma_force() = 1;
+    hipError_t le = hipSuccess;
+    bool ok = true;
+    if (grouped) ok = gemm_try_dma_grouped(nullptr, b_n[0], g[0], b_n[1], g[1], batch, nullptr, nullptr, &le);
+    else {
+        for (int i = 0; i < 2 && ok && le == hipSuccess; ++i) ok = gemm_try_dma(nullptr, false, b_n[i], g[i], batch, nullptr, nullptr, &le);
+    }
+    gemm_big_policy() = saved; gemm_ll_policy() = saved_ll; gemm_dma_policy() = saved_dma; gemm_dma_force() = saved_force;
+    if (!ok) { drop(); return bad_shape("gemm pair test: not a pair of LDS-DMA products"); }
+    if (le == hipSuccess) le = hipDeviceSynchronize();
+    for (int i = 0; i < 2 && le == hipSuccess; ++i)
+        le = hipMemcpy(hC[i], dC[i], sizeof(double) * g[i].M * g[i].N * batch, hipMemcpyDeviceToHost);
+    drop();
+    HIPCHK(le);
+    return GMRF_OK;
+}
+
 gmrf_status gmrf_test_gemm_shapes(gmrf_handle* h, double* rows, int64_t cap_rows, int64_t* n_rows) {
     if (!h || !n_rows) return bad_shape("null argument");
     HIPCHK(hipStreamSynchronize(h->stream));
diff --git a/diffeqgmrfs.jl_amd/csrc/misc_kernels.hpp b/diffeqgmrfs.jl_amd/csrc/misc_kernels.hpp
--- a/diffeqgmrfs.jl_amd/csrc/misc_kernels.hpp
+++ b/diffeqgmrfs.jl_amd/csrc/misc_kernels.hpp
@@ -128,18 +128,6 @@
     else if (r < k && off < bs)
         v = philox_normal(seed, (uint64_t)(blk * bs + off), (uint64_t)(first_id + (int64_t)blockIdx.y * id_stride + r));
     P[(int64_t)blockIdx.y * rows * n_pad + idx] = v;
-}
-
-__global__ void unpack_panel_mean(const double* __restrict__ P, int64_t n_pad, double* __restrict__ dst, int64_t ld,
-                                  double* __restrict__ mean_out, int bs, int bsp, int64_t n, int k, int kp) {
-    const int64_t idx = (int64_t)blockIdx.x * blockDim.x + threadIdx.x;
-    if (idx >= n * (int64_t)(k + 1)) return;
-    const int64_t r = idx / n, j = idx % n;
-    const int64_t blk = j / bs, off = j % bs;
-    const double* Pp = P + (int64_t)blockIdx.y * (kp + 1) * n_pad + blk * bsp + off;
-    const double mu = Pp[(int64_t)kp * n_pad];
-    if (r == k) mean_out[(int64_t)blockIdx.y * n + j] = mu;
-    else dst[((int64_t)blockIdx.y * k + r) * ld + j] = Pp[r * n_pad] + mu;
 }
 
 struct BxtArgs {
diff --git a/include/gmrf_hip.h b/include/gmrf_hip.h
--- a/include/gmrf_hip.h
+++ b/include/gmrf_hip.h
@@ -283,6 +283,8 @@
                            int32_t transB, int32_t tri_flags, int32_t lower_only,
                            double alpha, const double* A, int64_t lda, const double* B,
                            int64_t ldb, double beta, double* C, int64_t ldc);
+gmrf_status gmrf_test_gemm_pair(int32_t device, int32_t batch, int32_t grouped, const int64_t* desc, const double* ab,
+                                const double* A0, const double* B0, double* C0, const double* A1, const double* B1, double* C1);
 gmrf_status gmrf_test_gemm_rate(int32_t device, int64_t M, int64_t N, int64_t K, int32_t transB,
                                 int32_t tri_flags, int32_t lower_only, int32_t batch,
                                 int32_t big, int32_t reps, double* ms_per_launch);
```

Result: faster. 54040 solves/s (median of 6 runs) (+1.5%).
